# MonsieurETM/QPSK

Hardware: AMD Instinct MI355X
Metric: complex Msamples/s demodulated + % HBM roofline, 2400-baud RRC+Costas path (higher is better)
Workload: dtype f32

## Files before the change

qpsk_amd/csrc/api.cpp:

```cpp
#include "../../include/qpsk_hip.h"
#include "host_math.h"
#include "kernels.h"

#include <hip/hip_runtime.h>
#include <limits.h>
#include <math.h>
#include <stdarg.h>
#include <stdio.h>
#include <stdlib.h>
#include <string.h>
#include <time.h>
#include <algorithm>
#include <initializer_list>
#include <map>
#include <vector>

using namespace qpsk;

static thread_local char g_err[512] = "";

static int fail(int code, const char *fmt, ...)
{
    va_list ap;
    va_start(ap, fmt);
    vsnprintf(g_err, sizeof g_err, fmt, ap);
    va_end(ap);
    return code;
}

#define HIP_TRY(expr)                                                                         \
    do {                                                                                      \
        hipError_t e_ = (expr);                                                               \
        if (e_ != hipSuccess)                                                                 \
            return fail(QPSK_ERR_HIP, "%s: %s (%s:%d)", #expr, hipGetErrorString(e_), __FILE__, __LINE__); \
    } while (0)

#define KERNEL_TRY(expr)                                                                      \
    do {                                                                                      \
        (void)hipGetLastError();  \
        int e_ = (expr);                                                                      \
        if (e_ != 0)                                                                          \
            return fail(QPSK_ERR_HIP, "%s: %s (%s:%d)", #expr, hipGetErrorString((hipError_t)e_), __FILE__, __LINE__); \
    } while (0)

struct DevBuf {
    void *p = nullptr;
    size_t cap = 0;
};

struct Tuning {
    int fused_g = -1, fused_s = -1, fused_lds = -1;
    int generic = -1;
    int pipe_nf = -1;
    int pipe_v = -1, pipe_g = -1;
    int layout_lo = -1, layout_hi = -1;
    int pipe_variant = -1;
    int hist_generic = -1;
    int fir_generic = -1;
    int stream_scan = -1;
    int stream_poll = -1;
    int stream_block = -1;
    int stream_carrier = -1;
    int lean_dma = -1;
    int hist_onepass = -1;
    int est_waves = -1;
    int lean_pair = -1;
    int viterbi_lds = -1;
    int fft_fused = -1;
    int viterbi_chunk_rows = -1;
};

static const struct { const char *name; int Tuning::*field; } TUNING_KEYS[] = {
    {"QPSK_FUSED_G", &Tuning::fused_g},       {"QPSK_FUSED_S", &Tuning::fused_s},     {"QPSK_FUSED_LDS", &Tuning::fused_lds},
    {"QPSK_FUSED_GENERIC", &Tuning::generic}, {"QPSK_PIPE_NF", &Tuning::pipe_nf},
    {"QPSK_PIPE_DBG", &Tuning::pipe_variant}, {"QPSK_HIST_GENERIC", &Tuning::hist_generic},
    {"QPSK_PIPE_V", &Tuning::pipe_v},         {"QPSK_PIPE_G", &Tuning::pipe_g},
    {"QPSK_PIPE_LAYOUT_LO", &Tuning::layout_lo}, {"QPSK_PIPE_LAYOUT_HI", &Tuning::layout_hi},
    {"QPSK_FIR_GENERIC", &Tuning::fir_generic}, {"QPSK_FFT_FUSED", &Tuning::fft_fused},
    {"QPSK_STREAM_BLOCK", &Tuning::stream_block}, {"QPSK_STREAM_POLL", &Tuning::stream_poll},
    {"QPSK_STREAM_SCAN", &Tuning::stream_scan}, {"QPSK_STREAM_CARRIER", &Tuning::stream_carrier},
    {"QPSK_LEAN_DMA", &Tuning::lean_dma},     {"QPSK_LEAN_PAIR", &Tuning::lean_pair},
    {"QPSK_EST_WAVES", &Tuning::est_waves},   {"QPSK_HIST_ONEPASS", &Tuning::hist_onepass},
    {"QPSK_VITERBI_LDS", &Tuning::viterbi_lds},   {"QPSK_VITERBI_CHUNK_ROWS", &Tuning::viterbi_chunk_rows},
};

#ifdef QPSK_PIPE_PROFILE
static const int PIPE_VARIANT_MASK = ~0;
#else
static const int PIPE_VARIANT_MASK = 4 | 8 | 16 | 64 | 128 | 256 | 512 | 1024 | 8192;
#endif

struct qpsk_ctx {
    int device = 0;
    Tuning tune;
    int ncu = 256;
    const char *last_kernel = "";
    int viterbi_launches = 0;
    bool taps_symmetric = false;
    hipStream_t stream = nullptr;
    qpsk_params prm{};
    int cycles = 0, nsym = 0;
    float taps[QPSK_NTAPS];
    float damping = 0.f, alpha = 0.f, beta = 0.f;
    float min_freq = 0.f, max_freq = 0.f;
    float *d_taps = nullptr;
    float *d_gains = nullptr;
    unsigned *h_done = nullptr, *d_done = nullptr;
    unsigned done_expect = 0;
    int *h_status = nullptr;
    int *d_status = nullptr;
    std::vector<float> h_gains;
    DevBuf index, filtered, mixed, keystream, sympad, mislist;
    DevBuf datacostas;
    DevBuf vitdec;
    DevBuf softgain;
    int32_t *d_hint = nullptr;
    int32_t *h_hist_stats = nullptr, *d_hist_stats = nullptr;
    bool hint_valid = false;
    int keystream_len = 0;
    std::map<int, double *> twiddles;
    float *d_fast = nullptr;
    bool fast_valid = false;
    int nstreams = 0;
    float *s_memory = nullptr, *s_dec = nullptr, *s_loop = nullptr, *s_mixer = nullptr;
    float *s_ctab = nullptr, *s_cstate = nullptr;
    bool carrier_shared = false;
    unsigned carrier_blocks = 0;
    unsigned carrier_scans = 0;
    float *carrier_pending = nullptr;
    bool stream_work_unchecked = false;
    bool streams_poisoned = false;
    unsigned char *h_stage = nullptr, *d_stage = nullptr;
    size_t stage_cap = 0;
    int ntx = 0;
    uint8_t *t_hist = nullptr;
    float *t_mixer = nullptr;
    DevBuf tx_b;
    uint8_t *df_state = nullptr, *df_tables = nullptr;
    size_t df_stride = 0;
    int df_nstreams = 0, df_nsync = 0, df_min_score = 0, df_nbytes = 0, df_max_packets = 0;
    unsigned long long df_sync_lo[2] = {0, 0}, df_sync_hi[2] = {0, 0};
    bool df_ready = false;
    bool df_coded = false;
    int df_mode = 0, df_nsteps = 0;
    int df_nbody = 0;
    bool df_punct = false;
    Puncture df_pattern = {1, 1u, 1u, 2};
    float df_scale = 0.f;
    unsigned df_crc_init = 0;
    DevBuf dfstage;
};

static const int MAX_BW = 64;

static int ensure(qpsk_ctx *c, DevBuf &b, size_t bytes)
{
    if (b.cap >= bytes) return QPSK_OK;
    if (b.p) {
        HIP_TRY(hipStreamSynchronize(c->stream));
        HIP_TRY(hipFree(b.p));
        b.p = nullptr;
        b.cap = 0;
    }
    hipError_t e = hipMalloc(&b.p, bytes);
    if (e != hipSuccess) {
        b.p = nullptr;
        return fail(QPSK_ERR_ALLOC, "hipMalloc(%zu bytes): %s", bytes, hipGetErrorString(e));
    }
    b.cap = bytes;
    return QPSK_OK;
}

static int check_status(qpsk_ctx *c)
{
    const int st = __atomic_exchange_n(c->h_status, 0, __ATOMIC_ACQ_REL);
    if (st != STATUS_PIPE_TIMEOUT) c->stream_work_unchecked = false;
    if (st == STATUS_PIPE_TIMEOUT) {
        if (c->nstreams > 0 && c->stream_work_unchecked) {
            c->streams_poisoned = true;
            c->carrier_shared = false;
            c->carrier_pending = nullptr;
        }
        c->stream_work_unchecked = false;
        return fail(QPSK_ERR_HIP, "pipeline kernel: producer/consumer wait timed out; results of the calls since the last synchronisation are invalid");
    }
    if (st == STATUS_PHASE_RANGE)
        return fail(QPSK_ERR_RANGE, "Costas loop phase beyond the bounded 2 pi wrap (input amplitude far outside the modem's range; "
                                    "the reference's phase_wrap() would spin or hang, costas_loop.c:61-67); results of the calls since the last synchronisation are invalid");
    if (st == STATUS_BAD_INDEX)
        return fail(QPSK_ERR_ARG, "an external timing offset (qpsk_rx_batch_ext d_index_in) lies outside 0..%d: the kernel demodulated that frame "
                                  "at offset 0; results of the calls since the last synchronisation are invalid", MAX_INDEX);
    if (st == STATUS_EST_NONFINITE)
        return fail(QPSK_ERR_RANGE, "qpsk_carrier_est_batch: a NaN / Inf sample inside the window the estimate reads; results of the calls since "
                                    "the last synchronisation are invalid");
    if (st == STATUS_SOFT_NONFINITE)
        return fail(QPSK_ERR_RANGE, "qpsk_soft_batch / qpsk_deframer_push_coded: a NaN / Inf sample among those a row's sums or soft output use, or a NaN / Inf gain; "
                                    "results of the calls since the last synchronisation are invalid");
    if (st == STATUS_SOFT_BAD_LAG)
        return fail(QPSK_ERR_ARG, "qpsk_soft_batch: a lag in d_lag is negative or puts the payload beyond the row (that row's soft output is zeros); "
                                  "results of the calls since the last synchronisation are invalid");
    if (st == STATUS_NONFINITE)
        return fail(QPSK_ERR_RANGE, "a Costas loop ended on a NaN / Inf state: the input held a non-finite sample (the reference hangs in phase_wrap() "
                                    "on an infinite phase, costas_loop.c:61-67); results of the calls since the last synchronisation are invalid");
    if (st != 0) return fail(QPSK_ERR_HIP, "kernel status %d", st);
    return QPSK_OK;
}

int qpsk_test_inject_status(qpsk_ctx *c, int code)
{
    if (!c || !c->h_status) return fail(QPSK_ERR_ARG, "null context");
    __atomic_store_n(c->h_status, code, __ATOMIC_RELEASE);
    return QPSK_OK;
}

int qpsk_test_hist_state(qpsk_ctx *c, int32_t *out)
{
    if (!c || !out) return fail(QPSK_ERR_ARG, "null argument");
    out[0] = out[1] = out[2] = out[3] = out[4] = -1;
    if (!c->d_hint) return QPSK_OK;
    HIP_TRY(hipSetDevice(c->device));
    HIP_TRY(hipStreamSynchronize(c->stream));
    int32_t h[2];
    HIP_TRY(hipMemcpy(h, c->d_hint, sizeof h, hipMemcpyDeviceToHost));
    out[0] = c->hint_valid ? h[0] : -1;
    out[1] = h[1];
    out[2] = c->h_hist_stats[0]; out[3] = c->h_hist_stats[1]; out[4] = c->h_hist_stats[2];
    return QPSK_OK;
}

static int bind(const qpsk_ctx *c)
{
    HIP_TRY(hipSetDevice(c->device));
    return QPSK_OK;
}

static int use_context_gains(qpsk_ctx *c)
{
    const float g[2] = {c->alpha, c->beta};
    if (c->h_gains.size() != 2 || c->h_gains[0] != g[0] || c->h_gains[1] != g[1]) {
        HIP_TRY(hipStreamSynchronize(c->stream));
        c->h_gains.assign(g, g + 2);
        HIP_TRY(hipMemcpyAsync(c->d_gains, c->h_gains.data(), sizeof g, hipMemcpyHostToDevice, c->stream));
    }
    return QPSK_OK;
}

extern "C" {

const char *qpsk_last_error(void) { return g_err; }
const char *qpsk_version(void) { return "qpsk_hip 0.3 (gfx950)"; }

int qpsk_device_count(void)
{
    int n = 0;
    if (hipGetDeviceCount(&n) != hipSuccess) return 0;
    return n;
}

void qpsk_params_default(qpsk_params *p)
{
    if (!p) return;
    p->fs = 9600.0;
    p->rs = 2400.0;
    p->frame_size = 512;
    p->rrc_alpha = .35f;
    p->loop_bw = (float)(2.0 * 3.14159265358979323846 / 100.0f);
    p->min_freq = -1.0f;
    p->max_freq = 1.0f;
    p->timing_mode = QPSK_TIMING_HIST;
    p->fixed_index = 0;
}

static int upload_config(qpsk_ctx *c)
{
    float t128[128];
    memset(t128, 0, sizeof t128);
    memcpy(t128, c->taps, sizeof c->taps);
    c->taps_symmetric = true;
    for (int k = 0; k < QPSK_NTAPS / 2; k++)
        if (memcmp(&c->taps[k], &c->taps[QPSK_NTAPS - 1 - k], sizeof(float)) != 0) c->taps_symmetric = false;
    HIP_TRY(hipMemcpyAsync(c->d_taps, t128, sizeof t128, hipMemcpyHostToDevice, c->stream));
    const float g[2] = {c->alpha, c->beta};
    c->h_gains.assign(g, g + 2);
    HIP_TRY(hipMemcpyAsync(c->d_gains, c->h_gains.data(), sizeof g, hipMemcpyHostToDevice, c->stream));
    HIP_TRY(hipStreamSynchronize(c->stream));
    return QPSK_OK;
}

int qpsk_ctx_create(qpsk_ctx **out, int device, const qpsk_params *p, void *stream)
{
    if (!out || !p) return fail(QPSK_ERR_ARG, "qpsk_ctx_create: null argument");
    *out = nullptr;
    int ndev = 0;
    hipError_t e = hipGetDeviceCount(&ndev);
    if (e != hipSuccess || ndev <= 0)
        return fail(QPSK_ERR_NO_DEVICE, "no HIP device available (%s); this library has no CPU path",
                    e == hipSuccess ? "device count 0" : hipGetErrorString(e));
    if (device < 0) HIP_TRY(hipGetDevice(&device));
    if (device >= ndev) return fail(QPSK_ERR_NO_DEVICE, "device %d out of range (%d devices)", device, ndev);
    if (!(p->fs > 0.0) || !(p->rs > 0.0) || p->frame_size <= 0)
        return fail(QPSK_ERR_ARG, "fs, rs and frame_size must be positive");
    const int cycles = (int)(p->fs / p->rs);
    if (cycles < 1 || cycles > 64) return fail(QPSK_ERR_ARG, "CYCLES = (int)(fs/rs) = %d out of range 1..64", cycles);
    if (p->frame_size % cycles != 0)
        return fail(QPSK_ERR_ARG, "frame_size %d is not a multiple of CYCLES %d", p->frame_size, cycles);
    if (p->timing_mode < QPSK_TIMING_HIST || p->timing_mode > QPSK_TIMING_FFT)
        return fail(QPSK_ERR_ARG, "unknown timing_mode %d", p->timing_mode);
    if (p->fixed_index < 0 || p->fixed_index > MAX_INDEX)
        return fail(QPSK_ERR_ARG, "fixed_index %d outside 0..%d", p->fixed_index, MAX_INDEX);

    HIP_TRY(hipSetDevice(device));
    KERNEL_TRY(prepare_kernels());
    KERNEL_TRY(prepare_pipe_kernel());
    KERNEL_TRY(prepare_timing_scan());
    KERNEL_TRY(prepare_stream_block());
    KERNEL_TRY(prepare_stream_scan());
    KERNEL_TRY(prepare_carrier_est());
    qpsk_ctx *c = new qpsk_ctx();
    c->device = device;
    for (const auto &k : TUNING_KEYS) {
        const char *v = getenv(k.name);
        if (!v || !*v) continue;
        if (k.field == &Tuning::viterbi_chunk_rows) {
            char *end = nullptr;
            const long n = strtol(v, &end, 10);
            if (end == v || *end) continue;
            c->tune.*(k.field) = n < 0 ? -1 : n > INT_MAX ? INT_MAX : (int)n;
            continue;
        }
        c->tune.*(k.field) = atoi(v);
    }
    if (c->tune.viterbi_chunk_rows == 0) {
        delete c;
        return fail(QPSK_ERR_ARG, "qpsk_ctx_create: QPSK_VITERBI_CHUNK_ROWS = 0 in the environment (>= 1, or negative for the library's own choice)");
    }
    {
        int ncu = 0;
        if (hipDeviceGetAttribute(&ncu, hipDeviceAttributeMultiprocessorCount, device) == hipSuccess && ncu > 0)
            c->ncu = ncu;
    }
    c->prm = *p;
    c->cycles = cycles;
    c->nsym = p->frame_size / cycles;
    c->stream = (hipStream_t)stream;
    qpsk_host_rrc_taps((float)p->fs, (float)p->rs, p->rrc_alpha, c->taps);
    c->damping = sqrtf(2.0f) / 2.0f;
    qpsk_host_loop_gains(c->damping, p->loop_bw, &c->alpha, &c->beta);
    c->min_freq = p->min_freq;
    c->max_freq = p->max_freq;
    if (hipMalloc((void **)&c->d_taps, 128 * sizeof(float)) != hipSuccess ||
        hipMalloc((void **)&c->d_gains, MAX_BW * 2 * sizeof(float)) != hipSuccess ||
        hipHostMalloc((void **)&c->h_status, sizeof(int), hipHostMallocMapped) != hipSuccess ||
        hipHostGetDevicePointer((void **)&c->d_status, c->h_status, 0) != hipSuccess) {
        qpsk_ctx_destroy(c);
        return fail(QPSK_ERR_ALLOC, "hipMalloc of configuration buffers failed");
    }
    *c->h_status = 0;
    if (hipHostMalloc((void **)&c->h_done, sizeof(unsigned), hipHostMallocMapped) != hipSuccess ||
        hipHostGetDevicePointer((void **)&c->d_done, c->h_done, 0) != hipSuccess) {
        qpsk_ctx_destroy(c);
        return fail(QPSK_ERR_ALLOC, "pinned counter");
    }
    *c->h_done = 0;
    int rc = upload_config(c);
    if (rc != QPSK_OK) { qpsk_ctx_destroy(c); return rc; }
    *out = c;
    return QPSK_OK;
}

static void free_streams(qpsk_ctx *c)
{
    if (c->h_stage) hipHostFree(c->h_stage);
    hipFree(c->d_stage);
    c->h_stage = c->d_stage = nullptr;
    c->stage_cap = 0;
    hipFree(c->s_memory); hipFree(c->s_dec); hipFree(c->s_loop); hipFree(c->s_mixer); hipFree(c->s_ctab); hipFree(c->s_cstate);
    c->s_memory = c->s_dec = c->s_loop = c->s_mixer = c->s_ctab = c->s_cstate = nullptr;
    c->carrier_shared = false;
    c->carrier_pending = nullptr;
    c->nstreams = 0;
}

static void free_deframer(qpsk_ctx *c)
{
    hipFree(c->df_state); hipFree(c->df_tables);
    c->df_state = c->df_tables = nullptr;
    c->df_ready = false;
    c->df_coded = false;
    c->df_punct = false;
    c->df_nstreams = 0;
}

static void free_transmitters(qpsk_ctx *c)
{
    hipFree(c->t_hist); hipFree(c->t_mixer); hipFree(c->tx_b.p);
    c->t_hist = nullptr;
    c->t_mixer = nullptr;
    c->tx_b = DevBuf();
    c->ntx = 0;
}

void qpsk_ctx_destroy(qpsk_ctx *c)
{
    if (!c) return;
    hipSetDevice(c->device);
    hipStreamSynchronize(c->stream);
    hipFree(c->d_taps);
    hipFree(c->d_gains);
    if (c->h_status) hipHostFree(c->h_status);
    if (c->h_done) hipHostFree(c->h_done);
    hipFree(c->index.p);
    hipFree(c->filtered.p);
    hipFree(c->mixed.p);
    hipFree(c->keystream.p);
    hipFree(c->sympad.p);
    hipFree(c->mislist.p);
    hipFree(c->softgain.p);
    hipFree(c->vitdec.p);
    hipFree(c->dfstage.p);
    if (c->d_hint) hipFree(c->d_hint);
    if (c->h_hist_stats) hipHostFree(c->h_hist_stats);
    for (auto &kv : c->twiddles) hipFree(kv.second);
    hipFree(c->d_fast);
    free_streams(c);
    free_transmitters(c);
    free_deframer(c);
    delete c;
}

int qpsk_ctx_sync(qpsk_ctx *c)
{
    if (!c) return fail(QPSK_ERR_ARG, "null context");
    HIP_TRY(hipSetDevice(c->device));
    HIP_TRY(hipStreamSynchronize(c->stream));
    return check_status(c);
}

int qpsk_pack_symbols(qpsk_ctx *c, const uint8_t *d_sym, long long nrows, int nsym, uint8_t *d_packed)
{
    if (!c || !d_sym || !d_packed || nrows < 0 || nsym <= 0) return fail(QPSK_ERR_ARG, "qpsk_pack_symbols: bad argument");
    if (bind(c)) return QPSK_ERR_HIP;
    if ((nsym & 15) == 0 && (((uintptr_t)d_sym & 15) || ((uintptr_t)d_packed & 3)))
        return fail(QPSK_ERR_ARG, "qpsk_pack_symbols: d_sym must be 16-byte and d_packed 4-byte aligned");
    KERNEL_TRY(launch_pack_dibits(d_sym, d_packed, (size_t)nrows, nsym, c->stream));
    return QPSK_OK;
}

int qpsk_unpack_symbols_host(const uint8_t *h_packed, long long nrows, int nsym, uint8_t *h_sym)
{
    if (!h_packed || !h_sym || nrows < 0 || nsym <= 0) return fail(QPSK_ERR_ARG, "qpsk_unpack_symbols_host: bad argument");
    const size_t pb = (size_t)(nsym + 3) / 4;
    for (long long r = 0; r < nrows; r++) {
        const uint8_t *p = h_packed + (size_t)r * pb;
        uint8_t *o = h_sym + (size_t)r * (size_t)nsym;
        for (int i = 0; i < nsym; i++) o[i] = (uint8_t)((p[i >> 2] >> (2 * (i & 3))) & 3u);
    }
    return QPSK_OK;
}

int qpsk_ctx_check(qpsk_ctx *c)
{
    if (!c) return fail(QPSK_ERR_ARG, "null context");
    return check_status(c);
}

int qpsk_set_error(int code, const char *msg)
{
    return fail(code, "%s", msg ? msg : "");
}

int qpsk_ctx_set_stream(qpsk_ctx *c, void *stream)
{
    if (!c) return fail(QPSK_ERR_ARG, "null context");
    HIP_TRY(hipSetDevice(c->device));
    HIP_TRY(hipStreamSynchronize(c->stream));
    c->stream = (hipStream_t)stream;
    return QPSK_OK;
}

int qpsk_ctx_set_tuning(qpsk_ctx *c, const char *name, int value)
{
    if (!c || !name) return fail(QPSK_ERR_ARG, "null argument");
    for (const auto &k : TUNING_KEYS)
        if (!strcmp(k.name, name)) {
            if (value == 0 && k.field == &Tuning::viterbi_chunk_rows)
                return fail(QPSK_ERR_ARG, "qpsk_ctx_set_tuning: QPSK_VITERBI_CHUNK_ROWS = 0 (>= 1, or negative for the library's own choice)");
            c->tune.*(k.field) = value < 0 ? -1 : value;
            return QPSK_OK;
        }
    return fail(QPSK_ERR_ARG, "qpsk_ctx_set_tuning: unknown name '%s'", name);
}

int qpsk_ctx_cycles(const qpsk_ctx *c) { return c ? c->cycles : 0; }
int qpsk_ctx_nsym(const qpsk_ctx *c) { return c ? c->nsym : 0; }
const char *qpsk_ctx_last_kernel(const qpsk_ctx *c) { return c ? c->last_kernel : ""; }

int qpsk_ctx_get_taps(const qpsk_ctx *c, float *h)
{
    if (!c || !h) return fail(QPSK_ERR_ARG, "null argument");
    memcpy(h, c->taps, sizeof c->taps);
    return QPSK_OK;
}

int qpsk_ctx_get_gains(const qpsk_ctx *c, float *a, float *b)
{
    if (!c || !a || !b) return fail(QPSK_ERR_ARG, "null argument");
    *a = c->alpha;
    *b = c->beta;
    return QPSK_OK;
}

int qpsk_ctx_set_taps(qpsk_ctx *c, const float *h)
{
    if (!c || !h) return fail(QPSK_ERR_ARG, "null argument");
    if (bind(c)) return QPSK_ERR_HIP;
    memcpy(c->taps, h, sizeof c->taps);
    c->fast_valid = false;
    return upload_config(c);
}

int qpsk_ctx_set_loop(qpsk_ctx *c, float alpha, float beta, float min_freq, float max_freq)
{
    if (!c) return fail(QPSK_ERR_ARG, "null argument");
    if (bind(c)) return QPSK_ERR_HIP;
    c->min_freq = min_freq; c->max_freq = max_freq;
    if (alpha == c->alpha && beta == c->beta && !(alpha == 0.0f && beta == 0.0f)) return QPSK_OK;
    c->alpha = alpha; c->beta = beta;
    return upload_config(c);
}

static int tuned(int v, int dflt) { return v >= 0 ? v : dflt; }

static int fir_full_rate(qpsk_ctx *c, const float *x, const float *memory, float *y, int nframes, int length, size_t in_pitch = 0)
{
    if (c->taps_symmetric && tuned(c->tune.fir_generic, 0) == 0)
        return launch_rrc_fir_stream(x, memory, y, c->d_taps, nframes, length, c->stream, in_pitch, c->ncu);
    return launch_rrc_fir(x, memory, y, c->d_taps, nframes, length, c->stream, in_pitch);
}

static void pick_tiling(const qpsk_ctx *c, int nframes, int nbw, int *G, int *S)
{
    int g = nframes / 256;
    if (g < 1) g = 1;
    if (g > 64 / nbw) g = 64 / nbw;
    if (g < 1) g = 1;
    g = tuned(c->tune.fused_g, g);
    if (g < 1) g = 1;
    if (g * nbw > 64) g = 64 / nbw;
    int s = tuned(c->tune.fused_s, 64);
    s &= ~7;
    if (s < 8) s = 8;
    const size_t budget = (size_t)tuned(c->tune.fused_lds, 64 * 1024);
    while (s > 8 && fused_lds_bytes(g, s, c->cycles, nbw) > budget) s -= 8;
    while (g > 1 && fused_lds_bytes(g, s, c->cycles, nbw) > (size_t)MAX_LDS_BYTES) g--;
    *G = g;
    *S = s;
}

static int get_twiddles(qpsk_ctx *c, int n, double **out)
{
    auto it = c->twiddles.find(n);
    if (it != c->twiddles.end()) { *out = it->second; return QPSK_OK; }
    const size_t cnt = n >= 2 ? (size_t)n / 2 : 1;
    std::vector<double> h(2 * cnt, 0.0);
    qpsk_host_twiddles(n, h.data());
    double *tw = nullptr;
    HIP_TRY(hipMalloc((void **)&tw, sizeof(double) * 2 * cnt));
    HIP_TRY(hipMemcpy(tw, h.data(), sizeof(double) * 2 * cnt, hipMemcpyHostToDevice));
    c->twiddles[n] = tw;
    *out = tw;
    return QPSK_OK;
}

static int fft_timing_tables(qpsk_ctx *c, double **tw_out, double **cs_out)
{
    const int C = c->cycles, nfft = timing_fft_nfft();
    if (C < 2 || C > 8 || (C & (C - 1)))
        return fail(QPSK_ERR_ARG, "QPSK_TIMING_FFT needs CYCLES in {2,4,8} (the symbol-rate bin NFFT/CYCLES must be exact and the offset < 8); CYCLES = %d", C);
    if (c->prm.frame_size < timing_fft_first() + nfft)
        return fail(QPSK_ERR_ARG, "QPSK_TIMING_FFT needs frame_size >= %d", timing_fft_first() + nfft);
    double *tw = nullptr;
    int rc = get_twiddles(c, nfft, &tw);
    if (rc) return rc;
    double *cs = nullptr;
    auto it = c->twiddles.find(-C);
    if (it == c->twiddles.end()) {
        std::vector<double> full(2 * (size_t)C);
        qpsk_host_phases(C, full.data());
        HIP_TRY(hipMalloc((void **)&cs, sizeof(double) * 2 * C));
        HIP_TRY(hipMemcpy(cs, full.data(), sizeof(double) * 2 * C, hipMemcpyHostToDevice));
        c->twiddles[-C] = cs;
    } else {
        cs = it->second;
    }
    *tw_out = tw;
    *cs_out = cs;
    return QPSK_OK;
}

static int fft_timing_indices(qpsk_ctx *c, const float *d_in, int nframes, int32_t *d_index, float *d_y = nullptr,
                              double *d_X = nullptr, size_t pitch = 0, double *d_bin = nullptr)
{
    double *tw = nullptr, *cs = nullptr;
    int rc = fft_timing_tables(c, &tw, &cs);
    if (rc) return rc;
    KERNEL_TRY(launch_timing_fft(d_in, nframes, c->prm.frame_size, c->cycles, c->d_taps, tw, cs, d_index, d_y, d_X, d_bin, c->stream, pitch,
                                 c->ncu, c->taps_symmetric && tuned(c->tune.fir_generic, 0) == 0));
    return QPSK_OK;
}

static bool scan_fused_ok(const qpsk_ctx *c, const float *d_in)
{
    return c->cycles == 8 && c->prm.frame_size % timing_scan_tile() == 0 && ((uintptr_t)d_in % 16) == 0 &&
           tuned(c->tune.hist_generic, 0) == 0;
}

static int timing_indices(qpsk_ctx *c, const float *d_in, size_t pitch, int nframes, const int32_t **d_index_out, bool fused_fft = false)
{
    *d_index_out = nullptr;
    if (c->prm.timing_mode == QPSK_TIMING_FIXED) return QPSK_OK;
    int rc = ensure(c, c->index, sizeof(int32_t) * (size_t)nframes);
    if (rc) return rc;
    if (fused_fft && c->prm.timing_mode == QPSK_TIMING_FFT) return QPSK_OK;
    if (c->prm.timing_mode == QPSK_TIMING_HIST) {
        if (scan_fused_ok(c, d_in) && (pitch & 1) == 0) {
            KERNEL_TRY(launch_timing_scan(d_in, nframes, c->prm.frame_size, c->d_taps, (int32_t *)c->index.p, nullptr,
                                          c->d_status, c->stream, pitch, c->taps_symmetric && tuned(c->tune.fir_generic, 0) == 0));
            *d_index_out = (const int32_t *)c->index.p;
            return QPSK_OK;
        }
        const size_t bytes = sizeof(float) * 2 * (size_t)nframes * c->prm.frame_size;
        rc = ensure(c, c->filtered, bytes);
        if (rc) return rc;
        KERNEL_TRY(fir_full_rate(c, d_in, nullptr, (float *)c->filtered.p, nframes, c->prm.frame_size, pitch));
        KERNEL_TRY(launch_timing_hist((const float *)c->filtered.p, nframes, c->prm.frame_size, c->cycles,
                                      (int32_t *)c->index.p, nullptr, tuned(c->tune.hist_generic, 0) == 2, c->stream));
        *d_index_out = (const int32_t *)c->index.p;
        return QPSK_OK;
    }
    rc = fft_timing_indices(c, d_in, nframes, (int32_t *)c->index.p, nullptr, nullptr, pitch);
    if (rc) return rc;
    *d_index_out = (const int32_t *)c->index.p;
    return QPSK_OK;
}

struct ExtAcq {
    const int32_t *index;
    const float *seed;
};

enum RxKind { K_GENERIC, K_FUSED_PIPE, K_PIPE2, K_LEAN };

struct RxRoute {
    RxKind kind = K_GENERIC;
    int G = 0;
    int nf = 0;
    unsigned long long layout = 0;
    bool pipe_ok = false;
    bool fused_fft = false;
    bool need_pad = false;
    bool data_rule = false;
    bool need_dump = false;
};

static bool tuned_layout(const qpsk_ctx *c, unsigned long long *layout)
{
    if (c->tune.layout_lo < 0 && c->tune.layout_hi < 0) return false;
    *layout = ((unsigned long long)(unsigned)tuned(c->tune.layout_lo, 0) << 4) | ((unsigned long long)(unsigned)tuned(c->tune.layout_hi, 0) << 24);
    return true;
}

static int rx_route(const qpsk_ctx *c, const FusedArgs &a, bool want_data, RxRoute *rt)
{
    const int nframes = a.nframes, nbw = a.nbw;
    *rt = RxRoute{};
    const bool pipe_ok = rt->pipe_ok = c->cycles == pipe_cycles() && (a.frame_size % 2) == 0 && (a.frame_pitch % 2) == 0 &&
                                       ((uintptr_t)a.x % 16) == 0 && nbw * pipe_frames(1) <= 64 && tuned(c->tune.generic, 0) == 0;
    const int by_size = nframes > 16 * c->ncu ? 2 : 1;
    int pipe_v = tuned(c->tune.pipe_v, by_size);
    unsigned long long own_layout = 0;
    const bool has_layout = tuned_layout(c, &own_layout);

    if (pipe_ok && c->taps_symmetric && (pipe_v == 3 || c->tune.pipe_v < 0) && !(want_data && !a.data_rule)) {
        int G = tuned(c->tune.pipe_g, (nframes + c->ncu - 1) / c->ncu);
        if (G > pipe2_max_frames()) G = pipe2_max_frames();
        G += G & 1;
        const bool wanted = pipe_v == 3 || G >= 4;
        const unsigned long long layout = has_layout ? own_layout : G >= 2 ? lean_default_layout(G / 2) : 0;
        if (wanted && layout && lean_shape_ok(a, G)) {
            const LayoutCount n = layout_count(layout);
            if (n.units == G / 2 && lean_lds_bytes(G, n.nwin) <= (size_t)MAX_LDS_BYTES) {
                rt->kind = K_LEAN;
                rt->G = G;
                rt->layout = layout;
                rt->need_pad = nframes % G != 0;
                rt->data_rule = a.data_rule != 0;
            }
        }
    }
    const bool older = rt->kind != K_LEAN && pipe_ok;
    if (pipe_v == 3) pipe_v = by_size;
    if (older && pipe_v == 2) {
        int G = tuned(c->tune.pipe_g, (nframes + c->ncu - 1) / c->ncu);
        if (G > pipe2_max_frames()) G = pipe2_max_frames();
        if (G * nbw > 64) G = 64 / nbw;
        if (G < 1) G = 1;
        unsigned long long layout = own_layout;
        if (has_layout) {
            const LayoutCount n = layout_count(layout);
            if (n.units < 1 || (G + 1) / 2 != n.units || pipe2_lds_bytes(G, n.nwin, nbw) > (size_t)MAX_LDS_BYTES)
                return fail(QPSK_ERR_ARG, "QPSK_PIPE_LAYOUT_*: %d units on %d waves do not match %d frames per workgroup", n.units, n.nwin, G);
        } else {
            for (;;) {
                layout = pipe2_default_layout((G + 1) / 2);
                if (layout && pipe2_lds_bytes(G, layout_count(layout).nwin, nbw) <= (size_t)MAX_LDS_BYTES) break;
                if (G == 1) return fail(QPSK_ERR_ARG, "pipeline geometry does not fit: %d loops per frame", nbw);
                G--;
            }
        }
        rt->kind = K_PIPE2;
        rt->G = G;
        rt->layout = layout;
    } else if (older) {
        const int full = pipe_max_nf();
        int nf = 1;
        while (nf < full && (long long)c->ncu * pipe_frames(nf) < nframes) nf++;
        nf = tuned(c->tune.pipe_nf, nf);
        if (nf < 1) nf = 1;
        if (nf > full) nf = full;
        while (pipe_frames(nf) * nbw > 64 || pipe_lds_bytes(nf, nbw) > (size_t)MAX_LDS_BYTES) {
            if (nf == 1) return fail(QPSK_ERR_ARG, "pipeline geometry does not fit: nf %d, %d loops per frame", nf, nbw);
            nf--;
        }
        rt->kind = K_FUSED_PIPE;
        rt->nf = nf;
    }
    rt->need_dump = want_data && !rt->data_rule && !a.costas;
    rt->fused_fft = c->prm.timing_mode == QPSK_TIMING_FFT && !a.index && nbw == 1 && tuned(c->tune.fft_fused, 1) != 0 &&
                    a.frame_size >= timing_fft_first() + timing_fft_nfft() &&
                    ((rt->kind == K_FUSED_PIPE && rt->nf == pipe_max_nf() && !(a.dbg & (128 | 4))) ||
                     (rt->kind == K_LEAN && lean_est_ok(a, rt->G, rt->layout)));
    return QPSK_OK;
}

static int rx_hist_onepass(qpsk_ctx *c, const FusedArgs &a, const RxRoute &rt, int32_t *d_index, bool *taken)
{
    *taken = false;
    if (!rt.pipe_ok || !c->taps_symmetric || !scan_fused_ok(c, (const float *)a.x) || c->tune.pipe_v >= 0) return QPSK_OK;
    if (!c->d_hint) {
        HIP_TRY(hipMalloc((void **)&c->d_hint, 2 * sizeof(int32_t)));
        HIP_TRY(hipMemset(c->d_hint, 0, 2 * sizeof(int32_t)));
        HIP_TRY(hipHostMalloc((void **)&c->h_hist_stats, 4 * sizeof(int32_t), hipHostMallocMapped));
        HIP_TRY(hipHostGetDevicePointer((void **)&c->d_hist_stats, c->h_hist_stats, 0));
        c->h_hist_stats[0] = c->h_hist_stats[1] = c->h_hist_stats[2] = -1;
        c->hint_valid = false;
    }
    const int op = tuned(c->tune.hist_onepass, -1);
    const int seen = __atomic_load_n(&c->h_hist_stats[1], __ATOMIC_ACQUIRE), off_majority = __atomic_load_n(&c->h_hist_stats[2], __ATOMIC_ACQUIRE);
    const bool guess_is_good = seen > 0 && off_majority == 0;
    if (op == 0 || !c->hint_valid || !(op == 1 || guess_is_good) || !rx_hist_shape_ok(a)) return QPSK_OK;
    if (int rc = ensure(c, c->index, sizeof(int32_t) * (size_t)a.nframes)) return rc;
    if (int rc = ensure(c, c->mislist, sizeof(int32_t) * (size_t)a.nframes)) return rc;
    int32_t *mis_count = c->d_hint + 1;
    KERNEL_TRY(launch_rx_hist(a, (int32_t *)c->index.p, c->d_hint, (int32_t *)c->mislist.p, mis_count, c->d_status, c->stream));
    FusedArgs af = a;
    af.index = (const int32_t *)c->index.p;
    af.frame_list = (const int32_t *)c->mislist.p;
    af.frame_list_count = mis_count;
    af.G = 4;
    af.S = 64;
    KERNEL_TRY(launch_rx_fused(af, c->stream));
    KERNEL_TRY(launch_index_majority((const int32_t *)c->index.p, a.nframes, c->d_hint, mis_count, c->d_hist_stats, c->stream));
    c->last_kernel = "rx_hist_kernel (one pass on the guessed index) + rx_fused_kernel (fall-back list)";
    if (d_index)
        HIP_TRY(hipMemcpyAsync(d_index, c->index.p, sizeof(int32_t) * (size_t)a.nframes, hipMemcpyDeviceToDevice, c->stream));
    *taken = true;
    return QPSK_OK;
}

static int rx_launch(qpsk_ctx *c, const FusedArgs &a, const RxRoute &rt)
{
    if (a.est_tw && !(rt.kind == K_FUSED_PIPE && rt.nf == pipe_max_nf()) && rt.kind != K_LEAN)
        return fail(QPSK_ERR_STATE, "internal: in-launch FFT timing estimate planned for a kernel that has none");
    if (a.data_rule && rt.kind != K_LEAN)
        return fail(QPSK_ERR_STATE, "internal: data rule planned for a kernel that has none");
    switch (rt.kind) {
    case K_LEAN:
        KERNEL_TRY(launch_rx_lean(a, rt.G, rt.layout, c->d_status, c->stream));
        c->last_kernel = a.est_tw ? "rx_lean_kernel (FFT timing estimate inside the launch)" : "rx_lean_kernel";
        break;
    case K_PIPE2:
        KERNEL_TRY(launch_rx_pipe2(a, rt.G, rt.layout, c->d_status, c->stream));
        c->last_kernel = "rx_pipe2_kernel";
        break;
    case K_FUSED_PIPE:
        KERNEL_TRY(launch_rx_fused_pipe(a, rt.nf, c->d_status, c->stream));
        c->last_kernel = a.est_tw ? "rx_fused_pipe_kernel (FFT timing estimate inside the launch)" : "rx_fused_pipe_kernel";
        break;
    default:
        KERNEL_TRY(launch_rx_fused(a, c->stream));
        c->last_kernel = "rx_fused_kernel";
    }
    return QPSK_OK;
}

static int rx_batch_common(qpsk_ctx *c, const float *d_in, long long frame_pitch, int nframes, int nbw, uint8_t *d_sym,
                           float *d_freq, float *d_phase, float *d_costas, int32_t *d_index, float *d_hz,
                           const ExtAcq *ext = nullptr, uint8_t *d_data = nullptr)
{
    if (!c || !d_in || !(d_sym || d_data)) return fail(QPSK_ERR_ARG, "qpsk_rx_batch: null context, input or symbol buffer");
    if (nframes <= 0) return fail(QPSK_ERR_ARG, "qpsk_rx_batch: nframes = %d", nframes);
    if (frame_pitch == 0) frame_pitch = c->prm.frame_size;
    if (frame_pitch < c->prm.frame_size)
        return fail(QPSK_ERR_ARG, "qpsk_rx_batch_pitched: frame_pitch %lld below frame_size %d", frame_pitch, c->prm.frame_size);
    if (bind(c)) return QPSK_ERR_HIP;
    FusedArgs a{};
    a.x = reinterpret_cast<const float2 *>(d_in);
    a.frame_pitch = (size_t)frame_pitch;
    a.nframes = nframes;
    a.frame_size = c->prm.frame_size;
    a.cycles = c->cycles;
    a.nsym = c->nsym;
    pick_tiling(c, nframes, nbw, &a.G, &a.S);
    a.fixed_index = c->prm.fixed_index;
    a.dbg = tuned(c->tune.pipe_variant, 0) & PIPE_VARIANT_MASK;
    a.lean_dma = tuned(c->tune.lean_dma, 1) != 0;
    a.lean_twowin = tuned(c->tune.lean_dma, 1) != 2 ? 1 : 0;
    a.est_waves = tuned(c->tune.est_waves, 0);
    a.lean_pair = tuned(c->tune.lean_pair, 3);
    a.taps = c->d_taps;
    a.gains = c->d_gains;
    a.nbw = nbw;
    a.min_freq = c->min_freq;
    a.max_freq = c->max_freq;
    a.rs = c->prm.rs;
    a.sym = d_sym ? d_sym : d_data;
    a.data_rule = d_data && !d_sym;
    a.freq = d_freq;
    a.phase = d_phase;
    a.costas = reinterpret_cast<float2 *>(d_costas);
    a.hz = d_hz;
    a.status = c->d_status;
    if (ext) a.index = ext->index;
    if (ext && ext->seed) {
        a.state_in = ext->seed;
        a.seed_setters = 1;
    }

    RxRoute rt;
    if (int rc = rx_route(c, a, d_data != nullptr, &rt)) return rc;

    a.data_rule = rt.data_rule;
    if (rt.need_pad) {
        if (int rc = ensure(c, c->sympad, (size_t)rt.G * (size_t)c->nsym)) return rc;
        a.sym_pad = (uint8_t *)c->sympad.p;
    }
    if (rt.need_dump) {
        if (int rc = ensure(c, c->datacostas, sizeof(float2) * (size_t)nframes * (size_t)c->nsym)) return rc;
        a.costas = (float2 *)c->datacostas.p;
    }

    const bool hist_guess = c->prm.timing_mode == QPSK_TIMING_HIST && !ext;
    if (hist_guess) {
        bool taken = false;
        const int rc = rx_hist_onepass(c, a, rt, d_index, &taken);
        if (rc || taken) return rc;
    }

    const int32_t *idx = a.index;
    if (!idx) {
        if (int rc = timing_indices(c, d_in, (size_t)frame_pitch, nframes, &idx, rt.fused_fft)) return rc;
        a.index = idx;
    }
    if (rt.fused_fft) {
        double *est_tw = nullptr, *est_cs = nullptr;
        if (int rc = fft_timing_tables(c, &est_tw, &est_cs)) return rc;
        a.est_tw = reinterpret_cast<const double2 *>(est_tw);
        a.est_cs = reinterpret_cast<const double2 *>(est_cs);
        a.index_out = d_index ? (int32_t *)c->index.p : nullptr;
        if (d_index) idx = (const int32_t *)c->index.p;
    }

    if (int rc = rx_launch(c, a, rt)) return rc;

    if (hist_guess && c->d_hint && idx && tuned(c->tune.hist_onepass, -1) != 0) {
        KERNEL_TRY(launch_index_majority(idx, nframes, c->d_hint, c->d_hint + 1, c->d_hist_stats, c->stream));
        c->hint_valid = true;
    }
    if (rt.kind == K_LEAN && (nframes & 1)) {
        const size_t last0 = (size_t)((nframes - 1) / rt.G) * (size_t)rt.G;
        HIP_TRY(hipMemcpyAsync(a.sym + (size_t)(nframes - 1) * (size_t)c->nsym, a.sym_pad + ((size_t)(nframes - 1) - last0) * (size_t)c->nsym,
                               (size_t)c->nsym, hipMemcpyDeviceToDevice, c->stream));
    }
    if (d_data && !a.data_rule)
        KERNEL_TRY(launch_data_from_costas(a.costas, d_data, (size_t)nframes * (size_t)c->nsym, c->stream));
    if (d_index) {
        if (idx == d_index) {
        } else if (idx)
            HIP_TRY(hipMemcpyAsync(d_index, idx, sizeof(int32_t) * (size_t)nframes, hipMemcpyDeviceToDevice, c->stream));
        else
            KERNEL_TRY(launch_fill_i32(d_index, nframes, c->prm.fixed_index, c->stream));
    }
    return QPSK_OK;
}

static int rx_prologue(qpsk_ctx *c)
{
    if (!c) return QPSK_OK;
    if (bind(c)) return QPSK_ERR_HIP;
    return use_context_gains(c);
}

int qpsk_rx_batch(qpsk_ctx *c, const float *d_in, int nframes, uint8_t *d_sym, float *d_freq, float *d_phase,
                  float *d_costas, int32_t *d_index, float *d_hz)
{
    if (int rp = rx_prologue(c)) return rp;
    return rx_batch_common(c, d_in, 0, nframes, 1, d_sym, d_freq, d_phase, d_costas, d_index, d_hz);
}

int qpsk_rx_batch_pitched(qpsk_ctx *c, const float *d_in, long long frame_pitch, int nframes, uint8_t *d_sym, float *d_freq,
                          float *d_phase, float *d_costas, int32_t *d_index, float *d_hz)
{
    if (int rp = rx_prologue(c)) return rp;
    if (frame_pitch <= 0) return fail(QPSK_ERR_ARG, "qpsk_rx_batch_pitched: frame_pitch = %lld", frame_pitch);
    return rx_batch_common(c, d_in, frame_pitch, nframes, 1, d_sym, d_freq, d_phase, d_costas, d_index, d_hz);
}

static int rx_batch_bw_impl(qpsk_ctx *c, const float *d_in, int nframes, const float *h_loop_bw, int nbw, uint8_t *d_sym,
                            float *d_freq, float *d_phase, int32_t *d_index, const ExtAcq *ext)
{
    if (!c || !h_loop_bw) return fail(QPSK_ERR_ARG, "qpsk_rx_batch_bw: null argument");
    if (nbw < 1 || nbw > MAX_BW) return fail(QPSK_ERR_ARG, "nbw = %d outside 1..%d", nbw, MAX_BW);
    if (bind(c)) return QPSK_ERR_HIP;
    std::vector<float> g(2 * (size_t)nbw);
    for (int b = 0; b < nbw; b++)
        qpsk_host_loop_gains(c->damping, h_loop_bw[b], &g[2 * b], &g[2 * b + 1]);
    if (g != c->h_gains) {
        HIP_TRY(hipStreamSynchronize(c->stream));
        c->h_gains = g;
        HIP_TRY(hipMemcpyAsync(c->d_gains, c->h_gains.data(), sizeof(float) * g.size(), hipMemcpyHostToDevice, c->stream));
    }
    return rx_batch_common(c, d_in, 0, nframes, nbw, d_sym, d_freq, d_phase, nullptr, d_index, nullptr, ext);
}

int qpsk_rx_batch_bw(qpsk_ctx *c, const float *d_in, int nframes, const float *h_loop_bw, int nbw, uint8_t *d_sym,
                     float *d_freq, float *d_phase, int32_t *d_index)
{
    return rx_batch_bw_impl(c, d_in, nframes, h_loop_bw, nbw, d_sym, d_freq, d_phase, d_index, nullptr);
}

int qpsk_rx_batch_ext(qpsk_ctx *c, const float *d_in, long long frame_pitch, int nframes, const int32_t *d_index_in, const float *d_seed,
                      uint8_t *d_sym, float *d_freq, float *d_phase, float *d_costas, int32_t *d_index, float *d_hz)
{
    if (int rp = rx_prologue(c)) return rp;
    if (frame_pitch < 0) return fail(QPSK_ERR_ARG, "qpsk_rx_batch_ext: frame_pitch = %lld", frame_pitch);
    const ExtAcq ext = {d_index_in, d_seed};
    return rx_batch_common(c, d_in, frame_pitch, nframes, 1, d_sym, d_freq, d_phase, d_costas, d_index, d_hz, &ext);
}

int qpsk_rx_batch_data(qpsk_ctx *c, const float *d_in, long long frame_pitch, int nframes, const int32_t *d_index_in, const float *d_seed,
                       uint8_t *d_data, uint8_t *d_sym, float *d_freq, float *d_phase, int32_t *d_index, float *d_hz)
{
    if (int rp = rx_prologue(c)) return rp;
    if (frame_pitch < 0) return fail(QPSK_ERR_ARG, "qpsk_rx_batch_data: frame_pitch = %lld", frame_pitch);
    if (!d_data) return fail(QPSK_ERR_ARG, "qpsk_rx_batch_data: d_data is NULL");
    const ExtAcq ext = {d_index_in, d_seed};
    return rx_batch_common(c, d_in, frame_pitch, nframes, 1, d_sym, d_freq, d_phase, nullptr, d_index, d_hz, &ext, d_data);
}

int qpsk_sync_batch(qpsk_ctx *c, const uint8_t *d_data, int nframes, int nsym, const uint8_t *h_sync, int nsync, int lag_min, int lag_max,
                    int nout, uint8_t *d_out, int32_t *d_lag, int32_t *d_rot, int32_t *d_score)
{
    if (!c || !d_data || !h_sync) return fail(QPSK_ERR_ARG, "qpsk_sync_batch: null context, data or sync word");
    if (nframes <= 0 || nsym <= 0) return fail(QPSK_ERR_ARG, "qpsk_sync_batch: nframes = %d, nsym = %d", nframes, nsym);
    if (nsync < 1 || nsync > SYNC_MAX_WORD) return fail(QPSK_ERR_ARG, "qpsk_sync_batch: nsync = %d outside 1..%d", nsync, SYNC_MAX_WORD);
    if (nout < 0 || lag_min < 0 || lag_max < lag_min || (long long)lag_max + nsync + nout > nsym)
        return fail(QPSK_ERR_ARG, "qpsk_sync_batch: lags %d..%d, nsync %d, nout %d do not fit a row of %d", lag_min, lag_max, nsync, nout, nsym);
    if (!d_out && !d_lag && !d_rot && !d_score) return fail(QPSK_ERR_ARG, "qpsk_sync_batch: every output is NULL");
    for (int i = 0; i < nsync; i++)
        if (h_sync[i] > 3) return fail(QPSK_ERR_ARG, "qpsk_sync_batch: sync[%d] = %d is not a dibit", i, (int)h_sync[i]);
    if (d_out && nout > 0) {
        const uintptr_t o0 = (uintptr_t)d_out, o1 = o0 + (size_t)nframes * (size_t)nout;
        const uintptr_t d0 = (uintptr_t)d_data, d1 = d0 + (size_t)nframes * (size_t)nsym;
        if (o0 < d1 && d0 < o1) return fail(QPSK_ERR_ARG, "qpsk_sync_batch: d_out overlaps d_data");
    }
    if (bind(c)) return QPSK_ERR_HIP;
    KERNEL_TRY(launch_sync_search(d_data, nframes, nsym, h_sync, nsync, lag_min, lag_max, nout, nout > 0 ? d_out : nullptr, d_lag, d_rot,
                                  d_score, c->stream));
    c->last_kernel = "sync_search_kernel";
    return QPSK_OK;
}

int qpsk_rx_batch_bw_ext(qpsk_ctx *c, const float *d_in, int nframes, const float *h_loop_bw, int nbw, const int32_t *d_index_in,
                         const float *d_seed, uint8_t *d_sym, float *d_freq, float *d_phase, int32_t *d_index)
{
    const ExtAcq ext = {d_index_in, d_seed};
    return rx_batch_bw_impl(c, d_in, nframes, h_loop_bw, nbw, d_sym, d_freq, d_phase, d_index, &ext);
}

static int costas_over_symbols(qpsk_ctx *c, float *d_symbols, int nframes, int nsym, int dstride, float *d_state,
                               uint8_t *d_sym, float *d_costas, const float *refill = nullptr,
                               const int32_t *refill_index = nullptr, bool refill_planar = false)
{
    float *carrier_tab = c->carrier_pending;
    c->carrier_pending = nullptr;
    if (tuned(c->tune.generic, 0)) {
        if (carrier_tab) KERNEL_TRY(launch_carrier_table(c->s_cstate, carrier_tab, c->prm.frame_size, true, c->stream));
        KERNEL_TRY(launch_costas(d_symbols, nframes, nsym, dstride, 1, c->d_gains, c->min_freq, c->max_freq, d_state, d_state,
                                 d_sym, d_costas, c->d_status, c->stream));
        if (refill) {
            if (dstride != nsym) return fail(QPSK_ERR_ARG, "internal: refill needs packed rows");
            KERNEL_TRY(launch_decimate(refill, refill_index, d_symbols, nframes, nsym * c->cycles, c->cycles, nsym, c->stream));
        }
        return QPSK_OK;
    }
    FusedArgs a{};
    a.nframes = nframes;
    a.nsym = nsym;
    a.frame_size = nsym * c->cycles;
    a.cycles = c->cycles;
    a.refill = reinterpret_cast<const float2 *>(refill);
    a.refill_dst = reinterpret_cast<float2 *>(d_symbols);
    a.refill_planar = refill_planar ? 1 : 0;
    a.index = refill_index;
    a.gains = c->d_gains;
    a.nbw = 1;
    a.min_freq = c->min_freq;
    a.max_freq = c->max_freq;
    a.rs = c->prm.rs;
    a.state_in = d_state;
    a.state_out = d_state;
    a.sym = d_sym;
    a.costas = reinterpret_cast<float2 *>(d_costas);
    a.dsrc = reinterpret_cast<const float2 *>(d_symbols);
    a.dstride = dstride;
    a.status = c->d_status;
    if (carrier_tab) {
        a.carrier_state = c->s_cstate;
        a.carrier_tab = reinterpret_cast<float2 *>(carrier_tab);
        a.carrier_frame = c->prm.frame_size;
    }
    a.dbg = tuned(c->tune.pipe_variant, 0) & PIPE_VARIANT_MASK;
    int nf = (nframes + c->ncu * pipe_frames(1) - 1) / (c->ncu * pipe_frames(1));
    if (nf < 1) nf = 1;
    if (nf > pipe_max_nf()) nf = pipe_max_nf();
    KERNEL_TRY(launch_costas_pipe(a, nf, c->d_status, c->stream));
    return QPSK_OK;
}

int qpsk_rrc_fir_batch(qpsk_ctx *c, float *d_memory, const float *d_in, float *d_out, int nframes, int length)
{
    if (!c || !d_in || !d_out) return fail(QPSK_ERR_ARG, "qpsk_rrc_fir_batch: null argument");
    if (nframes <= 0 || length <= 0) return fail(QPSK_ERR_ARG, "qpsk_rrc_fir_batch: nframes %d length %d", nframes, length);
    if (bind(c)) return QPSK_ERR_HIP;
    const float *src = d_in;
    if (d_in == d_out) {
        const size_t bytes = sizeof(float) * 2 * (size_t)nframes * length;
        int rc = ensure(c, c->mixed, bytes);
        if (rc) return rc;
        HIP_TRY(hipMemcpyAsync(c->mixed.p, d_in, bytes, hipMemcpyDeviceToDevice, c->stream));
        src = (const float *)c->mixed.p;
    }
    KERNEL_TRY(fir_full_rate(c, src, d_memory, d_out, nframes, length));
    if (d_memory) KERNEL_TRY(launch_delay_line(src, d_memory, nframes, length, c->stream));
    return QPSK_OK;
}

int qpsk_rrc_fir_batch_fast(qpsk_ctx *c, float *d_memory, const float *d_in, float *d_out, int nframes, int length)
{
    if (!c || !d_in || !d_out) return fail(QPSK_ERR_ARG, "qpsk_rrc_fir_batch_fast: null argument");
    if (nframes <= 0 || length <= 0) return fail(QPSK_ERR_ARG, "qpsk_rrc_fir_batch_fast: nframes %d length %d", nframes, length);
    if (d_in == d_out) return fail(QPSK_ERR_ARG, "qpsk_rrc_fir_batch_fast: every block reads 126 samples in front of it: separate buffers");
    if (bind(c)) return QPSK_ERR_HIP;
    if (!c->fast_valid) {
        const int n = rrc_fir_fast_nfft();
        std::vector<float> t(4 * (size_t)n);
        qpsk_host_fir_fast_tables(c->taps, t.data(), t.data() + 2 * n);
        if (!c->d_fast) HIP_TRY(hipMalloc((void **)&c->d_fast, sizeof(float) * t.size()));
        HIP_TRY(hipStreamSynchronize(c->stream));
        HIP_TRY(hipMemcpy(c->d_fast, t.data(), sizeof(float) * t.size(), hipMemcpyHostToDevice));
        c->fast_valid = true;
    }
    KERNEL_TRY(launch_rrc_fir_fast(d_in, d_memory, d_out, c->d_fast, c->d_fast + 2 * rrc_fir_fast_nfft(), nframes, length, c->stream));
    if (d_memory) KERNEL_TRY(launch_delay_line(d_in, d_memory, nframes, length, c->stream));
    return QPSK_OK;
}

int qpsk_timing_hist_batch(qpsk_ctx *c, const float *d_filtered, int nframes, int32_t *d_index, int32_t *d_hist)
{
    if (!c || !d_filtered || !d_index) return fail(QPSK_ERR_ARG, "qpsk_timing_hist_batch: null argument");
    if (nframes <= 0) return fail(QPSK_ERR_ARG, "nframes = %d", nframes);
    if (bind(c)) return QPSK_ERR_HIP;
    KERNEL_TRY(launch_timing_hist(d_filtered, nframes, c->prm.frame_size, c->cycles, d_index, d_hist,
                                  tuned(c->tune.hist_generic, 0) == 2, c->stream));
    return QPSK_OK;
}

int qpsk_timing_scan_batch(qpsk_ctx *c, const float *d_in, int nframes, int32_t *d_index, int32_t *d_hist)
{
    if (!c || !d_in || !d_index) return fail(QPSK_ERR_ARG, "qpsk_timing_scan_batch: null argument");
    if (nframes <= 0) return fail(QPSK_ERR_ARG, "nframes = %d", nframes);
    if (bind(c)) return QPSK_ERR_HIP;
    if (!(c->cycles == 8 && c->prm.frame_size % timing_scan_tile() == 0 && ((uintptr_t)d_in % 16) == 0))
        return fail(QPSK_ERR_ARG, "qpsk_timing_scan_batch needs CYCLES = 8, frame_size %% %d == 0 and 16-byte aligned input "
                                  "(use qpsk_rrc_fir_batch + qpsk_timing_hist_batch otherwise)", timing_scan_tile());
    KERNEL_TRY(launch_timing_scan(d_in, nframes, c->prm.frame_size, c->d_taps, d_index, d_hist, c->d_status, c->stream, 0,
                                  c->taps_symmetric && tuned(c->tune.fir_generic, 0) == 0));
    return QPSK_OK;
}

int qpsk_timing_fft_batch(qpsk_ctx *c, const float *d_in, int nframes, int32_t *d_index, float *d_filtered, double *d_spectrum)
{
    if (!c || !d_in || !d_index) return fail(QPSK_ERR_ARG, "qpsk_timing_fft_batch: null argument");
    if (nframes <= 0) return fail(QPSK_ERR_ARG, "nframes = %d", nframes);
    if (bind(c)) return QPSK_ERR_HIP;
    return fft_timing_indices(c, d_in, nframes, d_index, d_filtered, d_spectrum);
}

int qpsk_timing_fft_bin_batch(qpsk_ctx *c, const float *d_in, int nframes, int32_t *d_index, float *d_filtered, double *d_bin)
{
    if (!c || !d_in || !d_index) return fail(QPSK_ERR_ARG, "qpsk_timing_fft_bin_batch: null argument");
    if (nframes <= 0) return fail(QPSK_ERR_ARG, "nframes = %d", nframes);
    if (bind(c)) return QPSK_ERR_HIP;
    return fft_timing_indices(c, d_in, nframes, d_index, d_filtered, nullptr, 0, d_bin);
}

static float carrier_est_omega(int k, int C, int n)
{
    const double tau = 2.0 * 3.14159265358979323846;
    return (float)(tau * (double)(k * C) / (double)(4 * n));
}

int qpsk_carrier_est_batch(qpsk_ctx *c, const float *d_in, long long frame_pitch, int nframes, int start, int n, float *d_seed,
                           float *d_freq, int32_t *d_bin, double *d_line)
{
    if (!c || !d_in) return fail(QPSK_ERR_ARG, "qpsk_carrier_est_batch: null context or input");
    if (!d_seed && !d_freq && !d_bin && !d_line) return fail(QPSK_ERR_ARG, "qpsk_carrier_est_batch: every output is NULL");
    if (nframes <= 0) return fail(QPSK_ERR_ARG, "qpsk_carrier_est_batch: nframes = %d", nframes);
    if (n < 64 || n > 8192 || (n & (n - 1)))
        return fail(QPSK_ERR_ARG, "qpsk_carrier_est_batch: n = %d must be a power of two in 64..8192", n);
    const int fs = c->prm.frame_size;
    if (start < 0 || (long long)start + n > fs)
        return fail(QPSK_ERR_ARG, "qpsk_carrier_est_batch: start %d + n %d outside the frame (%d samples)", start, n, fs);
    if (frame_pitch == 0) frame_pitch = fs;
    if (frame_pitch < fs || (frame_pitch % 2) != 0)
        return fail(QPSK_ERR_ARG, "qpsk_carrier_est_batch: frame_pitch = %lld (0, or even and >= frame_size %d)", frame_pitch, fs);
    const int C = c->cycles;
    int klo = 1, khi = 0;
    for (int k = -(n / (2 * C)); k <= n / (2 * C); k++) {
        if ((long long)(k < 0 ? -k : k) * 2 * C >= n) continue;
        const float w = carrier_est_omega(k, C, n);
        if (!(w >= c->min_freq && w <= c->max_freq)) continue;
        if (klo > khi) klo = k;
        khi = k;
    }
    if (klo > khi)
        return fail(QPSK_ERR_ARG, "qpsk_carrier_est_batch: no bin |k| < n / (2 CYCLES) = %d / %d lies in the loop clamp [%g, %g]", n, 2 * C,
                    (double)c->min_freq, (double)c->max_freq);
    const int kdef = klo <= 0 && khi >= 0 ? 0 : (khi < 0 ? khi : klo);
    if (bind(c)) return QPSK_ERR_HIP;
    double *tw = nullptr;
    if (int rt = get_twiddles(c, n, &tw)) return rt;
    KERNEL_TRY(launch_carrier_est(d_in, (size_t)frame_pitch, nframes, start, n, C, klo, khi, kdef, c->d_taps, tw, d_seed, d_freq, d_bin,
                                  d_line, c->d_status, c->taps_symmetric && tuned(c->tune.fir_generic, 0) == 0, c->stream));
    c->last_kernel = "carrier_est_kernel";
    return QPSK_OK;
}

int qpsk_soft_batch(qpsk_ctx *c, const float *d_costas, long long row_pitch, int nrows, int nsym, int skip, int mode, float scale,
                    const float *d_gain_in, const int32_t *d_lag, const int32_t *d_rot, int first, int nout, int8_t *d_soft,
                    float *d_quality, double *d_sums)
{
    if (!c || !d_costas) return fail(QPSK_ERR_ARG, "qpsk_soft_batch: null context or input");
    if (!d_soft && !d_quality && !d_sums) return fail(QPSK_ERR_ARG, "qpsk_soft_batch: every output is NULL");
    if (nrows <= 0 || nsym <= 0 || nsym > SOFT_MAX_NSYM)
        return fail(QPSK_ERR_ARG, "qpsk_soft_batch: nrows = %d, nsym = %d (1..%d)", nrows, nsym, SOFT_MAX_NSYM);
    if (skip < 0 || skip >= nsym) return fail(QPSK_ERR_ARG, "qpsk_soft_batch: skip = %d outside 0..%d", skip, nsym - 1);
    if (mode != QPSK_SOFT_UNIT && mode != QPSK_SOFT_LLR) return fail(QPSK_ERR_ARG, "qpsk_soft_batch: unknown mode %d", mode);
    if (!(scale > 0.0f && scale <= 3.402823466e+38f)) return fail(QPSK_ERR_ARG, "qpsk_soft_batch: scale = %g is not finite and > 0", (double)scale);
    if (row_pitch == 0) row_pitch = nsym;
    if (row_pitch < nsym) return fail(QPSK_ERR_ARG, "qpsk_soft_batch: row_pitch = %lld (0, or >= nsym %d)", row_pitch, nsym);
    if ((uintptr_t)d_costas % 8) return fail(QPSK_ERR_ARG, "qpsk_soft_batch: d_costas is not 8-byte aligned");
    if (d_soft) {
        if (nout < 0 || first < 0 || (long long)first + nout > nsym)
            return fail(QPSK_ERR_ARG, "qpsk_soft_batch: first %d, nout %d do not fit a row of %d", first, nout, nsym);
        if ((uintptr_t)d_soft % 2) return fail(QPSK_ERR_ARG, "qpsk_soft_batch: d_soft is not 2-byte aligned");
        const uintptr_t o0 = (uintptr_t)d_soft, o1 = o0 + 2 * (size_t)nrows * (size_t)nout;
        const uintptr_t i0 = (uintptr_t)d_costas, i1 = i0 + 8 * ((size_t)(nrows - 1) * (size_t)row_pitch + (size_t)nsym);
        if (o0 < i1 && i0 < o1) return fail(QPSK_ERR_ARG, "qpsk_soft_batch: d_soft overlaps d_costas");
    }
    static_assert(QPSK_SOFT_UNIT == SOFT_MODE_UNIT && QPSK_SOFT_LLR == SOFT_MODE_LLR, "the kernels take the header's mode values");
    if (bind(c)) return QPSK_ERR_HIP;
    const size_t pitch = (size_t)row_pitch;
    const bool need_sums = d_quality || d_sums || !d_gain_in;
    if (!d_soft) {
// ... 971 lines not shown
```

qpsk_amd/csrc/kernels.h:

```cpp
#ifndef QPSK_KERNELS_H
#define QPSK_KERNELS_H

#include <hip/hip_runtime.h>
#include <stddef.h>
#include <stdint.h>

namespace qpsk {

constexpr int LOOKBACK = 128;
constexpr int LOOKAHEAD = 8;
constexpr int MAX_LDS_BYTES = 160 * 1024;
constexpr int MAX_INDEX = 7;
constexpr int STATUS_PIPE_TIMEOUT = 1;
constexpr int STATUS_PHASE_RANGE = 2;
constexpr int STATUS_NONFINITE = 3;
constexpr int STATUS_BAD_INDEX = 4;
constexpr int STATUS_EST_NONFINITE = 5;
constexpr int STATUS_SOFT_NONFINITE = 6;
constexpr int STATUS_SOFT_BAD_LAG = 7;

struct FusedArgs {
    const float2 *x;
    size_t frame_pitch;
    int nframes, frame_size, cycles, nsym;
    int G, S;
    int mixed;
    int share_simd0;
    const int32_t *index;
    int fixed_index;
    const double2 *est_tw, *est_cs;
    int32_t *index_out;
    int lean_twowin;
    int lean_dma;
    int est_waves;
    int lean_pair;
    int dbg;
    const float2 *dsrc;
    int dstride;
    const float2 *refill;
    float2 *refill_dst;
    int refill_planar;
    const int32_t *frame_list, *frame_list_count;
    const float *taps;
    const float *gains;
    int nbw;
    float min_freq, max_freq;
    double rs;
    const float *state_in;
    int seed_setters;
    float *state_out;
    uint8_t *sym;
    uint8_t *sym_pad;
    float *freq, *phase;
    float2 *costas;
    float *hz;
    int *status;
    float *carrier_state;
    float2 *carrier_tab;
    int carrier_frame;
    int data_rule;
};

size_t fused_lds_bytes(int G, int S, int cycles, int nbw);
int prepare_kernels(void);
int launch_rx_fused(const FusedArgs &a, hipStream_t s);
size_t pipe_lds_bytes(int NF, int nbw);
int pipe_frames(int NF);
int pipe_cycles(void);
int pipe_max_nf(void);
int prepare_pipe_kernel(void);
int launch_rx_fused_pipe(const FusedArgs &a, int NF, int *status, hipStream_t s);
int launch_costas_pipe(const FusedArgs &a, int NF, int *status, hipStream_t s);
size_t pipe2_lds_bytes(int G, int nwin, int nbw);
int pipe2_max_fir(void);
int pipe2_max_frames(void);
int pipe2_max_units_per_wave(void);
int pipe2_max_hw_waves(void);
unsigned long long pipe2_default_layout(int NU);
struct LayoutCount { int units, nwin; };
inline LayoutCount layout_count(unsigned long long layout)
{
    LayoutCount n = {0, 0};
    for (int w = 1; w < 16; w++) {
        const int cw = (int)((layout >> (4 * w)) & 15);
        n.units += cw;
        n.nwin += cw != 0;
    }
    return n;
}
int launch_rx_pipe2(const FusedArgs &a, int G, unsigned long long layout, int *status, hipStream_t s);
size_t lean_lds_bytes(int G, int nwin);
unsigned long long lean_default_layout(int NU);
bool lean_shape_ok(const FusedArgs &a, int G);
int launch_rx_lean(const FusedArgs &a, int G, unsigned long long layout, int *status, hipStream_t s);
bool lean_est_ok(const FusedArgs &a, int G, unsigned long long layout);
bool rx_hist_shape_ok(const FusedArgs &a);
int launch_rx_hist(const FusedArgs &a, int32_t *index_true, const int32_t *hint, int32_t *mis_list, int32_t *mis_count, int *status, hipStream_t s);
int launch_index_majority(const int32_t *index, int nframes, int32_t *hint, int32_t *mis_count, int32_t *h_stats, hipStream_t s);
int launch_rrc_fir(const float *x, const float *memory, float *y, const float *taps, int nframes, int length,
                   hipStream_t s, size_t in_pitch = 0);
int launch_rrc_fir_stream(const float *x, const float *memory, float *y, const float *taps, int nframes, int length,
                          hipStream_t s, size_t in_pitch = 0, int ncu = 0);
int launch_delay_line(const float *x, float *memory, int nframes, int length, hipStream_t s);
int launch_rrc_fir_fast(const float *x, const float *memory, float *y, const float *H, const float *tw, int nframes, int length,
                        hipStream_t s);
int rrc_fir_fast_hop(void);
int rrc_fir_fast_nfft(void);
int launch_timing_hist(const float *y, int nframes, int frame_size, int cycles, int32_t *index, int32_t *hist,
                       bool generic, hipStream_t s);
int launch_costas(const float *d, int nframes, int nsym, int dstride, int nbw, const float *gains, float min_freq,
                  float max_freq, const float *state_in, float *state_out, uint8_t *sym, float *costas, int *status,
                  hipStream_t s);
int launch_decimate(const float *filtered, const int32_t *index, float *dec, int nstreams, int frame_size,
                    int cycles, int nsym, hipStream_t s);
int launch_mixer(const int16_t *pcm, float *out, float *state, int nstreams, int frame_size, hipStream_t s);
int launch_fft(const double *in, double *out, const double *tw, int nbatch, int n, int log2n, int inverse,
               hipStream_t s);
int fft_lds_max_n(void);
int fft_big_block(void);
int launch_fft_big(const double *in, double *out, const double *twb, const double *twn, int nbatch, int n, int log2n,
                   int inverse, hipStream_t s);
size_t timing_scan_lds_bytes(void);
int timing_scan_tile(void);
int prepare_timing_scan(void);
int launch_timing_scan(const float *x, int nframes, int frame_size, const float *taps, int32_t *index, int32_t *hist,
                       int *status, hipStream_t s, size_t pitch = 0, bool symmetric = false);
int launch_timing_fft(const float *x, int nframes, int frame_size, int cycles, const float *taps, const double *tw,
                      const double *cs, int32_t *index, float *yout, double *Xout, double *Xk, hipStream_t s, size_t pitch = 0,
                      int ncu = 0, bool symmetric = false);
int timing_fft_nfft(void);
int timing_fft_first(void);
int prepare_carrier_est(void);
int launch_carrier_est(const float *x, size_t pitch, int nframes, int start, int n, int cycles, int klo, int khi, int kdef,
                       const float *taps, const double *tw, float *seed, float *freq, int32_t *bin, double *line, int *status,
                       bool symmetric, hipStream_t s);
struct StreamBlockArgs {
    const int16_t *pcm;
    const float2 *cplx;
    float *mixer;
    float2 *memory;
    float2 *dec;
    float *loop;
    const float *loop_in;
    float *loop_out;
    const float *taps, *gains;
    float min_freq, max_freq;
    int frame_size, cycles, nsym, hist_timing, fixed_index;
    uint8_t *sym;
    float2 *costas;
    int32_t *index;
    float2 *filtered;
    int *status;
    unsigned *done;
    const float2 *ctab;
    float2 *ctab_next;
    float *cstate;
};
struct StreamBlockInline {
    static constexpr int MAX_STREAMS = 8, MAX_SAMPLES = 1024;
    float loop[2 * MAX_STREAMS];
    uint4 pcm[MAX_SAMPLES / 8];
};
size_t stream_block_lds_bytes(int frame_size, int nsym);
int stream_block_max_frame(void);
int prepare_stream_block(void);
int launch_stream_block(const StreamBlockArgs &a, int nstreams, hipStream_t s, const StreamBlockInline *inl = nullptr);
int stream_scan_tile(void);
int prepare_stream_scan(void);
int launch_stream_scan(const int16_t *pcm, const float *x, float *mixer, float *memory, float *yout, const float *taps, int32_t *index,
                       int nstreams, int frame_size, int *status, hipStream_t s, const float *ctab = nullptr, float *ctab_next = nullptr,
                       float *cstate = nullptr, unsigned cseq = 0, int cycles = 8);
int launch_carrier_table(float *cstate, float *tab, int frame_size, bool rest_only, hipStream_t s);
int launch_carrier_broadcast(const float *cstate, float *mixer, int nstreams, hipStream_t s);
int launch_crc16(const uint8_t *data, int npackets, int nbytes, uint16_t *crc, hipStream_t s);
int launch_interleave(uint8_t *data, int npackets, int nbytes, unsigned b, int dir, hipStream_t s);
int launch_scramble(uint8_t *sym, const uint8_t *keystream, int npackets, int nsym, hipStream_t s);
int launch_pack_dibits(const uint8_t *sym, uint8_t *packed, size_t nrows, int nsym, hipStream_t s);
constexpr int SYNC_MAX_WORD = 128;
int launch_sync_search(const uint8_t *data, int nframes, int nsym, const uint8_t *h_sync, int nsync, int lag_min, int lag_max, int nout,
                       uint8_t *out, int32_t *lag, int32_t *rot, int32_t *score, hipStream_t s);
int launch_data_from_costas(const float2 *costas, uint8_t *data, size_t n, hipStream_t s);
constexpr int SOFT_ONE_PASS_MAX = 4096;
constexpr int SOFT_MAX_NSYM = 1 << 21;
constexpr int SOFT_MODE_UNIT = 0, SOFT_MODE_LLR = 1;
int launch_soft_onepass(const float *x, size_t pitch, int nrows, int nsym, int skip, int mode, float scale, const float *gain_in,
                        const int32_t *lag, const int32_t *rot, int first, int nout, int8_t *soft, float *quality, double *sums, int *status,
                        hipStream_t s);
int launch_soft_sums(const float *x, size_t pitch, int nrows, int nsym, int skip, int mode, float scale, float *gain_out, float *quality,
                     double *sums, int *status, hipStream_t s);
int launch_soft_apply(const float *x, size_t pitch, int nrows, int nsym, const float *gain, bool check_gain, const int32_t *lag,
                      const int32_t *rot, int first, int nout, int8_t *soft, int *status, hipStream_t s);
constexpr int VITERBI_MAX_STEPS = 131072;
constexpr int VITERBI_LDS_MAX_BYTES = 65536;
constexpr int VITERBI_OPEN_START = 1, VITERBI_OPEN_END = 2, VITERBI_PROFILE_FORWARD_ONLY = 0x100, VITERBI_PROFILE_CYCLES = 0x200;
size_t viterbi_scratch_bytes_per_row(int nsteps);
struct Puncture {
    int period;
    unsigned keep0, keep1;
    int K;
};
inline long long punct_nsent(const Puncture &p, int nsteps)
{
    const unsigned r = (unsigned)(nsteps % p.period), low = (1u << r) - 1u;
    return (long long)(nsteps / p.period) * p.K + __builtin_popcount(p.keep0 & low) + __builtin_popcount(p.keep1 & low);
}
int launch_viterbi(const int8_t *soft, size_t pitch, int nrows, int nsteps, const Puncture *punct, const uint8_t *flip, int flags,
                   unsigned long long *scratch, bool lds, uint8_t *bits, int32_t *info, hipStream_t s);
int launch_conv_encode(const uint8_t *bits, int nrows, int nbits, int nsteps, uint8_t *dibits, hipStream_t s);
int launch_conv_encode_punct(const uint8_t *bits, int nrows, int nbits, int nsteps, const Puncture &punct, uint8_t *dibits, hipStream_t s);
struct DeframeHeader {
    long long len;
    long long h;
    long long ppos;
    int pending, have, prot, pscore;
};
constexpr int DEFRAME_TAIL_OFFSET = 64, DEFRAME_PEND_OFFSET = 192;
constexpr int DEFRAME_MAX_BYTES = 1024, DEFRAME_MAX_PACKETS = 64, DEFRAME_MAX_NSYM = 1 << 21;
struct DeframeHuntArgs {
    int nstreams, nsym;
    int nsync, min_score;
    uint8_t *state;
    size_t state_stride;
    unsigned long long sync_lo[2], sync_hi[2];
    long long *pos;
    int32_t *rot, *score;
    int32_t *count;
};
__device__ __forceinline__ void report(const DeframeHuntArgs &a, size_t r, long long pos, int rot, int score, int lane)
{
    if (a.pos) {
        if (lane == 0) a.pos[r] = pos;
    }
    if (a.rot) {
        if (lane == 0) a.rot[r] = rot;
    }
    if (a.score) {
        if (lane == 0) a.score[r] = score;
    }
}
struct DeframeArgs : DeframeHuntArgs {
    uint8_t *bytes;
    const uint8_t *data;
    const float2 *costas;
    int nbytes, max_packets;
    int bytes_per_lane;
    const uint8_t *keystream;
    const uint16_t *crc_adv;
    uint8_t *crc_ok;
};
int launch_deframe(const DeframeArgs &a, hipStream_t s);
constexpr int DEFRAME_CODED_MAX_STEPS = 8 * (DEFRAME_MAX_BYTES + 2) + 6;
struct DeframeCodedArgs : DeframeHuntArgs {
    uint8_t *bytes;
    const float2 *costas;
    const float *gain;
    int check_gain;
    int nbytes, max_packets;
    int nsteps;
    int per_stream;
    int8_t *stage;
    const uint8_t *flip;
    const uint16_t *crc_adv;
    unsigned crc_init;
    uint8_t *crc_ok;
    int32_t *info;
    int *status;
};
struct DeframeCodedBody {
    int nbody;
    int stage_pitch;
    int punctured;
    Puncture punct;
};
int launch_deframe_coded_hunt(const DeframeCodedArgs &a, const DeframeCodedBody &b, hipStream_t s);
int launch_deframe_coded_decode(const DeframeCodedArgs &a, const DeframeCodedBody &b, int row0, int nrows, unsigned long long *scratch, bool lds,
                                hipStream_t s);
int tx_history_symbols(void);
int launch_tx_shape(const uint8_t *sym, uint8_t *hist, const float *taps, float *sig, int nstreams, int nsym,
                    int cycles, hipStream_t s);
int launch_tx_upmix(const float *sig, int16_t *pcm, float *state, int nstreams, int length, hipStream_t s);
int launch_fill_i32(int32_t *p, int n, int32_t v, hipStream_t s);
int launch_sincos_hash(uint32_t first, uint32_t count, unsigned long long *acc, hipStream_t s);

}
#endif
```

qpsk_amd/csrc/kernels.hip:

```cpp
#include <hip/hip_runtime.h>
#include <stdint.h>
#include "qpsk_device.h"
#include "fft_lds.h"
#include "kernels.h"

namespace qpsk {

constexpr int FUSED_THREADS = 256;

__global__ void __launch_bounds__(FUSED_THREADS)
rx_fused_kernel(FusedArgs a)
{
    extern __shared__ __attribute__((aligned(16))) unsigned char smem[];
    const int G = a.G, S = a.S, C = a.cycles, L = a.frame_size, N = a.nsym, nbw = a.nbw;
    const int W = S * C + LOOKBACK + LOOKAHEAD;
    float *taps = reinterpret_cast<float *>(smem);
    float2 *xs = reinterpret_cast<float2 *>(smem + 512);
    float2 *ds = xs + (size_t)G * W;
    float2 *zs = ds + (size_t)G * S;
    uint8_t *ss = reinterpret_cast<uint8_t *>(zs + (size_t)G * nbw * S);
    int *idx = reinterpret_cast<int *>(ss + (size_t)G * nbw * S);
    int *fid = idx + G;

    const int tid = threadIdx.x;
    const int f0 = blockIdx.x * G;
    const int total = a.frame_list_count ? min(*a.frame_list_count, a.nframes) : a.nframes;
    if (f0 >= total) return;
    const int gcount = min(G, total - f0);

    if (tid < 128)
        taps[tid] = tid < NTAPS ? a.taps[tid] : 0.0f;
    if (tid < G) {
        const int fr = tid < gcount ? (a.frame_list ? a.frame_list[f0 + tid] : f0 + tid) : 0;
        fid[tid] = fr;
        idx[tid] = (tid < gcount) ? checked_index(a.index ? a.index[fr] : a.fixed_index, a.status) : 0;
    }

    const int lane_g = tid / nbw, lane_b = tid % nbw;
    const bool costas_lane = tid < gcount * nbw && tid < 64;
    Loop st = {0.0f, 0.0f};
    bool over = false;
    LoopGains lg = {0.0f, 0.0f, a.min_freq, a.max_freq};
    __syncthreads();
    if (costas_lane) {
        lg.alpha = a.gains[2 * lane_b];
        lg.beta = a.gains[2 * lane_b + 1];
        if (a.state_in) {
            st.phase = a.state_in[2 * ((size_t)fid[lane_g] * nbw + lane_b)];
            st.freq = a.state_in[2 * ((size_t)fid[lane_g] * nbw + lane_b) + 1];
            if (a.seed_setters) seed_setters(st.phase, st.freq, a.min_freq, a.max_freq, over);
        }
    }

    const int nchunks = (N + S - 1) / S;
    for (int c = 0; c < nchunks; c++) {
        const int sym0 = c * S;
        const int base = sym0 * C - LOOKBACK;

        for (int i = tid; i < gcount * W; i += FUSED_THREADS) {
            const int g = i / W, w = i - g * W;
            const int n = base + w;
            float2 v = make_float2(0.0f, 0.0f);
            if (n >= 0 && n < L)
                v = a.x[(size_t)fid[g] * a.frame_pitch + n];
            xs[(size_t)g * W + w] = v;
        }
        __syncthreads();

        for (int o = tid; o < gcount * S; o += FUSED_THREADS) {
            const int g = o / S, j = o - g * S;
            const int n = (sym0 + j) * C + idx[g];
            float2 d = make_float2(0.0f, 0.0f);
            if (n < L && sym0 + j < N) {
                const float2 *w = xs + (size_t)g * W + (n - HIST - base);
                float2 y = make_float2(0.0f, 0.0f);
#pragma unroll 8
                for (int k = 0; k < NTAPS; k++)
                    fir_mac(y, w[k], taps[k]);
                d = fir_gain(y);
            }
            ds[o] = d;
        }
        __syncthreads();

        if (costas_lane) {
            const int cnt = min(S, N - sym0);
            const float2 *dl = ds + (size_t)lane_g * S;
            for (int j = 0; j < cnt; j++) {
                const float2 z = (c == 0 && j == 0) ? costas_step<true>(st, lg, dl[j], over) : costas_step<false>(st, lg, dl[j], over);
                ss[(size_t)tid * S + j] = (uint8_t)slicer(z);
                if (a.costas)
                    zs[(size_t)tid * S + j] = z;
            }
        }
        __syncthreads();

        {
            const int cnt = min(S, N - sym0);
            const int rows = gcount * nbw;
            for (int i = tid; i < rows * cnt; i += FUSED_THREADS) {
                const int r = i / cnt, j = i - r * cnt;
                const size_t o = ((size_t)fid[r / nbw] * nbw + r % nbw) * N + sym0 + j;
                a.sym[o] = ss[(size_t)r * S + j];
                if (a.costas)
                    a.costas[o] = zs[(size_t)r * S + j];
            }
        }
    }

    if (costas_lane) {
        const size_t o = (size_t)fid[lane_g] * nbw + lane_b;
        if (a.freq) a.freq[o] = st.freq;
        if (a.phase) a.phase[o] = st.phase;
        if (a.hz) a.hz[o] = (float)((double)st.freq * a.rs / TAU);
        if (a.state_out) {
            a.state_out[2 * o] = st.phase;
            a.state_out[2 * o + 1] = st.freq;
        }
        if (over && a.status) __hip_atomic_store(a.status, STATUS_PHASE_RANGE, __ATOMIC_RELAXED, __HIP_MEMORY_SCOPE_SYSTEM);
        else if (a.status && !loop_state_finite(st.phase, st.freq))
            __hip_atomic_store(a.status, STATUS_NONFINITE, __ATOMIC_RELAXED, __HIP_MEMORY_SCOPE_SYSTEM);
    }
}

size_t fused_lds_bytes(int G, int S, int cycles, int nbw)
{
    const size_t W = (size_t)S * cycles + LOOKBACK + LOOKAHEAD;
    size_t b = 512 + sizeof(float2) * ((size_t)G * W + (size_t)G * S + (size_t)G * nbw * S);
    b += (size_t)G * nbw * S;
    b = (b + 15) & ~(size_t)15;
    b += sizeof(int) * 2 * (size_t)G;
    return b;
}

constexpr int FIR_THREADS = 256;
constexpr int FR = 8;
constexpr int FIR_TILE = FIR_THREADS * FR;
constexpr int FIR_WIN = FIR_TILE + HIST;
constexpr int FIR_SLOTS = FIR_WIN + FIR_WIN / 8 + 1;

__global__ void __launch_bounds__(FIR_THREADS, 2)
rrc_fir_kernel(const float2 *__restrict__ x, const float2 *__restrict__ memory, float2 *__restrict__ y,
               const float *__restrict__ taps_g, int length, size_t in_pitch)
{
    __shared__ __attribute__((aligned(16))) float taps[128];
    __shared__ float2 xs[FIR_SLOTS];
    const int tid = threadIdx.x, f = blockIdx.y;
    const int n0 = blockIdx.x * FIR_TILE;
    if (tid < 128)
        taps[tid] = tid < NTAPS ? taps_g[tid] : 0.0f;
    for (int i = tid; i < FIR_WIN; i += FIR_THREADS) {
        const int n = n0 - HIST + i;
        float2 v = make_float2(0.0f, 0.0f);
        if (n >= 0) {
            if (n < length) v = x[(size_t)f * in_pitch + n];
        } else if (memory) {
            v = memory[(size_t)f * NTAPS + (NTAPS + n)];
        }
        xs[i + (i >> 3)] = v;
    }
    __syncthreads();

    const float2 *rd = xs + 9 * tid;
    const float4 *taps4 = reinterpret_cast<const float4 *>(taps);
    constexpr int TS = NTAPS + FR - 1, NB = (TS + 7) / 8;
    static_assert(FR == 8, "the pinned step names 8 products");
    float tg[3][8];
    float2 wv[2][8];
    auto fetch_block = [&](int tb) {
        if (tb * 8 < NTAPS) {
            const float4 ta = taps4[2 * tb], tc = taps4[2 * tb + 1];
            float *g_ = tg[tb % 3];
            g_[0] = ta.x; g_[1] = ta.y; g_[2] = ta.z; g_[3] = ta.w;
            g_[4] = tc.x; g_[5] = tc.y; g_[6] = tc.z; g_[7] = tc.w;
        }
#pragma unroll
        for (int u = 0; u < 8; u++) {
            const int t = tb * 8 + u;
            if (t < TS) wv[tb & 1][u] = rd[t + (t >> 3)];
        }
    };
    v2f ac[FR];
#pragma unroll
    for (int r = 0; r < FR; r++) ac[r] = v2f{0.0f, 0.0f};
    fetch_block(0);
    static_for<0, NB>([&](auto tbc) {
        constexpr int tb = decltype(tbc)::value;
        if (tb + 1 < NB) fetch_block(tb + 1);
        static_for<0, 8>([&](auto uc) {
            constexpr int u = decltype(uc)::value, t = tb * 8 + u;
            if constexpr (t < TS) {
                const v2f v = v2f{wv[tb & 1][u].x, wv[tb & 1][u].y};
                v2f p[FR];
                static_for<0, FR>([&](auto rc) {
                    constexpr int r = decltype(rc)::value, k = t - r;
                    if constexpr (k >= 0 && k < NTAPS) p[r] = v * tg[(k >> 3) % 3][k & 7];
                });
                if constexpr (t >= FR - 1 && t < NTAPS) {
                    asm volatile("" : "+v"(p[0]), "+v"(p[1]), "+v"(p[2]), "+v"(p[3]), "+v"(p[4]), "+v"(p[5]), "+v"(p[6]), "+v"(p[7]));
                } else {
#define QPSK_PIN_P(r) if constexpr (t - (r) >= 0 && t - (r) < NTAPS) asm volatile("" : "+v"(p[r]))
                    QPSK_PIN_P(0); QPSK_PIN_P(1); QPSK_PIN_P(2); QPSK_PIN_P(3);
                    QPSK_PIN_P(4); QPSK_PIN_P(5); QPSK_PIN_P(6); QPSK_PIN_P(7);
#undef QPSK_PIN_P
                }
                static_for<0, FR>([&](auto rc) {
                    constexpr int r = decltype(rc)::value, k = t - r;
                    if constexpr (k >= 0 && k < NTAPS) ac[r] = ac[r] + p[r];
                });
                asm volatile("" : "+v"(ac[0]), "+v"(ac[1]), "+v"(ac[2]), "+v"(ac[3]), "+v"(ac[4]), "+v"(ac[5]), "+v"(ac[6]), "+v"(ac[7]));
            }
        });
    });
    __syncthreads();
#pragma unroll
    for (int r = 0; r < FR; r++)
        xs[9 * tid + r] = fir_gain(make_float2(ac[r].x, ac[r].y));
    __syncthreads();
#pragma unroll
    for (int j = 0; j < FR; j++) {
        const int i = j * FIR_THREADS + tid, n = n0 + i;
        if (n < length)
            y[(size_t)f * length + n] = xs[i + (i >> 3)];
    }
}

__global__ void __launch_bounds__(128)
delay_line_kernel(const float2 *__restrict__ x, float2 *memory, int length)
{
    const int f = blockIdx.x, i = threadIdx.x;
    float2 v = make_float2(0.0f, 0.0f);
    if (i < NTAPS) {
        const int src = i + length - NTAPS;
        v = src >= 0 ? x[(size_t)f * length + src] : memory[(size_t)f * NTAPS + (i + length)];
    }
    __syncthreads();
    if (i < NTAPS)
        memory[(size_t)f * NTAPS + i] = v;
}

constexpr int TH_FRAMES = 16;
constexpr int TH_TILE = 64;

__global__ void __launch_bounds__(64)
timing_hist_kernel(const float *__restrict__ y, int nframes, int frame_size, int cycles, int32_t *index,
                   int32_t *hist_out)
{
    __shared__ float2 tile[TH_FRAMES][TH_TILE + 1];
    const int lane = threadIdx.x;
    const int f0 = blockIdx.x * TH_FRAMES;
    const int fl = (lane >> 1) & (TH_FRAMES - 1), comp = lane & 1;
    const bool scanning = lane < 2 * TH_FRAMES && f0 + fl < nframes;
    const float2 *y2 = reinterpret_cast<const float2 *>(y);
    const int ntiles = (frame_size + TH_TILE - 1) / TH_TILE;

    float2 pre[TH_FRAMES];
    auto fetch = [&](int t) {
        const int s = min(t * TH_TILE + lane, frame_size - 1);
#pragma unroll
        for (int r = 0; r < TH_FRAMES; r++)
            pre[r] = y2[(size_t)min(f0 + r, nframes - 1) * frame_size + s];
    };

    int hist[8] = {0, 0, 0, 0, 0, 0, 0, 0};
    float av = 0.0f, mx = 0.0f;
    const float fc = (float)cycles;
    int j = 0;
    const float *row = reinterpret_cast<const float *>(&tile[fl][0]) + comp;
    fetch(0);
    for (int t = 0; t < ntiles; t++) {
#pragma unroll
        for (int r = 0; r < TH_FRAMES; r++)
            tile[r][lane] = pre[r];
        if (t + 1 < ntiles) fetch(t + 1);
        __syncthreads();
        if (scanning) {
            const int cnt = min(TH_TILE, frame_size - t * TH_TILE);
            auto symbol_end = [&]() {
                av = av / fc;
                if (av > mx) mx = av;
                const float hv = mx / 8.0f;
                int k = 8;
#pragma unroll
                for (int q = 7; q >= 1; q--)
                    if (av <= hv * (float)q) k = q;
#pragma unroll
                for (int q = 1; q < 8; q++)
                    hist[q] += (q == k) ? 1 : 0;
            };
            if (cycles == 8 && cnt == TH_TILE && j == 0) {
#pragma unroll 2
                for (int sy = 0; sy < TH_TILE / 8; sy++) {
                    float v[8];
#pragma unroll
                    for (int u = 0; u < 8; u++) v[u] = row[2 * (sy * 8 + u)];
#pragma unroll
                    for (int u = 0; u < 8; u++) av += fabsf(v[u]);
                    symbol_end();
                }
            } else if (cycles == 4 && cnt == TH_TILE && j == 0) {
#pragma unroll 2
                for (int sy = 0; sy < TH_TILE / 4; sy++) {
                    float v[4];
#pragma unroll
                    for (int u = 0; u < 4; u++) v[u] = row[2 * (sy * 4 + u)];
#pragma unroll
                    for (int u = 0; u < 4; u++) av += fabsf(v[u]);
                    symbol_end();
                }
            } else {
                for (int i = 0; i < cnt; i++) {
                    av += fabsf(row[2 * i]);
                    if (++j == cycles) {
                        j = 0;
                        symbol_end();
                    }
                }
            }
        }
        __syncthreads();
    }
    int hmax = 0, best = 0;
#pragma unroll
    for (int q = 0; q < 8; q++) {
        const int h = hist[q] + __shfl_xor(hist[q], 1);
        if (h > hmax) { hmax = h; best = q; }
        if (hist_out && scanning && comp == 0) hist_out[(size_t)(f0 + fl) * 8 + q] = h;
    }
    if (scanning && comp == 0)
        index[f0 + fl] = best;
}

constexpr int TH8_FRAMES = 4;
constexpr int TH8_TILE = 128;
constexpr int TH8_PITCH = TH8_TILE + 4;

__global__ void __launch_bounds__(64)
timing_hist8_kernel(const float *__restrict__ y, int nframes, int frame_size, int32_t *index, int32_t *hist_out)
{
    __shared__ __attribute__((aligned(16))) float tile[2][TH8_FRAMES][TH8_PITCH];
    const int lane = threadIdx.x;
    const int f0 = blockIdx.x * TH8_FRAMES;
    const int ntiles = frame_size / TH8_TILE;

    const float4 *y4 = reinterpret_cast<const float4 *>(y);
    float4 pre[TH8_FRAMES];
    auto fetch = [&](int t) {
#pragma unroll
        for (int r = 0; r < TH8_FRAMES; r++)
            pre[r] = y4[((size_t)min(f0 + r, nframes - 1) * frame_size + (size_t)t * TH8_TILE) / 2 + lane];
    };

    const int fl = lane >> 4, comp = (lane >> 3) & 1, q = lane & 7;
    const float qf = (float)q;
    const float4 *row = reinterpret_cast<const float4 *>(&tile[comp][fl][0]);
    float av = 0.0f, mx = 0.0f;
    int cum = 0;

    fetch(0);
    for (int t = 0; t < ntiles; t++) {
        __syncthreads();
#pragma unroll
        for (int r = 0; r < TH8_FRAMES; r++) {
            *reinterpret_cast<float2 *>(&tile[0][r][2 * lane]) = make_float2(pre[r].x, pre[r].z);
            *reinterpret_cast<float2 *>(&tile[1][r][2 * lane]) = make_float2(pre[r].y, pre[r].w);
        }
        if (t + 1 < ntiles) fetch(t + 1);
        __syncthreads();
#pragma unroll 4
        for (int s = 0; s < TH8_TILE / 8; s++) {
            const float4 a = row[2 * s], b = row[2 * s + 1];
            av += fabsf(a.x); av += fabsf(a.y); av += fabsf(a.z); av += fabsf(a.w);
            av += fabsf(b.x); av += fabsf(b.y); av += fabsf(b.z); av += fabsf(b.w);
            av *= 0.125f;
            if (av > mx) mx = av;
            const float th = (mx * 0.125f) * qf;
            cum += (av <= th) ? 0 : 1;
        }
    }
    if (q == 0) cum = frame_size / 8;
    int h = __shfl_up(cum, 1) - cum;
    if (q == 0) h = 0;
    h += __shfl_xor(h, 8);
    int hmax = 0, best = 0;
#pragma unroll
    for (int k = 0; k < 8; k++) {
        const int hk = __shfl(h, (lane & ~7) + k);
        if (hk > hmax) { hmax = hk; best = k; }
    }
    if (f0 + fl < nframes && comp == 0) {
        if (hist_out) hist_out[(size_t)(f0 + fl) * 8 + q] = h;
        if (q == 0) index[f0 + fl] = best;
    }
}

__global__ void __launch_bounds__(64)
costas_kernel(const float2 *__restrict__ d, int nframes, int nsym, int dstride, int nbw, const float *__restrict__ gains,
              float min_freq, float max_freq, const float *state_in, float *state_out, uint8_t *sym,
              float2 *costas, int *status)
{
    const int t = blockIdx.x * 64 + threadIdx.x;
    if (t >= nframes * nbw) return;
    const int f = t / nbw, b = t - f * nbw;
    Loop st = {0.0f, 0.0f};
    if (state_in) { st.phase = state_in[2 * t]; st.freq = state_in[2 * t + 1]; }
    const LoopGains lg = {gains[2 * b], gains[2 * b + 1], min_freq, max_freq};
    bool over = false;
    const float2 *p = d + (size_t)f * dstride;
    for (int i = 0; i < nsym; i++) {
        const float2 z = i == 0 ? costas_step<true>(st, lg, p[i], over) : costas_step<false>(st, lg, p[i], over);
        if (sym) sym[(size_t)t * nsym + i] = (uint8_t)slicer(z);
        if (costas) costas[(size_t)t * nsym + i] = z;
    }
    if (state_out) { state_out[2 * t] = st.phase; state_out[2 * t + 1] = st.freq; }
    if (over && status) __hip_atomic_store(status, STATUS_PHASE_RANGE, __ATOMIC_RELAXED, __HIP_MEMORY_SCOPE_SYSTEM);
    else if (status && !loop_state_finite(st.phase, st.freq))
        __hip_atomic_store(status, STATUS_NONFINITE, __ATOMIC_RELAXED, __HIP_MEMORY_SCOPE_SYSTEM);
}

__global__ void __launch_bounds__(256)
decimate_kernel(const float2 *__restrict__ filtered, const int32_t *__restrict__ index, float2 *dec,
                int nstreams, int frame_size, int cycles, int nsym)
{
    const int i = blockIdx.x * 256 + threadIdx.x, f = blockIdx.y;
    if (i >= nsym) return;
    float2 *row = dec + (size_t)f * nsym;
    const int src = i * cycles + index[f];
    row[i] = src < frame_size ? filtered[(size_t)f * frame_size + src] : make_float2(0.0f, 0.0f);
}

constexpr int MX_STREAMS = 16;
constexpr int MX_TILE = 128;

__global__ void __launch_bounds__(64)
mixer_kernel(const int16_t *__restrict__ pcm, float2 *__restrict__ out, float *state, int nstreams, int frame_size)
{
    __shared__ __attribute__((aligned(16))) float2 ph[MX_STREAMS][MX_TILE + 2];
    const int lane = threadIdx.x, f0 = blockIdx.x * MX_STREAMS;
    const bool scanning = lane < MX_STREAMS && f0 + lane < nstreams;
    const int f = min(f0 + (lane & (MX_STREAMS - 1)), nstreams - 1);
    float2 p = make_float2(state[4 * f], state[4 * f + 1]);
    const float rr = state[4 * f + 2], ri = state[4 * f + 3];
    const int ntiles = (frame_size + MX_TILE - 1) / MX_TILE;

    const bool fast = f0 + MX_STREAMS <= nstreams && (frame_size & 1) == 0 &&
                      (reinterpret_cast<uintptr_t>(pcm) & 3) == 0 && (reinterpret_cast<uintptr_t>(out) & 15) == 0;
    uint32_t pre[MX_STREAMS];
    auto fetch = [&](int t) {
#pragma unroll
        for (int r = 0; r < MX_STREAMS; r++) {
            const int16_t *rowp = pcm + (size_t)(f0 + r) * frame_size + (size_t)t * MX_TILE;
            pre[r] = reinterpret_cast<const uint32_t *>(rowp)[lane];
        }
    };
    float nri = -ri;
    asm volatile("" : "+v"(nri));
    auto step = [&]() {
        const float2 a = make_float2(p.x * rr, p.y * rr);
        const float2 b = make_float2(p.y * nri, p.x * ri);
        p = make_float2(a.x + b.x, a.y + b.y);
    };
    if (fast && frame_size >= MX_TILE) fetch(0);
    for (int t = 0; t < ntiles; t++) {
        const int cnt = min(MX_TILE, frame_size - t * MX_TILE);
        __syncthreads();
        if (scanning) {
            float4 *prow = reinterpret_cast<float4 *>(&ph[lane][0]);
            if (cnt == MX_TILE) {
#pragma unroll 8
                for (int i = 0; i < MX_TILE / 2; i++) {
                    step();
                    const float2 p0 = p;
                    step();
                    prow[i] = make_float4(p0.x, p0.y, p.x, p.y);
                }
            } else {
                for (int i = 0; i < cnt; i++) {
                    step();
                    ph[lane][i] = p;
                }
            }
        }
        __syncthreads();
        if (fast && cnt == MX_TILE) {
            float4 c[MX_STREAMS];
#pragma unroll
            for (int r = 0; r < MX_STREAMS; r++)
                c[r] = *reinterpret_cast<const float4 *>(&ph[r][2 * lane]);
#pragma unroll
            for (int r = 0; r < MX_STREAMS; r++) {
                float2 *orow = out + (size_t)(f0 + r) * frame_size + (size_t)t * MX_TILE;
                const float v0 = (float)(int16_t)(pre[r] & 0xffffu) / 16384.0f;
                const float v1 = (float)(int16_t)(pre[r] >> 16) / 16384.0f;
                reinterpret_cast<float4 *>(orow)[lane] =
                    make_float4(c[r].x * v0, c[r].y * v0, c[r].z * v1, c[r].w * v1);
            }
            if ((t + 2) * MX_TILE <= frame_size) fetch(t + 1);
        } else {
            for (int i = lane; i < cnt; i += 64) {
#pragma unroll 1
                for (int r = 0; r < MX_STREAMS && f0 + r < nstreams; r++) {
                    const size_t at = (size_t)(f0 + r) * frame_size + (size_t)t * MX_TILE + i;
                    const float v = (float)pcm[at] / 16384.0f;
                    const float2 c = ph[r][i];
                    out[at] = make_float2(c.x * v, c.y * v);
                }
            }
        }
    }
    const float pr = p.x, pi = p.y;
    if (scanning) {
        const float mag = (float)sqrt((double)pr * (double)pr + (double)pi * (double)pi);
        state[4 * f] = pr / mag;
        state[4 * f + 1] = pi / mag;
    }
}

__global__ void __launch_bounds__(256)
fft_kernel(const double2 *__restrict__ in, double2 *__restrict__ out, const double2 *__restrict__ tw, int n,
           int log2n, int inverse)
{
    extern __shared__ __attribute__((aligned(16))) unsigned char smem[];
    double2 *v = reinterpret_cast<double2 *>(smem);
    const int tid = threadIdx.x;
    const double2 *src = in + (size_t)blockIdx.x * n;
    double2 *dst = out + (size_t)blockIdx.x * n;
    for (int i = tid; i < n; i += blockDim.x) {
        const int r = (int)(__brev((unsigned)i) >> (32 - log2n));
        v[r] = src[i];
    }
    __syncthreads();
    fft_lds_stages(v, tw, n, log2n, tid, (int)blockDim.x, inverse ? 1.0 : -1.0);
    const double dn = (double)n;
    for (int i = tid; i < n; i += blockDim.x) {
        double2 r = v[i];
        if (!inverse) { r.x = r.x / dn; r.y = r.y / dn; }
        dst[i] = r;
    }
}

__global__ void fill_i32_kernel(int32_t *p, int n, int32_t v)
{
    const int i = blockIdx.x * blockDim.x + threadIdx.x;
    if (i < n) p[i] = v;
}

__global__ void sincos_hash_kernel(uint32_t first, uint32_t count, unsigned long long *acc)
{
    unsigned long long h = 0;
    for (uint32_t i = blockIdx.x * blockDim.x + threadIdx.x; i < count; i += gridDim.x * blockDim.x) {
        const uint32_t u = first + i;
        for (int sg = 0; sg < 2; sg++) {
            const float y = __uint_as_float(u | ((uint32_t)sg << 31));
            const SinCos r = sincos_f32(y);
            unsigned long long v = ((unsigned long long)__float_as_uint(r.s) << 32) | __float_as_uint(r.c);
            v ^= (unsigned long long)(u | ((uint32_t)sg << 31)) * 0x9E3779B97F4A7C15ull;
            v *= 0xD6E8FEB86659FD93ull;
            v ^= v >> 32;
            h += v;
        }
    }
    atomicAdd(acc, h);
}

#define LAUNCH_CHECK()                          \
    do {                                        \
        hipError_t e_ = hipGetLastError();      \
        if (e_ != hipSuccess) return (int)e_;   \
    } while (0)

int launch_rx_fused(const FusedArgs &a, hipStream_t s)
{
    if (a.est_tw) return (int)hipErrorInvalidValue;
    const int blocks = (a.nframes + a.G - 1) / a.G;
    const size_t lds = fused_lds_bytes(a.G, a.S, a.cycles, a.nbw);
    hipLaunchKernelGGL(rx_fused_kernel, dim3(blocks), dim3(FUSED_THREADS), lds, s, a);
    LAUNCH_CHECK();
    return 0;
}

__global__ void fft_big_first_kernel(const double2 *__restrict__ in, double2 *__restrict__ out, const double2 *__restrict__ twb,
                                     int n, int log2n, int inverse);
__global__ void fft_big_late_kernel(double2 *__restrict__ data, const double2 *__restrict__ twn, int n, int log2n, int inverse);

int prepare_kernels(void)
{
    hipError_t e = hipFuncSetAttribute(reinterpret_cast<const void *>(rx_fused_kernel),
                                       hipFuncAttributeMaxDynamicSharedMemorySize, MAX_LDS_BYTES);
    if (e != hipSuccess) return (int)e;
    e = hipFuncSetAttribute(reinterpret_cast<const void *>(fft_big_first_kernel), hipFuncAttributeMaxDynamicSharedMemorySize,
                            MAX_LDS_BYTES);
    if (e != hipSuccess) return (int)e;
    e = hipFuncSetAttribute(reinterpret_cast<const void *>(fft_big_late_kernel), hipFuncAttributeMaxDynamicSharedMemorySize,
                            MAX_LDS_BYTES);
    if (e != hipSuccess) return (int)e;
    e = hipFuncSetAttribute(reinterpret_cast<const void *>(fft_kernel),
                            hipFuncAttributeMaxDynamicSharedMemorySize, MAX_LDS_BYTES);
    return (int)e;
}

int launch_rrc_fir(const float *x, const float *memory, float *y, const float *taps, int nframes, int length,
                   hipStream_t s, size_t in_pitch)
{
    dim3 grid((length + FIR_TILE - 1) / FIR_TILE, nframes);
    hipLaunchKernelGGL(rrc_fir_kernel, grid, dim3(FIR_THREADS), 0, s, reinterpret_cast<const float2 *>(x),
                       reinterpret_cast<const float2 *>(memory), reinterpret_cast<float2 *>(y), taps, length,
                       in_pitch ? in_pitch : (size_t)length);
    LAUNCH_CHECK();
    return 0;
}

int launch_delay_line(const float *x, float *memory, int nframes, int length, hipStream_t s)
{
    hipLaunchKernelGGL(delay_line_kernel, dim3(nframes), dim3(128), 0, s, reinterpret_cast<const float2 *>(x),
                       reinterpret_cast<float2 *>(memory), length);
    LAUNCH_CHECK();
    return 0;
}

int launch_timing_hist(const float *y, int nframes, int frame_size, int cycles, int32_t *index, int32_t *hist,
                       bool generic, hipStream_t s)
{
    if (cycles == 8 && frame_size % TH8_TILE == 0 && (reinterpret_cast<uintptr_t>(y) & 15) == 0 && !generic) {
        hipLaunchKernelGGL(timing_hist8_kernel, dim3((nframes + TH8_FRAMES - 1) / TH8_FRAMES), dim3(64), 0, s, y,
                           nframes, frame_size, index, hist);
        LAUNCH_CHECK();
        return 0;
    }
    hipLaunchKernelGGL(timing_hist_kernel, dim3((nframes + TH_FRAMES - 1) / TH_FRAMES), dim3(64), 0, s, y, nframes,
                       frame_size, cycles, index, hist);
    LAUNCH_CHECK();
    return 0;
}

int launch_costas(const float *d, int nframes, int nsym, int dstride, int nbw, const float *gains, float min_freq,
                  float max_freq, const float *state_in, float *state_out, uint8_t *sym, float *costas, int *status,
                  hipStream_t s)
{
    const int threads = nframes * nbw;
    hipLaunchKernelGGL(costas_kernel, dim3((threads + 63) / 64), dim3(64), 0, s,
                       reinterpret_cast<const float2 *>(d), nframes, nsym, dstride, nbw, gains, min_freq, max_freq,
                       state_in, state_out, sym, reinterpret_cast<float2 *>(costas), status);
    LAUNCH_CHECK();
    return 0;
}

int launch_decimate(const float *filtered, const int32_t *index, float *dec, int nstreams, int frame_size,
                    int cycles, int nsym, hipStream_t s)
{
    dim3 grid((nsym + 255) / 256, nstreams);
    hipLaunchKernelGGL(decimate_kernel, grid, dim3(256), 0, s, reinterpret_cast<const float2 *>(filtered), index,
                       reinterpret_cast<float2 *>(dec), nstreams, frame_size, cycles, nsym);
    LAUNCH_CHECK();
    return 0;
}

int launch_mixer(const int16_t *pcm, float *out, float *state, int nstreams, int frame_size, hipStream_t s)
{
    hipLaunchKernelGGL(mixer_kernel, dim3((nstreams + MX_STREAMS - 1) / MX_STREAMS), dim3(64), 0, s, pcm,
                       reinterpret_cast<float2 *>(out), state, nstreams, frame_size);
    LAUNCH_CHECK();
    return 0;
}

constexpr int FFTB_LOG2 = 12, FFTB = 1 << FFTB_LOG2, FFTB_COLS = 16, FFTB_THREADS = 256;

__global__ void __launch_bounds__(FFTB_THREADS)
fft_big_first_kernel(const double2 *__restrict__ in, double2 *__restrict__ out, const double2 *__restrict__ twb, int n,
                     int log2n, int inverse)
{
    extern __shared__ __attribute__((aligned(16))) unsigned char smem[];
    double2 *v = reinterpret_cast<double2 *>(smem);
    const int tid = threadIdx.x;
    const double2 *src = in + (size_t)blockIdx.y * n;
    double2 *dst = out + (size_t)blockIdx.y * n;
    const int base = blockIdx.x * FFTB;
    for (int i = tid; i < FFTB; i += FFTB_THREADS)
        v[i] = src[__brev((unsigned)(base + i)) >> (32 - log2n)];
    __syncthreads();
    fft_lds_stages(v, twb, FFTB, FFTB_LOG2, tid, FFTB_THREADS, inverse ? 1.0 : -1.0);
    for (int i = tid; i < FFTB; i += FFTB_THREADS)
        dst[base + i] = v[i];
}

__global__ void __launch_bounds__(FFTB_THREADS)
fft_big_late_kernel(double2 *__restrict__ data, const double2 *__restrict__ twn, int n, int log2n, int inverse)
{
    extern __shared__ __attribute__((aligned(16))) unsigned char smem[];
    double2 *t = reinterpret_cast<double2 *>(smem);
    const int tid = threadIdx.x;
    const int rows = n >> FFTB_LOG2, lrows = log2n - FFTB_LOG2;
    const int c0 = blockIdx.x * FFTB_COLS;
    double2 *d = data + (size_t)blockIdx.y * n;
    for (int e = tid; e < rows * FFTB_COLS; e += FFTB_THREADS)
        t[e] = d[(size_t)(e / FFTB_COLS) * FFTB + c0 + (e % FFTB_COLS)];
    __syncthreads();
    const double sgn = inverse ? 1.0 : -1.0;
    for (int st = 1; st <= lrows; st++) {
        const int h = 1 << (st - 1);
        const int stride = n >> (FFTB_LOG2 + st);
        for (int b = tid; b < (rows / 2) * FFTB_COLS; b += FFTB_THREADS) {
            const int rr = b / FFTB_COLS, c = b % FFTB_COLS;
            const int kr = rr & (h - 1);
            const int lo = (((rr >> (st - 1)) << st) + kr) * FFTB_COLS + c, hi = lo + h * FFTB_COLS;
            const double2 w = twn[(size_t)(kr * FFTB + c0 + c) * stride];
            const double wr = w.x, wi = sgn * w.y;
            const double2 e = t[lo], o = t[hi];
            const double zr = wr * o.x - wi * o.y;
            const double zi = wr * o.y + wi * o.x;
            t[lo] = make_double2(e.x + zr, e.y + zi);
            t[hi] = make_double2(e.x - zr, e.y - zi);
        }
        __syncthreads();
    }
    const double dn = (double)n;
    for (int e = tid; e < rows * FFTB_COLS; e += FFTB_THREADS) {
        double2 r = t[e];
        if (!inverse) { r.x = r.x / dn; r.y = r.y / dn; }
        d[(size_t)(e / FFTB_COLS) * FFTB + c0 + (e % FFTB_COLS)] = r;
    }
}

int fft_lds_max_n(void) { return 8192; }
int fft_big_block(void) { return FFTB; }

int launch_fft_big(const double *in, double *out, const double *twb, const double *twn, int nbatch, int n, int log2n,
                   int inverse, hipStream_t s)
{
    const int rows = n >> FFTB_LOG2;
    if (n <= FFTB || rows * FFTB_COLS * (int)sizeof(double2) > MAX_LDS_BYTES || in == out) return (int)hipErrorInvalidValue;
    hipLaunchKernelGGL(fft_big_first_kernel, dim3(n / FFTB, nbatch), dim3(FFTB_THREADS), sizeof(double2) * (size_t)FFTB, s,
                       reinterpret_cast<const double2 *>(in), reinterpret_cast<double2 *>(out),
                       reinterpret_cast<const double2 *>(twb), n, log2n, inverse);
    LAUNCH_CHECK();
    hipLaunchKernelGGL(fft_big_late_kernel, dim3(FFTB / FFTB_COLS, nbatch), dim3(FFTB_THREADS),
                       sizeof(double2) * (size_t)rows * FFTB_COLS, s, reinterpret_cast<double2 *>(out),
                       reinterpret_cast<const double2 *>(twn), n, log2n, inverse);
    LAUNCH_CHECK();
    return 0;
}

int launch_fft(const double *in, double *out, const double *tw, int nbatch, int n, int log2n, int inverse,
               hipStream_t s)
{
    const int threads = n / 2 < 256 ? (n / 2 < 64 ? 64 : n / 2) : 256;
    hipLaunchKernelGGL(fft_kernel, dim3(nbatch), dim3(threads), sizeof(double2) * (size_t)n, s,
                       reinterpret_cast<const double2 *>(in), reinterpret_cast<double2 *>(out),
                       reinterpret_cast<const double2 *>(tw), n, log2n, inverse);
    LAUNCH_CHECK();
    return 0;
}

int launch_fill_i32(int32_t *p, int n, int32_t v, hipStream_t s)
{
    hipLaunchKernelGGL(fill_i32_kernel, dim3((n + 255) / 256), dim3(256), 0, s, p, n, v);
    LAUNCH_CHECK();
    return 0;
}

int launch_sincos_hash(uint32_t first, uint32_t count, unsigned long long *acc, hipStream_t s)
{
    hipLaunchKernelGGL(sincos_hash_kernel, dim3(2048), dim3(256), 0, s, first, count, acc);
    LAUNCH_CHECK();
    return 0;
}

}
```

qpsk_amd/csrc/rx_fused.hip:

```cpp
#include <hip/hip_runtime.h>
#include <stdint.h>
#include "qpsk_device.h"
#include "costas_asm.h"
#include "costas_asm_lo.h"
#include "fir_full8s_asm.h"
#include "fir_r2_asm.h"
#include "fir_r4_asm.h"
#include "fir_lean_asm.h"
#include "fir_lean_data_asm.h"
#include "fir_full8_asm.h"
#include "timing_fft_wave.h"
#include "carrier.h"
#ifdef QPSK_PIPE_PROFILE
#include "fir_lean_prof_asm.h"
#endif
#include "kernels.h"

#ifndef QPSK_PIPE1_ASM
#define QPSK_PIPE1_ASM 1
#endif

namespace qpsk {

static_assert(FIR_R2_ASM_END_VGPR <= 168, "rx_pipe2_kernel: three FIR waves per SIMD");
static_assert(FIR_R4_ASM_END_VGPR <= 256, "rx_fused_pipe_kernel: two waves per SIMD");

namespace pipe {

constexpr int C = 8;
constexpr int DR = 2;
constexpr int MAX_WAVES = 16;
constexpr int SPIN_LIMIT = 1 << 24;

#ifdef QPSK_PIPE_PROFILE
#define QPSK_ABLATE(a, bit) (((a).dbg & (bit)) != 0)
#else
#define QPSK_ABLATE(a, bit) false
#endif

template <int QL_, int R_, int MAX_NF_, int SPARE_, bool PINNED_>
struct Geom {
    static constexpr bool PINNED = PINNED_;
    static constexpr int QL = QL_;
    static constexpr int R = R_;
    static constexpr int MAX_NF = MAX_NF_;
    static constexpr int SPARE = SPARE_;
    static constexpr int FWV = 64 / QL;
    static constexpr int S = R * QL;
    static constexpr int CH = S * C;
    static constexpr int TSTEPS = NTAPS + C * (R - 1);
    static constexpr int PAD = R * C;
    static constexpr int WL = CH + 128;
    static constexpr int WSLOTS = ((WL + 2 * (WL / (2 * C)) + 31) / 32) * 32;
    static constexpr int DSTRIDE = DR * S + 2;
    static constexpr int ZSTRIDE = DR * S + 4;
    static constexpr int MAX_THREADS = SPARE ? 512 : 64 * (MAX_NF + 1);
    static_assert(QL == 16 && 64 % QL == 0 && 128 % PAD == 0, "slot arithmetic assumes 16 lanes per frame");
};
template <int QL_, int R_>
struct WaveMap {
    static constexpr int QL = QL_, R = R_;
};
using GeomNarrow = Geom<16, 4, 4, 1, true>;

#define QPSK_GEOM_CONSTANTS(GM)                                                                          \
    constexpr int QL = GM::QL, R = GM::R, FWV = GM::FWV, S = GM::S, CH = GM::CH, WSLOTS = GM::WSLOTS,    \
                  DSTRIDE = GM::DSTRIDE, ZSTRIDE = GM::ZSTRIDE, TSTEPS = GM::TSTEPS, PAD = GM::PAD,      \
                  MAX_NF = GM::MAX_NF;                                                                   \
    (void)QL; (void)R; (void)FWV; (void)S; (void)CH; (void)WSLOTS; (void)DSTRIDE; (void)ZSTRIDE;         \
    (void)TSTEPS; (void)PAD; (void)MAX_NF

#ifdef QPSK_PIPE_PROFILE
__device__ unsigned long long g_timeline[1024 * 48];
#define QPSK_TL_STAMP(SLOT) do { if ((a.dbg & 8388608) && lane == 0 && blockIdx.x < 1024) { unsigned long long t_; asm volatile("s_memrealtime %0\n\ts_waitcnt lgkmcnt(0)" : "=s"(t_)::"memory"); g_timeline[48 * blockIdx.x + (SLOT)] = t_; } } while (0)
#endif
struct Smem {
    float taps[128];
    int ready[MAX_WAVES];
    int consumed;
    int abort_flag;
    int pad_[2];
    int est_index[16];
};

__device__ __forceinline__ int ld_acquire(const int *p)
{
    int v = __hip_atomic_load(p, __ATOMIC_RELAXED, __HIP_MEMORY_SCOPE_WORKGROUP);
    __builtin_amdgcn_fence(__ATOMIC_ACQUIRE, "workgroup");
    return v;
}

__device__ __forceinline__ void st_release(int *p, int v)
{
    __builtin_amdgcn_fence(__ATOMIC_RELEASE, "workgroup");
    __hip_atomic_store(p, v, __ATOMIC_RELAXED, __HIP_MEMORY_SCOPE_WORKGROUP);
}

__device__ __forceinline__ void report_status(int *status, int what)
{
    __hip_atomic_store(status, what, __ATOMIC_RELAXED, __HIP_MEMORY_SCOPE_SYSTEM);
}

__device__ __forceinline__ bool wait_ge(int *p, int target, int *abort_flag)
{
    int spins = 0;
    while (ld_acquire(p) < target) {
        __builtin_amdgcn_s_sleep(2);
        if (++spins > SPIN_LIMIT || __hip_atomic_load(abort_flag, __ATOMIC_RELAXED, __HIP_MEMORY_SCOPE_WORKGROUP)) {
            __hip_atomic_store(abort_flag, 1, __ATOMIC_RELAXED, __HIP_MEMORY_SCOPE_WORKGROUP);
            return false;
        }
    }
    return true;
}

}

using namespace pipe;

struct StreamHi {
    template <class... A> static __device__ __forceinline__ void ring(A &&...a) { costas_asm_run_ring(a...); }
    template <class... A> static __device__ __forceinline__ void ring_pair(A &&...a) { costas_asm_run_ring_pair(a...); }
    template <class... A> static __device__ __forceinline__ unsigned run(A &&...a) { return costas_asm_run(a...); }
};
struct StreamLo {
    template <class... A> static __device__ __forceinline__ void ring(A &&...a) { costas_asm_run_ring_lo(a...); }
    template <class... A> static __device__ __forceinline__ void ring_pair(A &&...a) { costas_asm_run_ring_pair_lo(a...); }
    template <class... A> static __device__ __forceinline__ unsigned run(A &&...a) { return costas_asm_run_lo(a...); }
};

template <class GM, class ST = StreamHi, class SM>
__device__ __forceinline__ void costas_wave(const FusedArgs &a, SM *sm, const float2 *dring, float *zring, int G,
                                            int f0, int lane, int nchunks, int *status)
{
    QPSK_GEOM_CONSTANTS(GM);
    const int nbw = a.nbw, N = a.nsym;
    if (a.share_simd0 != ((a.dbg & 512) != 0)) __builtin_amdgcn_s_setprio(1);
    else __builtin_amdgcn_s_setprio(3);
    const bool pair = a.lean_pair != 0;
    const bool odd = pair && (lane & 1);
    const int g = pair ? lane >> 1 : lane / nbw, b = pair ? 0 : lane - g * nbw;
    const bool inwg = pair ? lane < 2 * G : lane < G * nbw;
    const bool active = inwg && f0 + g < a.nframes;
    Loop st = {0.0f, 0.0f};
    LoopGains lg = {0.0f, 0.0f, a.min_freq, a.max_freq};
    bool over = false;
    if (active) {
        lg.alpha = a.gains[2 * b];
        lg.beta = a.gains[2 * b + 1];
        if (a.state_in) {
            st.phase = a.state_in[2 * ((size_t)(f0 + g) * nbw + b)];
            st.freq = a.state_in[2 * ((size_t)(f0 + g) * nbw + b) + 1];
            if (a.seed_setters) seed_setters(st.phase, st.freq, a.min_freq, a.max_freq, over);
        }
    }
    const int gl = inwg ? g : 0;
    const int gw = a.mixed == 2 ? gl / 2 : a.mixed == 1 && gl >= 12 ? 3 + (gl - 12) / 2 : gl / FWV;
    const float2 *dl = dring + (size_t)gl * DSTRIDE;
    float *zl = zring + (size_t)(pair ? gl : lane) * ZSTRIDE;
    const bool fast_clamp = a.min_freq < 0.0f && a.max_freq > 0.0f;
    float ph = st.phase, fr = st.freq;
    auto zero_run = [&](int from, int to) {
        const uint4 *p = reinterpret_cast<const uint4 *>(dl + from);
        unsigned acc = 0;
        for (int i = 0; i < (to - from) / 2; i++) {
            const uint4 v = p[i];
            acc |= v.x | v.y | v.z | v.w;
        }
        return acc == 0u;
    };
    auto excusable = [&](unsigned long long lanes, int from, int to) {
        const bool z = ((lanes >> lane) & 1ull) != 0ull && __float_as_uint(ph) != 0x80000000u && __float_as_uint(fr) != 0x80000000u &&
                       zero_run(from, to);
        return (unsigned long long)__ballot(z);
    };
    const float al = lg.alpha, be = lg.beta, fmin_ = a.min_freq, fmax_ = a.max_freq;
    bool ok = true;
#ifdef QPSK_PIPE_PROFILE
    const bool cprof = (a.dbg & 32) && blockIdx.x == 0;
    unsigned long long cw = 0, cs = 0, ct = 0;
    auto ctick = [&](unsigned long long &acc) {
        if (cprof) {
            unsigned long long t;
            asm volatile("s_memtime %0\n\ts_waitcnt lgkmcnt(0)" : "=s"(t)::"memory");
            acc += t - ct;
            ct = t;
        }
    };
    unsigned long long dummy = 0;
    ctick(dummy);
#endif
#ifdef QPSK_PIPE_PROFILE
    const bool timeline = (a.dbg & 8388608) != 0;
    const bool ring_prof = (a.dbg & 4096) != 0 && (blockIdx.x == 0 || blockIdx.x == 77 || timeline);
    unsigned long long rp_in = 0, rp_out = 0, rp_t = 0, rp_calls = 0, rp_rt0 = 0, rp_rt1 = 0, rp_rt2 = 0;
    auto rp_real = [&]() {
        unsigned long long t = 0;
        if (ring_prof) asm volatile("s_memrealtime %0\n\ts_waitcnt lgkmcnt(0)" : "=s"(t)::"memory");
        return t;
    };
    rp_rt0 = rp_real();
    auto rp_tick = [&](unsigned long long &acc) {
        if (ring_prof) {
            unsigned long long t;
            asm volatile("s_memtime %0\n\ts_waitcnt lgkmcnt(0)" : "=s"(t)::"memory");
            if (rp_t) acc += t - rp_t;
            rp_t = t;
        }
    };
    const bool ring_stream = fast_clamp && !(a.dbg & (2 | 8 | 16 | ((a.dbg & 4096) ? 0 : 32))) && S == 4 * COSTAS_ASM_GROUP && DR == 2;
#else
    const bool ring_stream = fast_clamp && !(a.dbg & (8 | 16)) && S == 4 * COSTAS_ASM_GROUP && DR == 2;
#endif
    const int first_ring_chunk = __any(active && __float_as_uint(ph) == 0x80000000u) ? 1 : 0;
    for (int c = 0; c < nchunks && ok; c++) {
        if (ring_stream && c >= first_ring_chunk && (c + 1) * S <= N) {
            const int cfull = N / S;
            if (active) {
                constexpr int AG = COSTAS_ASM_GROUP;
                unsigned k = 4u * (unsigned)c;
                const unsigned kend = 4u * (unsigned)cfull;
                const unsigned d_base = lds_addr(dl), z_base = lds_addr(zl);
                const unsigned ready_addr = lds_addr(&sm->ready[gw]), consumed_addr = lds_addr(&sm->consumed);
                unsigned long long ign = 0ull;
                while (k < kend) {
                    if ((k & 3u) == 0u) {
                        ok = wait_ge(&sm->ready[gw], (int)(k >> 2) + 1, &sm->abort_flag);
                        if (!__all(ok)) { ok = false; break; }
                        if (ign) {
                            const int at = (int)(k & 7u) * AG;
                            ign = excusable(ign, at, at + S);
                        }
                    }
                    unsigned long long fl = 0ull;
                    bool ran = false;
                    if (!__any(__float_as_uint(fr) == 0x80000000u)) {
                        unsigned ks = __builtin_amdgcn_readfirstlane(k);
                        const unsigned kstop = ign ? min(kend, (ks | 3u) + 1u) : kend;
#ifdef QPSK_PIPE_PROFILE
                        rp_tick(rp_out);
                        if (rp_calls++ == 0) rp_rt1 = rp_real();
#endif
                        if (pair)
                            ST::ring_pair(ph, fr, d_base, z_base, ready_addr, consumed_addr, ks, kstop, al, be, fmin_, fmax_, odd, fl, ign);
                        else
                            ST::ring(ph, fr, d_base, z_base, ready_addr, consumed_addr, ks, kstop, al, be, fmin_, fmax_, fl, ign);
                        ran = true;
#ifdef QPSK_PIPE_PROFILE
                        rp_tick(rp_in);
                        rp_rt2 = rp_real();
#endif
                        k = ks;
                    }
                    if ((!ran || fl != 0ull) && k < kend) {
                        const int at = (int)(k & 7u) * AG;
                        const unsigned long long fresh = fl & ~ign;
                        if (ran && fresh) {
                            const unsigned long long zm = excusable(fresh, at, ((int)(k & 7u) | 3) * AG + AG);
                            if ((fresh & ~zm) == 0ull) { ign |= zm; continue; }
                        }
                        for (int i = 0; i < AG; i++) {
                            float tx, ty; unsigned qq;
                            zl[at + i] = ph;
                            costas_step_t<true>(ph, fr, al, be, fmin_, fmax_, dl[at + i], tx, ty, qq, over);
                        }
                        k++;
                        if ((k & 3u) == 0u && lane == 0) st_release(&sm->consumed, (int)(k >> 2));
                    }
                }
            }
            ok = __all(ok);
            c = cfull - 1;
            continue;
        }
        ok = wait_ge(&sm->ready[gw], c + 1, &sm->abort_flag);
        if (!__all(ok)) { ok = false; break; }
#ifdef QPSK_PIPE_PROFILE
        {
            const unsigned long long before = cw;
            ctick(cw);
            if (cprof && lane == 0 && (a.dbg & 2048) && (c < 4 || c % 8 == 0)) printf("  serial wave: chunk %d waited %llu cycles\n", c, cw - before);
        }
#endif
        const int slot = (c % DR) * S;
        const int cnt = min(S, N - c * S);
        if (active && !QPSK_ABLATE(a, 2)) {
            int j = 0;
            if (c == 0) {
                Loop s0 = {ph, fr};
                zl[slot] = ph;
                costas_step<true>(s0, lg, dl[slot], over);
                ph = s0.phase; fr = s0.freq;
                j = 1;
                for (; j < min(4, cnt); j++) {
                    float tx, ty; unsigned qq;
                    zl[slot + j] = ph;
                    if (fast_clamp) costas_step_t<true>(ph, fr, al, be, fmin_, fmax_, dl[slot + j], tx, ty, qq, over);
                    else costas_step_t<false>(ph, fr, al, be, fmin_, fmax_, dl[slot + j], tx, ty, qq, over);
                }
            }
            if (fast_clamp && !(a.dbg & 8)) {
                constexpr int AG = COSTAS_ASM_GROUP;
                unsigned long long ign = 0ull;
                while (cnt - j >= AG) {
                    unsigned da = lds_addr(dl + slot + j), za = lds_addr(zl + slot + j);
                    unsigned long long fl = 0ull;
                    bool ran = false;
                    const unsigned want = __builtin_amdgcn_readfirstlane((unsigned)(cnt - j) / AG);
                    unsigned left = want;
                    if (!__any(__float_as_uint(fr) == 0x80000000u)) {
                        left = ST::run(ph, fr, da, za, want, al, be, fmin_, fmax_, fl, ign);
                        ran = true;
                    }
                    j += AG * (int)(want - left);
                    if (left != 0) {
                        const unsigned long long fresh = fl & ~ign;
                        if (ran && fresh) {
                            const unsigned long long zm = excusable(fresh, slot + j, slot + j + AG * (int)left);
                            if ((fresh & ~zm) == 0ull) { ign |= zm; continue; }
                        }
                        for (int i = 0; i < AG; i++, j++) {
                            float tx, ty; unsigned qq;
                            zl[slot + j] = ph;
                            costas_step_t<true>(ph, fr, al, be, fmin_, fmax_, dl[slot + j], tx, ty, qq, over);
                        }
                    }
                }
            }
            float2 dcur = dl[slot + j];
            if (fast_clamp) {
#pragma unroll 1
                for (; j < cnt; j++) {
                    const float2 dnext = dl[slot + j + 1];
                    float tx, ty; unsigned qq;
                    zl[slot + j] = ph;
                    costas_step_t<true>(ph, fr, al, be, fmin_, fmax_, dcur, tx, ty, qq, over);
                    dcur = dnext;
                }
            } else {
#pragma unroll 4
                for (; j < cnt; j++) {
                    const float2 dnext = dl[slot + j + 1];
                    float tx, ty; unsigned qq;
                    zl[slot + j] = ph;
                    costas_step_t<false>(ph, fr, al, be, fmin_, fmax_, dcur, tx, ty, qq, over);
                    dcur = dnext;
                }
            }
        }
        if (lane == 0) st_release(&sm->consumed, c + 1);
#ifdef QPSK_PIPE_PROFILE
        ctick(cs);
#endif
    }
#ifdef QPSK_PIPE_PROFILE
    if (cprof && lane == 0 && !ring_prof)
        printf("serial wave: %d chunks; cycles per chunk: wait for the FIR waves %llu, steps %llu\n", nchunks, cw / nchunks, cs / nchunks);
    if (timeline) {
        if (lane == 0 && blockIdx.x < 1024) {
            unsigned long long *tl = g_timeline + 48 * blockIdx.x;
            tl[1] = rp_rt0; tl[2] = rp_rt1; tl[3] = rp_rt2; tl[4] = rp_real();
        }
    } else if (ring_prof && lane == 0)
        printf("wg %3d serial wave: %d chunks, %llu entries into the stream; cycles per chunk inside the stream %llu (= %llu per step), "
               "outside it (waiting for the FIR waves, redone groups) %llu; wall time (100 MHz clock): wave start -> first step %.2f us, "
               "first -> last step %.2f us\n", (int)blockIdx.x, nchunks, rp_calls, rp_in / nchunks,
               rp_in / nchunks / S, rp_out / nchunks, (double)(rp_rt1 - rp_rt0) * 0.01, (double)(rp_rt2 - rp_rt1) * 0.01);
#endif
    st.phase = ph; st.freq = fr;
    if (active && ok && !odd) {
        const size_t o = (size_t)(f0 + g) * nbw + b;
        if (a.freq) a.freq[o] = st.freq;
        if (a.phase) a.phase[o] = st.phase;
        if (a.hz) a.hz[o] = (float)((double)st.freq * a.rs / TAU);
        if (a.state_out) { a.state_out[2 * o] = st.phase; a.state_out[2 * o + 1] = st.freq; }
    }
    if (!ok && lane == 0) report_status(status, STATUS_PIPE_TIMEOUT);
    if (over) report_status(status, STATUS_PHASE_RANGE);
    else if (active && ok && !loop_state_finite(ph, fr)) report_status(status, STATUS_NONFINITE);
}

template <class GM, int RW = GM::R, bool DATA = false>
__device__ __forceinline__ void flush_records(const FusedArgs &a, const float *zring, const float2 *dring, int g, int frame,
                                              int q, int chunk, uint8_t *sym_row = nullptr)
{
    constexpr int DSTRIDE = GM::DSTRIDE;
    constexpr int R = RW, S = GM::S, ZSTRIDE = GM::ZSTRIDE;
    static_assert(R == 2 || R == 4, "packs 2 or 4 symbols per store");
    const int nbw = a.nbw, N = a.nsym;
    const int slot = (chunk % DR) * S, sym0 = chunk * S;
    const int cnt = min(S, N - sym0);
    for (int b = 0; b < nbw; b++) {
        const int row = g * nbw + b;
        const size_t o = ((size_t)frame * nbw + b) * N + sym0 + R * q;
        float2 z[R];
        uint32_t packed = 0;
        float phv[R];
        float2 dv[R];
        {
            const float *zp = zring + (size_t)row * ZSTRIDE + slot + R * q;
            const float2 *dp = dring + (size_t)g * DSTRIDE + slot + R * q;
            if constexpr (R == 4) {
                const float4 p4 = *reinterpret_cast<const float4 *>(zp);
                const float4 da = reinterpret_cast<const float4 *>(dp)[0], db = reinterpret_cast<const float4 *>(dp)[1];
                phv[0] = p4.x; phv[1] = p4.y; phv[2] = p4.z; phv[3] = p4.w;
                dv[0] = make_float2(da.x, da.y); dv[1] = make_float2(da.z, da.w);
                dv[2] = make_float2(db.x, db.y); dv[3] = make_float2(db.z, db.w);
            } else {
                const float2 p2 = *reinterpret_cast<const float2 *>(zp);
                const float4 da = *reinterpret_cast<const float4 *>(dp);
                phv[0] = p2.x; phv[1] = p2.y;
                dv[0] = make_float2(da.x, da.y); dv[1] = make_float2(da.z, da.w);
            }
        }
#pragma unroll
        for (int r = 0; r < R; r++)
            z[r] = derotate<false>(phv[r], dv[r]);
        if (chunk == 0 && q == 0)
            z[0] = derotate<true>(phv[0], dv[0]);
#pragma unroll
        for (int r = 0; r < R; r++)
            packed |= (uint32_t)(DATA ? data_rule(z[r]) : slicer(z[r])) << (8 * r);
        if (a.sym) {
            uint8_t *so = sym_row ? sym_row + sym0 + R * q : a.sym + o;
            if (R * q + R <= cnt && ((N | sym0) & (R - 1)) == 0) {
                if constexpr (R == 4) *reinterpret_cast<uint32_t *>(so) = packed;
                else *reinterpret_cast<uint16_t *>(so) = (uint16_t)packed;
            } else {
                for (int r = 0; r < R; r++)
                    if (R * q + r < cnt) so[r] = (uint8_t)(packed >> (8 * r));
            }
        }
        if (a.costas) {
            for (int r = 0; r < R; r++)
                if (R * q + r < cnt) a.costas[o + r] = z[r];
        }
    }
}

__global__ void __launch_bounds__(64 * (GeomNarrow::MAX_NF + 2))
costas_pipe_kernel(FusedArgs a, int *status)
{
    using GM = GeomNarrow;
    QPSK_GEOM_CONSTANTS(GM);
    static_assert(R == 2 || R == 4, "flush_records packs 2 or 4 symbols per store");
    extern __shared__ __attribute__((aligned(16))) unsigned char smem_raw[];
    Smem *sm = reinterpret_cast<Smem *>(smem_raw);
    const int NF = (int)blockDim.x / 64 - 1 - (a.carrier_state ? 1 : 0);
    const int G = NF * FWV;
    float2 *dring = reinterpret_cast<float2 *>(smem_raw + sizeof(Smem));
    float *zring = reinterpret_cast<float *>(dring + (size_t)G * DSTRIDE);
    const int tid = threadIdx.x, wave = tid >> 6, lane = tid & 63;
    const int N = a.nsym;
    const int f0 = blockIdx.x * G;
    const int nchunks = (N + S - 1) / S;
    if (tid < MAX_WAVES) sm->ready[tid] = 0;
    if (tid == 0) { sm->consumed = 0; sm->abort_flag = 0; }
    __syncthreads();

    if (wave == 0) {
        costas_wave<GM>(a, sm, dring, zring, G, f0, lane, nchunks, status);
        return;
    }
    if (wave == NF + 1) {
        if (blockIdx.x == 0 && lane == 0)
            carrier_block(a.carrier_state, a.carrier_tab, a.carrier_frame, carrier_split(a.carrier_frame), a.carrier_frame / 2);
        return;
    }
    const int w = wave - 1;
    const int fl = lane / QL, q = lane % QL;
    const int g = w * FWV + fl;
    const int frame = f0 + g;
    const bool fvalid = frame < a.nframes;
    const float2 *src = a.dsrc + (size_t)(fvalid ? frame : 0) * a.dstride;
    int flushed = 0;
    bool ok = true;
    float2 pre[R];
    auto fetch = [&](int c) {
#pragma unroll
        for (int r = 0; r < R; r++)
            pre[r] = src[min(c * S + R * q + r, N - 1)];
    };
    fetch(0);
    for (int c = 0; c < nchunks; c++) {
        if (c >= DR) {
            ok = wait_ge(&sm->consumed, c - DR + 1, &sm->abort_flag);
            if (!ok) break;
            for (; flushed < c - DR + 1; flushed++)
                if (fvalid) flush_records<GM>(a, zring, dring, g, frame, q, flushed);
        }
        float2 *dw = dring + (size_t)g * DSTRIDE + (c % DR) * S + R * q;
#pragma unroll
        for (int r = 0; r < R; r++)
            dw[r] = pre[r];
        if (c + 1 < nchunks) fetch(c + 1);
        if (lane == 0) st_release(&sm->ready[w], c + 1);
        if (a.refill && fvalid) {
            const float2 *blk = a.refill + (size_t)frame * a.frame_size;
            float2 *row = a.refill_dst + (size_t)frame * a.dstride;
            const int ix = checked_index(a.index ? a.index[frame] : a.fixed_index, a.status);
#pragma unroll
            for (int r = 0; r < R; r++) {
                const int i = c * S + R * q + r, s = i * a.cycles + ix;
                if (i < N) {
                    if (a.refill_planar) {
                        const int pl = ix % a.cycles, sy = i + ix / a.cycles;
                        row[i] = sy < N ? blk[(size_t)pl * N + sy] : make_float2(0.0f, 0.0f);
                    } else {
                        row[i] = s < a.frame_size ? blk[s] : make_float2(0.0f, 0.0f);
                    }
                }
            }
        }
    }
    if (ok) {
        ok = wait_ge(&sm->consumed, nchunks, &sm->abort_flag);
        if (ok)
            for (; flushed < nchunks; flushed++)
                if (fvalid) flush_records<GM>(a, zring, dring, g, frame, q, flushed);
    }
    if (!ok && lane == 0) report_status(status, STATUS_PIPE_TIMEOUT);
}

template <class GM>
__global__ void __launch_bounds__(GM::MAX_THREADS)
rx_fused_pipe_kernel(FusedArgs a, int *status)
{
    QPSK_GEOM_CONSTANTS(GM);
    extern __shared__ __attribute__((aligned(16))) unsigned char smem_raw[];
    Smem *sm = reinterpret_cast<Smem *>(smem_raw);
    const bool spares = GM::SPARE && !(a.dbg & 4);
    const int nwaves = (int)blockDim.x / 64;
    const bool mixed = a.mixed != 0;
    const int nfir = spares ? (nwaves - 1) - (nwaves - 1) / 4 : nwaves - 1;
    const int G = a.mixed == 1 ? 4 * FWV : a.mixed == 2 ? 2 * nfir : nfir * FWV;
    float2 *win = reinterpret_cast<float2 *>(smem_raw + sizeof(Smem));
    float2 *dring = win + (size_t)G * WSLOTS;
    float *zring = reinterpret_cast<float *>(dring + (size_t)G * DSTRIDE);

    const int tid = threadIdx.x, lane = tid & 63;
    const int wave = __builtin_amdgcn_readfirstlane(tid >> 6);
    const int L = a.frame_size, N = a.nsym;
    const int f0 = blockIdx.x * G;
    const int nchunks = (N + S - 1) / S;

    for (int i = tid; i < 128; i += blockDim.x)
        sm->taps[i] = i < NTAPS ? a.taps[i] : 0.0f;
    if (tid < MAX_WAVES) sm->ready[tid] = 0;
    if (tid == 0) { sm->consumed = 0; sm->abort_flag = 0; }
    __syncthreads();

    if (a.est_tw) {
        float2 *ewin = win + (size_t)wave * tfft::WSLOTS;
        const unsigned erd = lds_addr(ewin + (tfft::R + tfft::PADS) * lane), etap = lds_addr(sm->taps);
        const int fe0 = f0 + 2 * wave;
        const float2 *srcA = a.x + (size_t)min(fe0, a.nframes - 1) * a.frame_pitch;
        const float2 *srcB = a.x + (size_t)min(fe0 + 1, a.nframes - 1) * a.frame_pitch;
        tfft::Pre5 pre = tfft::load_frame5(srcA, lane);
#pragma unroll
        for (int i = 0; i < 2; i++) {
            tfft::stage_frame5(ewin, lane, pre);
            if (i == 0) pre = tfft::load_frame5(srcB, lane);
            tfft::wave_sync();
            v2f e0, e1, e2, e3, e4, e5, e6, e7;
            fir_full8_asm(erd, etap, e0, e1, e2, e3, e4, e5, e6, e7);
            const v2f eacc[tfft::R] = {e0, e1, e2, e3, e4, e5, e6, e7};
            double epv[tfft::R];
            const tfft::cd u = tfft::power_bin(eacc, ewin, lane, a.est_tw, tfft::NFFT / C, nullptr, epv);
            if (lane == 0 && fe0 + i < a.nframes) {
                const int best = tfft::pick_index(u, a.est_cs, C, nullptr);
                sm->est_index[2 * wave + i] = best;
                if (a.index_out) a.index_out[fe0 + i] = best;
            }
        }
        __syncthreads();
    }

    if (wave == 0) {
        costas_wave<GM>(a, sm, dring, zring, G, f0, lane, nchunks, status);
        return;
    }

    int w, gbase, rslot;
    bool half = false;
    if (a.mixed == 2) {
        if (spares && (wave & 3) == 0) return;
        w = spares ? wave - 1 - wave / 4 : wave - 1;
        half = true;
        gbase = 2 * w;
        rslot = w;
    } else if (mixed) {
        if (wave >= 4 && wave <= 5) return;
        half = wave >= 6;
        w = half ? wave - 3 : wave - 1;
        gbase = half ? 12 + 2 * (wave - 6) : 4 * (wave - 1);
        rslot = w;
    } else {
        if (spares && (wave & 3) == 0) return;
        w = spares ? wave - 1 - wave / 4 : wave - 1;
        gbase = w * GM::FWV;
        rslot = w;
    }

  auto fir_wave = [&](auto wmap) {
    constexpr int PADS = 2;
    constexpr int QL = decltype(wmap)::QL, R = decltype(wmap)::R, FWV = 64 / QL, PAD = R * C,
                  TSTEPS = NTAPS + C * (R - 1);
    static_assert(QL * R == S && 128 % PAD == 0 && PAD >= 2 * C, "chunk size and window padding are the workgroup's");
    const int fl = lane / QL, q = lane % QL;

    const float4 *taps4 = reinterpret_cast<const float4 *>(sm->taps);
    constexpr int NLD = CH / 128;

    struct Ctx {
        int group, g, frame;
        bool fvalid, all_valid;
        float2 *wf;
        const float2 *rd;
        int wr0[FWV], wr1[FWV];
        bool even[FWV];
        bool h0[FWV], h1[FWV];
        float4 hist[FWV];
        const float4 *src[FWV];
        bool fv[FWV];
    };
    auto make_ctx = [&]() {
        Ctx cx;
        cx.group = rslot;
        cx.g = gbase + fl;
        cx.frame = f0 + cx.g;
        cx.fvalid = cx.frame < a.nframes;
        cx.all_valid = f0 + gbase + FWV <= a.nframes;
        cx.wf = win + (size_t)cx.g * WSLOTS;
        cx.rd = cx.wf + (PAD + PADS) * q;
#pragma unroll
        for (int ff = 0; ff < FWV; ff++) {
            const int fr = f0 + gbase + ff;
            cx.fv[ff] = fr < a.nframes;
            const int ix = a.est_tw ? (cx.fv[ff] ? sm->est_index[gbase + ff] : 0)
                                    : checked_index(a.index ? (cx.fv[ff] ? a.index[fr] : 0) : a.fixed_index, a.status);
            const int p0 = 2 * lane + 126 - ix;
            cx.wr0[ff] = (gbase + ff) * WSLOTS + p0 + PADS * (p0 / PAD);
            cx.wr1[ff] = (gbase + ff) * WSLOTS + (p0 + 1) + PADS * ((p0 + 1) / PAD);
            cx.even[ff] = (ix & 1) == 0;
            cx.h0[ff] = p0 >= 128;
            cx.h1[ff] = p0 + 1 >= 128;
            cx.hist[ff] = make_float4(0.0f, 0.0f, 0.0f, 0.0f);
            cx.src[ff] = reinterpret_cast<const float4 *>(a.x + (size_t)(cx.fv[ff] ? fr : 0) * a.frame_pitch);
        }
        return cx;
    };

    auto prefetch = [&](const Ctx &cx, float4 (&pre)[FWV][NLD], int c) {
        if (cx.all_valid && (c + 1) * CH <= L) {
#pragma unroll
            for (int ff = 0; ff < FWV; ff++)
#pragma unroll
                for (int j = 0; j < NLD; j++)
                    pre[ff][j] = load_once(&cx.src[ff][(c * CH + 128 * j + 2 * lane) >> 1]);
        } else {
#pragma unroll
            for (int ff = 0; ff < FWV; ff++) {
#pragma unroll
                for (int j = 0; j < NLD; j++) {
                    const int s = c * CH + 128 * j + 2 * lane;
                    const bool in = cx.fv[ff] && s + 1 < L;
                    float4 v = load_once(&cx.src[ff][in ? (s >> 1) : 0]);
                    if (!in) v = make_float4(0.0f, 0.0f, 0.0f, 0.0f);
                    pre[ff][j] = v;
                }
            }
        }
    };

#ifdef QPSK_PIPE_PROFILE
    const bool prof = (a.dbg & 32) && blockIdx.x == 0;
    unsigned long long tacc[5] = {0, 0, 0, 0, 0}, tlast = 0;
    auto tick = [&](int k) {
        if (prof) {
            unsigned long long t;
            asm volatile("s_memtime %0\n\ts_waitcnt lgkmcnt(0)" : "=s"(t)::"memory");
            if (k >= 0) tacc[k] += t - tlast;
// ... 466 lines not shown
    if (mine == 0) return;
    int u0 = 0, widx = 0;
    for (int v = 1; v < wave; v++) {
        const int cv = (int)((layout >> (4 * v)) & 15);
        u0 += cv;
        widx += cv != 0;
    }
    float2 *mywin = win + (size_t)widx * UF * WS;
    if (mine == 2)
        fir_wave2<2>(a, sm, mywin, dring, zring, G, widx, u0, f0, lane, nchunks, status);
    else
        fir_wave2<1>(a, sm, mywin, dring, zring, G, widx, u0, f0, lane, nchunks, status);
}

size_t pipe2_lds_bytes(int G, int nwin, int nbw)
{
    using GM = GeomNarrow;
    size_t b = sizeof(Smem) + sizeof(float2) * ((size_t)nwin * pipe2::UF * pipe2::WS + (size_t)G * GM::DSTRIDE) +
               sizeof(float) * (size_t)G * nbw * GM::ZSTRIDE;
    return (b + 15) & ~(size_t)15;
}

int pipe2_max_fir(void) { return pipe2::MAX_FIR; }
int pipe2_max_frames(void) { return pipe2::UF * pipe2::MAX_UNITS; }
int pipe2_max_units_per_wave(void) { return pipe2::MAX_UW; }
int pipe2_max_hw_waves(void) { return pipe2::MAX_THREADS / 64; }

unsigned long long pipe2_default_layout(int NU)
{
    using namespace pipe2;
    int cnt[16] = {0};
    const int hwmax = MAX_THREADS / 64;
    const bool share = NU > 8 && MAX_UW == 2;
    int left = NU;
    for (int round = 0; round < MAX_UW && left > 0; round++)
        for (int w = 1; w < hwmax && left > 0; w++) {
            if ((w & 3) == 0 && !(share && w == 4)) continue;
            if (share && (w == 11 || (round == 1 && w > 7))) continue;
            cnt[w]++;
            left--;
        }
    unsigned long long layout = 0;
    for (int w = 1; w < hwmax; w++) layout |= (unsigned long long)cnt[w] << (4 * w);
    return left == 0 ? layout : 0;
}

int launch_rx_pipe2(const FusedArgs &a0, int G, unsigned long long layout, int *status, hipStream_t s)
{
    using namespace pipe2;
    if (a0.est_tw) return (int)hipErrorInvalidValue;
    FusedArgs a = a0;
    const int NU = (G + UF - 1) / UF;
    int units = 0, nwin = 0, hw = 1;
    for (int w = 1; w < 16; w++) {
        const int cw = (int)((layout >> (4 * w)) & 15);
        if (cw > MAX_UW || (cw && w >= MAX_THREADS / 64)) return (int)hipErrorInvalidValue;
        units += cw;
        nwin += cw != 0;
        if (cw) hw = w + 1;
    }
    if (G < 1 || G > UF * MAX_UNITS || G * a.nbw > 64 || units != NU || (layout & 15) ||
        pipe2_lds_bytes(G, nwin, a.nbw) > (size_t)MAX_LDS_BYTES)
        return (int)hipErrorInvalidValue;
    a.G = G;
    a.lean_pair = 0;
    a.mixed = 2;
    a.share_simd0 = ((layout >> 16) & 15) != 0 || ((layout >> 32) & 15) != 0;
    const int blocks = (a.nframes + G - 1) / G;
    hipLaunchKernelGGL(rx_pipe2_kernel, dim3(blocks), dim3(64 * hw), pipe2_lds_bytes(G, nwin, a.nbw), s, a, layout, nwin, status);
    return (int)hipGetLastError();
}

namespace lean {
constexpr int PRM_DWORDS = 20;
constexpr int HW_WAVES = pipe2::MAX_THREADS / 64;
constexpr int WS = WS_LEAN_SLOTS;
struct Ctl {
    int ready[MAX_WAVES];
    int consumed;
    int abort_flag;
    int pad_[2];
};
struct GeomLean : GeomNarrow {
    static constexpr int DSTRIDE = 194;
    static constexpr int ZSTRIDE = 388;
};
constexpr int ROW_BYTES = 1552, Z_OFFSET_BYTES = 1024;
static_assert(GeomLean::DSTRIDE * 8 == ROW_BYTES && GeomLean::ZSTRIDE * 4 == ROW_BYTES &&
              Z_OFFSET_BYTES == DR * GeomNarrow::S * 8 && Z_OFFSET_BYTES + DR * GeomNarrow::S * 4 <= ROW_BYTES &&
              ROW_BYTES % 16 == 0 && (ROW_BYTES / 4) % 64 == 4, "ring rows: symbols, records, bank spread");
static_assert(sizeof(Ctl) % 16 == 0 && offsetof(Ctl, ready) == 0 && offsetof(Ctl, consumed) == 64 &&
              offsetof(Ctl, abort_flag) == 68, "fir_lean_asm.h addresses the counters by these offsets");
static_assert(PRM_DWORDS * 4 <= ROW_BYTES - Z_OFFSET_BYTES, "a parameter block fits the record half of a row");
static_assert(FIR_LEAN_END_VGPR <= 168, "three waves per SIMD");
static_assert(FIR_LEAN_WOFF == sizeof(float2) * pipe2::UF * WS, "fir_lean_loop2_dma2w: unit 1's window follows unit 0's");
static_assert(WS % 2 == 0 && pipe2::slot_of(pipe2::PAD * (pipe2::QL - 1) + pipe2::TSTEPS - 1) < WS &&
              pipe2::slot_of(pipe2::CH + HIST - 1) < WS + 16, "window: every position a lane reads, and a frame's spill stays in the next frame's history slots");
__device__ __host__ constexpr int rows_of(int G) { return G > HW_WAVES ? G : HW_WAVES; }
}
constexpr size_t LEAN_EST_LDS_BYTES = 128 * sizeof(float) + 32 * sizeof(int);

__device__ __forceinline__ uint8_t *lean_unit_rows(const FusedArgs &a, int f0, int u)
{
    const int fa = f0 + pipe2::UF * u;
    return fa + pipe2::UF <= a.nframes ? a.sym + (size_t)fa * a.nsym : a.sym_pad + (size_t)(pipe2::UF * u) * a.nsym;
}

template <int NUW>
__device__ __forceinline__ void lean_dma_table(unsigned *tab, float2 *mywin, unsigned ixpack, bool two_windows, int lane)
{
    using namespace pipe2;
    constexpr int WS = lean::WS;
#pragma unroll
    for (int ui = 0; ui < NUW; ui++)
#pragma unroll
        for (int ff = 0; ff < UF; ff++) {
            const int k = 2 * ui + ff;
            const int ix = (int)((ixpack >> (4 * k)) & 15u);
            const int S0 = slot_of(HIST - ix);
            for (int j = 0; j < 4; j++) {
                const int sl = S0 + 2 * (64 * j + lane);
                const int grp = sl / (PAD + PADS);
                int r = sl % (PAD + PADS);
                if (r >= PAD) r = PAD - 2;
                int n = PAD * grp + r - HIST + ix;
                if (n > CH - 2) n = CH - 2;
                tab[(4 * k + j) * 64 + lane] = 8u * (unsigned)n;
            }
            tab[(16 + k) * 64 + lane] = lds_addr(mywin + ((two_windows && ui == 1) ? UF * WS : 0) + ff * WS + S0);
        }
}

template <int NUW, bool DATA>
__device__ __forceinline__ void fir_wave_lean(const FusedArgs &a, lean::Ctl *sm, unsigned char *rows, float2 *mywin,
                                              int hwave, int u0, int f0, int lane, int nchunks, int *status, const int *est)
{
    using namespace pipe2;
    using GM = lean::GeomLean;
    constexpr int WS = lean::WS;
    float2 *dring = reinterpret_cast<float2 *>(rows);
    float *zring = reinterpret_cast<float *>(rows + lean::Z_OFFSET_BYTES);
    const int N = a.nsym;
    const int fl = lane / QL, q = lane % QL;
    const bool simd0 = (hwave & 3) == 0;
    unsigned *prm = reinterpret_cast<unsigned *>(rows + (size_t)hwave * lean::ROW_BYTES + lean::Z_OFFSET_BYTES);
    unsigned ixpack = ((unsigned)(4 * u0) << 16) | (simd0 && !(a.dbg & 1024) ? 0x80000000u : 0u);
#pragma unroll
    for (int ui = 0; ui < NUW; ui++)
#pragma unroll
        for (int ff = 0; ff < UF; ff++) {
            const int fr = f0 + UF * (u0 + ui) + ff;
            const int ix = checked_index(__builtin_amdgcn_readfirstlane(est ? est[UF * (u0 + ui) + ff] : a.index ? a.index[min(fr, a.nframes - 1)] : a.fixed_index), status);
            ixpack |= (unsigned)ix << (4 * (2 * ui + ff));
        }
    const bool use_dma = a.lean_dma && (ixpack & 0x1111u) == 0;
    const bool two_windows = NUW == 2 && a.lean_twowin && use_dma;
    LeanLaneAddr w;
#pragma unroll
    for (int ui = 0; ui < 2; ui++) {
        const int u = u0 + (ui < NUW ? ui : 0);
#pragma unroll
        for (int ff = 0; ff < UF; ff++) {
            const int fr = f0 + UF * u + ff;
            const int ix = (int)((ixpack >> (4 * (2 * (ui < NUW ? ui : 0) + ff))) & 7u);
            const int p0 = 2 * lane + HIST - ix;
            const int wu = (two_windows && ui == 1) ? UF * WS : 0;
            w.wr0[ui][ff] = lds_addr(mywin + wu + ff * WS + slot_of(p0)) - 8u * BLK;
            w.wr1[ui][ff] = lds_addr(mywin + wu + ff * WS + slot_of(p0 + 1)) - 8u * BLK;
            if (lane == 0) {
                size_t fsrc = (size_t)min(fr, a.nframes - 1);
#ifdef QPSK_PIPE_PROFILE
                if (a.dbg & 2097152) fsrc = (size_t)(UF * u + ff) * gridDim.x + blockIdx.x;
#endif
                unsigned long long src = (unsigned long long)(a.x + fsrc * a.frame_pitch);
#ifdef QPSK_PIPE_PROFILE
                if (a.dbg & 4194304) src = (unsigned long long)(a.x + (size_t)f0 * a.frame_pitch) + (unsigned long long)(UF * u + ff) * 4096ull;
#endif
                prm[4 * ui + 2 * ff] = (unsigned)src;
                prm[4 * ui + 2 * ff + 1] = (unsigned)(src >> 32);
            }
        }
        const int g = UF * u + fl;
        w.ring[ui] = lds_addr(dring + (size_t)g * GM::DSTRIDE + R * q);
        w.z[ui] = lds_addr(zring + (size_t)g * GM::ZSTRIDE + R * q);
        if (lane == 0) {
            const unsigned long long sb = (unsigned long long)lean_unit_rows(a, f0, u);
            prm[8 + 2 * ui] = (unsigned)sb;
            prm[8 + 2 * ui + 1] = (unsigned)(sb >> 32);
        }
    }
    w.wlim = lds_addr(mywin + WS + (WS - 2));
    w.wpad = lds_addr(mywin + WS + PAD);
    if (lane == 0) {
        prm[12] = (unsigned)nchunks;
        prm[13] = ixpack;
        prm[16] = (unsigned)(unsigned long long)a.taps;
        prm[17] = (unsigned)((unsigned long long)a.taps >> 32);
    }
    if (simd0 && !(a.dbg & 1024)) __builtin_amdgcn_s_setprio(3);
    const unsigned rd = lds_addr(mywin + fl * WS + (PAD + PADS) * q);
    int st;
#ifdef QPSK_PIPE_PROFILE
    if (a.dbg & 32) {
        unsigned pf[FIR_LEAN_NPROF];
        unsigned long long t0, t1;
        asm volatile("s_memtime %0\n\ts_waitcnt lgkmcnt(0)" : "=s"(t0)::"memory");
        if constexpr (NUW == 2)
            st = fir_lean_loop2_prof(lds_addr(prm), rd, 16u * lane, (unsigned)(fl * N + R * q), lds_addr(sm), w, pf);
        else
            st = fir_lean_loop1_prof(lds_addr(prm), rd, 16u * lane, (unsigned)(fl * N + R * q), lds_addr(sm), w, pf);
        asm volatile("s_memtime %0\n\ts_waitcnt lgkmcnt(0)" : "=s"(t1)::"memory");
        if ((blockIdx.x == 0 || blockIdx.x == 77) && lane == 0)
            printf("wg %3d FIR wave hw %2d (%d units): %d chunks, %llu cycles in the stream; per chunk: samples %u, stage+loads %u, "
                   "filter+gain %u, wait for the loop %u, flush %u, hand-over %u\n", (int)blockIdx.x, hwave, NUW, nchunks, t1 - t0,
                   pf[0] / nchunks, pf[1] / nchunks, pf[2] / nchunks, pf[3] / nchunks, pf[4] / nchunks, pf[5] / nchunks);
    } else if (a.dbg & (1 | 16384 | 32768 | 65536 | 262144 | 524288 | 1048576 | 4194304)) {
#define QPSK_LEAN_ABLATED(SFX)                                                                                          \
        (NUW == 2 ? fir_lean_loop2_##SFX(lds_addr(prm), rd, 16u * lane, (unsigned)(fl * N + R * q), lds_addr(sm), w)    \
                  : fir_lean_loop1_##SFX(lds_addr(prm), rd, 16u * lane, (unsigned)(fl * N + R * q), lds_addr(sm), w))
        if (a.dbg & 1) st = QPSK_LEAN_ABLATED(avalu);
        else if (a.dbg & 16384) st = QPSK_LEAN_ABLATED(alds);
        else if (a.dbg & 32768) st = QPSK_LEAN_ABLATED(aflush);
        else if (a.dbg & 65536) st = QPSK_LEAN_ABLATED(astage);
        else if (a.dbg & 262144) st = QPSK_LEAN_ABLATED(astore);
        else if (a.dbg & 524288) st = QPSK_LEAN_ABLATED(aring);
        else if (a.dbg & 4194304) st = QPSK_LEAN_ABLATED(atiled);
        else st = QPSK_LEAN_ABLATED(aorder);
#undef QPSK_LEAN_ABLATED
    } else
#endif
#ifdef QPSK_PIPE_PROFILE
    QPSK_TL_STAMP(32 + hwave);
#endif
    if constexpr (DATA) {
        unsigned *tab = reinterpret_cast<unsigned *>(mywin);
        if (use_dma) lean_dma_table<NUW>(tab, mywin, ixpack, two_windows, lane);
        if constexpr (NUW == 2) {
            if (use_dma && two_windows)
                st = fir_lean_loop2_dma2w_data(lds_addr(prm), rd, 16u * lane, (unsigned)(fl * N + R * q), lds_addr(sm), lds_addr(tab + lane), w);
            else if (use_dma)
                st = fir_lean_loop2_dma_data(lds_addr(prm), rd, 16u * lane, (unsigned)(fl * N + R * q), lds_addr(sm), lds_addr(tab + lane), w);
            else
                st = fir_lean_loop2_data(lds_addr(prm), rd, 16u * lane, (unsigned)(fl * N + R * q), lds_addr(sm), w);
        } else if (use_dma)
            st = fir_lean_loop1_dma_data(lds_addr(prm), rd, 16u * lane, (unsigned)(fl * N + R * q), lds_addr(sm), lds_addr(tab + lane), w);
        else
            st = fir_lean_loop1_data(lds_addr(prm), rd, 16u * lane, (unsigned)(fl * N + R * q), lds_addr(sm), w);
    } else if (use_dma) {
        unsigned *tab = reinterpret_cast<unsigned *>(mywin);
#pragma unroll
        for (int ui = 0; ui < NUW; ui++)
#pragma unroll
            for (int ff = 0; ff < UF; ff++) {
                const int k = 2 * ui + ff;
                const int ix = (int)((ixpack >> (4 * k)) & 15u);
                const int S0 = slot_of(HIST - ix);
                for (int j = 0; j < 4; j++) {
                    const int sl = S0 + 2 * (64 * j + lane);
                    const int grp = sl / (PAD + PADS);
                    int r = sl % (PAD + PADS);
                    if (r >= PAD) r = PAD - 2;
                    int n = PAD * grp + r - HIST + ix;
                    if (n > CH - 2) n = CH - 2;
                    tab[(4 * k + j) * 64 + lane] = 8u * (unsigned)n;
                }
                tab[(16 + k) * 64 + lane] = lds_addr(mywin + ((two_windows && ui == 1) ? UF * WS : 0) + ff * WS + S0);
            }
        if constexpr (NUW == 2) {
            if (two_windows)
                st = fir_lean_loop2_dma2w(lds_addr(prm), rd, 16u * lane, (unsigned)(fl * N + R * q), lds_addr(sm), lds_addr(tab + lane), w);
            else
                st = fir_lean_loop2_dma(lds_addr(prm), rd, 16u * lane, (unsigned)(fl * N + R * q), lds_addr(sm), lds_addr(tab + lane), w);
        } else
            st = fir_lean_loop1_dma(lds_addr(prm), rd, 16u * lane, (unsigned)(fl * N + R * q), lds_addr(sm), lds_addr(tab + lane), w);
    } else if constexpr (NUW == 2)
        st = fir_lean_loop2(lds_addr(prm), rd, 16u * lane, (unsigned)(fl * N + R * q), lds_addr(sm), w);
    else
        st = fir_lean_loop1(lds_addr(prm), rd, 16u * lane, (unsigned)(fl * N + R * q), lds_addr(sm), w);
    bool ok = st == 0;
    if (ok) {
        for (int c = nchunks - DR; c < nchunks && ok; c++) {
            ok = wait_ge(&sm->consumed, c + 1, &sm->abort_flag);
            if (ok)
#pragma unroll
                for (int ui = 0; ui < NUW; ui++) {
                    const int g = UF * (u0 + ui) + fl;
                    flush_records<GM, R, DATA>(a, zring, dring, g, f0 + g, q, c, lean_unit_rows(a, f0, u0 + ui) + (size_t)fl * N);
                }
        }
    } else if (lane == 0) {
        __hip_atomic_store(&sm->abort_flag, 1, __ATOMIC_RELAXED, __HIP_MEMORY_SCOPE_WORKGROUP);
    }
#ifdef QPSK_PIPE_PROFILE
    if ((a.dbg & 8388608) && lane == 0) {
        unsigned long long t;
        __builtin_amdgcn_s_waitcnt(0);
        asm volatile("s_memrealtime %0\n\ts_waitcnt lgkmcnt(0)" : "=s"(t)::"memory");
        if (blockIdx.x < 1024 && hwave < 11) g_timeline[48 * blockIdx.x + 5 + hwave] = t;
    }
#endif
    if (!ok && lane == 0) report_status(status, STATUS_PIPE_TIMEOUT);
}

template <bool DATA>
__global__ void __launch_bounds__(pipe2::MAX_THREADS)
rx_lean_kernel(FusedArgs a, unsigned long long layout, int nwin, int *status)
{
    using namespace pipe2;
    using GM = lean::GeomLean;
    extern __shared__ __attribute__((aligned(16))) unsigned char smem_raw[];
    lean::Ctl *sm = reinterpret_cast<lean::Ctl *>(smem_raw);
    const int G = a.G;
    float2 *win = reinterpret_cast<float2 *>(smem_raw + sizeof(lean::Ctl));
    unsigned char *rows = reinterpret_cast<unsigned char *>(win + (size_t)nwin * UF * lean::WS);
    const int tid = threadIdx.x, lane = tid & 63;
    const int wave = __builtin_amdgcn_readfirstlane(tid >> 6);
    const int f0 = blockIdx.x * G;
    const int nchunks = a.nsym / S;

#ifdef QPSK_PIPE_PROFILE
    if ((a.dbg & 8388608) && tid == 0) {
        unsigned long long t;
        asm volatile("s_memrealtime %0\n\ts_waitcnt lgkmcnt(0)" : "=s"(t)::"memory");
        if (blockIdx.x < 1024) g_timeline[48 * blockIdx.x] = t;
    }
#endif
    if (tid < MAX_WAVES) sm->ready[tid] = 0;
    if (tid == 0) { sm->consumed = 0; sm->abort_flag = 0; }
    const int *est = nullptr;
    if (a.est_tw) {
        float *etaps = reinterpret_cast<float *>(rows + (size_t)lean::rows_of(G) * lean::ROW_BYTES);
        int *eidx = reinterpret_cast<int *>(etaps + 128);
        for (int i = tid; i < 128; i += blockDim.x) etaps[i] = i < NTAPS ? a.taps[i] : 0.0f;
        __syncthreads();
        const int nw = (int)blockDim.x / 64;
        const int room = (int)((size_t)nwin * UF * lean::WS / tfft::WSLOTS);
        const int nwe = nw < room ? nw : room;
        if (wave < nwe) {
            float2 *ewin = win + (size_t)wave * tfft::WSLOTS;
            const unsigned erd = lds_addr(ewin + (tfft::R + tfft::PADS) * lane), etap = lds_addr(etaps);
            tfft::Pre5 pre = tfft::load_frame5(a.x + (size_t)min(f0 + wave, a.nframes - 1) * a.frame_pitch, lane);
            for (int fe = wave; fe < G; fe += nwe) {
                tfft::stage_frame5(ewin, lane, pre);
                if (fe + nwe < G) pre = tfft::load_frame5(a.x + (size_t)min(f0 + fe + nwe, a.nframes - 1) * a.frame_pitch, lane);
                tfft::wave_sync();
                v2f e0, e1, e2, e3, e4, e5, e6, e7;
                fir_full8_asm(erd, etap, e0, e1, e2, e3, e4, e5, e6, e7);
                const v2f eacc[tfft::R] = {e0, e1, e2, e3, e4, e5, e6, e7};
                double epv[tfft::R];
                const tfft::cd u = tfft::power_bin(eacc, ewin, lane, a.est_tw, tfft::NFFT / C, nullptr, epv);
                if (lane == 0) {
                    const int best = tfft::pick_index(u, a.est_cs, C, nullptr);
                    eidx[fe] = best;
                    if (a.index_out && f0 + fe < a.nframes) a.index_out[f0 + fe] = best;
                }
                tfft::wave_sync();
            }
        }
        est = eidx;
    }
    __syncthreads();

    if (wave == 0) {
        if (f0 + G > a.nframes) {
            bool ok = true;
            for (int u = (a.nframes - f0 + UF - 1) / UF; u < G / UF && ok; u++) ok = wait_ge(&sm->ready[u], 1, &sm->abort_flag);
            if (!ok) {
                if (lane == 0) report_status(status, STATUS_PIPE_TIMEOUT);
                return;
            }
        }
        costas_wave<GM>(a, sm, reinterpret_cast<const float2 *>(rows), reinterpret_cast<float *>(rows + lean::Z_OFFSET_BYTES), G,
                        f0, lane, nchunks, status);
        return;
    }
    const int mine = wave < 16 ? (int)((layout >> (4 * wave)) & 15) : 0;
    if (mine == 0) return;
#ifdef QPSK_PIPE_PROFILE
    QPSK_TL_STAMP(16 + wave);
#endif
    int u0 = 0, widx = 0;
    for (int v = 1; v < wave; v++) {
        const int cv = (int)((layout >> (4 * v)) & 15);
        u0 += cv;
        widx += a.lean_twowin ? cv : (cv != 0);
    }
    float2 *mywin = win + (size_t)widx * UF * lean::WS;
    if (mine == 2)
        fir_wave_lean<2, DATA>(a, sm, rows, mywin, wave, u0, f0, lane, nchunks, status, est);
    else
        fir_wave_lean<1, DATA>(a, sm, rows, mywin, wave, u0, f0, lane, nchunks, status, est);
}

size_t lean_lds_bytes(int G, int nwin)
{
    size_t b = sizeof(lean::Ctl) + sizeof(float2) * (size_t)nwin * pipe2::UF * lean::WS + (size_t)lean::rows_of(G) * lean::ROW_BYTES;
    return (b + 15) & ~(size_t)15;
}

unsigned long long lean_default_layout(int NU)
{
    if (NU == 8) {
        static const int c8[12] = {0, 2, 2, 2, 0, 1, 1, 0, 0, 0, 0, 0};
        unsigned long long l8 = 0;
        for (int w = 1; w < 12; w++) l8 |= (unsigned long long)c8[w] << (4 * w);
        return l8;
    }
    if (NU != pipe2::MAX_UNITS) return pipe2_default_layout(NU);
    static const int cnt[12] = {0, 2, 2, 2, 1, 2, 2, 2, 0, 1, 1, 1};
    unsigned long long layout = 0;
    for (int w = 1; w < 12; w++) layout |= (unsigned long long)cnt[w] << (4 * w);
    return layout;
}

bool lean_shape_ok(const FusedArgs &a, int G)
{
    return a.nbw == 1 && !a.costas && (!a.state_in || a.seed_setters) && !a.state_out && a.nsym % pipe2::S == 0 && a.nsym >= 2 * pipe2::S &&
           a.frame_size == a.nsym * C && G >= 2 && G % 2 == 0 && G <= pipe2::UF * pipe2::MAX_UNITS && a.nframes >= 1 &&
           !(a.dbg & (8 | 16));
}

struct LeanGeometry {
    bool ok;
    bool est_ok;
    int units, nwin, hw;
    int hw_est, nwe;
    bool twowin, pair;
    size_t lds, lds_est;
};

static LeanGeometry lean_geometry(const FusedArgs &a, int G, unsigned long long layout)
{
    using namespace pipe2;
    LeanGeometry g{};
    g.hw = 1;
    const LayoutCount n = layout_count(layout);
    g.units = n.units;
    g.nwin = n.nwin;
    bool valid = (layout & 15) == 0;
    for (int w = 1; w < 16; w++) {
        const int cw = (int)((layout >> (4 * w)) & 15);
        if (cw > 2 || (cw && w >= MAX_THREADS / 64)) valid = false;
        if (cw) g.hw = w + 1;
    }
    valid = valid && G >= 2 && g.units == G / UF && lean_lds_bytes(G, g.nwin) <= (size_t)MAX_LDS_BYTES;
    g.twowin = valid && a.lean_twowin && a.lean_dma && g.units > g.nwin && lean_lds_bytes(G, g.units) <= (size_t)MAX_LDS_BYTES;
    if (g.twowin) g.nwin = g.units;
    g.pair = (a.lean_pair == 2 && 2 * G <= 64) || (a.lean_pair == 1 && G <= 16) || (a.lean_pair == 3 && G <= 24);
    g.lds = lean_lds_bytes(G, g.nwin);
    {
        const int want = a.est_waves > 0 ? a.est_waves : 12;
        g.hw_est = g.hw < want ? want : g.hw;
        if (g.hw_est > MAX_THREADS / 64) g.hw_est = MAX_THREADS / 64;
    }
    const int room = (int)((size_t)g.nwin * UF * lean::WS / tfft::WSLOTS);
    g.nwe = g.hw_est < room ? g.hw_est : room;
    g.lds_est = g.lds + LEAN_EST_LDS_BYTES;
    g.ok = valid;
    g.est_ok = valid && a.frame_size >= tfft::N0 + tfft::NFFT && g.nwe >= 1 && (G + g.nwe - 1) / g.nwe <= tfft::MAX_FPW && G <= 32 &&
               g.lds_est <= (size_t)MAX_LDS_BYTES;
    return g;
}

bool lean_est_ok(const FusedArgs &a, int G, unsigned long long layout)
{
    return lean_geometry(a, G, layout).est_ok;
}

int launch_rx_lean(const FusedArgs &a0, int G, unsigned long long layout, int *status, hipStream_t s)
{
    FusedArgs a = a0;
    const LeanGeometry g = lean_geometry(a, G, layout);
    if (!g.ok || !lean_shape_ok(a, G) || (a.nframes % G != 0 && !a.sym_pad)) return (int)hipErrorInvalidValue;
    if (a.est_tw && (!g.est_ok || !a.est_cs || a.index)) return (int)hipErrorInvalidValue;
    a.G = G;
    a.mixed = 2;
    a.share_simd0 = ((layout >> 16) & 15) != 0 || ((layout >> 32) & 15) != 0;
    a.lean_twowin = g.twowin;
    a.lean_pair = g.pair;
    hipLaunchKernelGGL(a.data_rule ? rx_lean_kernel<true> : rx_lean_kernel<false>, dim3((a.nframes + G - 1) / G), dim3(64 * (a.est_tw ? g.hw_est : g.hw)), a.est_tw ? g.lds_est : g.lds, s, a,
                       layout, g.nwin, status);
    return (int)hipGetLastError();
}

template <class GM>
static int frames_of(int NF)
{
    return NF * GM::FWV;
}

template <class GM>
static size_t lds_bytes_of(int NF, int nbw)
{
    const size_t G = (size_t)frames_of<GM>(NF);
    size_t b = sizeof(Smem) + sizeof(float2) * (G * GM::WSLOTS + G * GM::DSTRIDE) + sizeof(float) * G * nbw * GM::ZSTRIDE;
    return (b + 15) & ~(size_t)15;
}

size_t pipe_lds_bytes(int NF, int nbw)
{
    return lds_bytes_of<GeomNarrow>(NF, nbw);
}

int pipe_frames(int NF) { return frames_of<GeomNarrow>(NF); }
int pipe_cycles(void) { return C; }
int pipe_max_nf(void) { return GeomNarrow::MAX_NF; }

int launch_rx_fused_pipe(const FusedArgs &a0, int NF, int *status, hipStream_t s)
{
    FusedArgs a = a0;
    a.lean_pair = 0;
    a.mixed = NF == GeomNarrow::MAX_NF && !(a.dbg & (128 | 4));
    if (!a.mixed && a.nbw > 1 && NF <= 3 && !(a.dbg & (128 | 4))) a.mixed = 2;
    const int G = pipe_frames(NF);
    const int blocks = (a.nframes + G - 1) / G;
    const size_t lds = pipe_lds_bytes(NF, a.nbw);
    if (NF < 1 || NF > pipe_max_nf() || lds > (size_t)MAX_LDS_BYTES || G * a.nbw > 64) return (int)hipErrorInvalidValue;
    if (a.est_tw && (a.mixed != 1 || !a.est_cs || a.frame_size < tfft::N0 + tfft::NFFT || a.index ||
                     (size_t)8 * tfft::WSLOTS > (size_t)G * GeomNarrow::WSLOTS))
        return (int)hipErrorInvalidValue;
    const int nfir = a.mixed == 2 ? 2 * NF : NF;
    auto nwaves = [&](int spare) { return (spare && !(a.dbg & 4)) ? nfir + 1 + (nfir - 1) / 3 : nfir + 1; };
    const dim3 threads(a.mixed == 1 ? 512 : 64 * nwaves(GeomNarrow::SPARE));
    hipLaunchKernelGGL(rx_fused_pipe_kernel<GeomNarrow>, dim3(blocks), threads, lds, s, a, status);
    hipError_t e = hipGetLastError();
    return (int)e;
}

int launch_costas_pipe(const FusedArgs &a0, int NF, int *status, hipStream_t s)
{
    using GM = GeomNarrow;
    FusedArgs a = a0;
    a.lean_pair = 0;
    const int G = NF * GM::FWV;
    const int blocks = (a.nframes + G - 1) / G;
    const size_t lds = sizeof(Smem) + sizeof(float2) * (size_t)G * GM::DSTRIDE + sizeof(float) * (size_t)G * GM::ZSTRIDE;
    hipLaunchKernelGGL(costas_pipe_kernel, dim3(blocks), dim3(64 * (NF + 1 + (a.carrier_state ? 1 : 0))), lds, s, a, status);
    return (int)hipGetLastError();
}

namespace histk {
constexpr int G = 16, NSCAN = 4, NFIR = 8, UF = 2, QL = 32, R = 8;
constexpr int TILE = QL * R;
constexpr int DRO = 2, PADS = 2, WPOS = TILE + HIST, WSF = 480, PITCH = TILE + 4;
constexpr int HW_WAVES = 14;
constexpr int THREADS = 64 * HW_WAVES;
__device__ constexpr int role_of(int hw)
{
    return hw == 0 ? 12 : hw <= 3 ? hw - 1 : hw <= 11 ? hw : hw == 13 ? 3 : -1;
}
__device__ __host__ constexpr int slot_of(int p) { return p + PADS * (p / R); }
static_assert(slot_of(WPOS - 1) < WSF && WSF % 2 == 0, "window geometry (timing_scan.hip)");
static_assert(COSTAS_ASM_LO_END_VGPR <= 128, "rx_hist_kernel: four waves on SIMD 0");
struct Ctl {
    int ready[NFIR];
    int consumed[NSCAN];
    int flushed[NSCAN];
    lean::Ctl loop;
};
}

__global__ void __launch_bounds__(histk::THREADS)
rx_hist_kernel(FusedArgs a, int32_t *index_true, const int32_t *hint, int32_t *mis_list, int32_t *mis_count, int *status)
{
    using namespace histk;
    using GM = lean::GeomLean;
    extern __shared__ __attribute__((aligned(16))) unsigned char smem_raw[];
    Ctl *sm = reinterpret_cast<Ctl *>(smem_raw);
    float2 *win = reinterpret_cast<float2 *>(smem_raw + sizeof(Ctl));
    float *ring = reinterpret_cast<float *>(win + (size_t)G * WSF);
    unsigned char *rows = reinterpret_cast<unsigned char *>(ring + (size_t)G * DRO * 2 * PITCH);
    float2 *dring = reinterpret_cast<float2 *>(rows);
    float *zring = reinterpret_cast<float *>(rows + lean::Z_OFFSET_BYTES);
    const int tid = threadIdx.x, lane = tid & 63;
    const int wave = role_of(__builtin_amdgcn_readfirstlane(tid >> 6));
    const int f0 = blockIdx.x * G;
    const int frame_size = a.frame_size, nframes = a.nframes;
    const int ntiles = frame_size / TILE, nchunks = a.nsym / pipe2::S;
    const int gi = __builtin_amdgcn_readfirstlane(hint[0]) & 7;
    int *abortf = &sm->loop.abort_flag;

    if (tid < NFIR) sm->ready[tid] = 0;
    if (tid < NSCAN) { sm->consumed[tid] = 0; sm->flushed[tid] = 0; }
    if (tid < MAX_WAVES) sm->loop.ready[tid] = 0;
    if (tid == 0) { sm->loop.consumed = 0; sm->loop.abort_flag = 0; }
    __syncthreads();

    if (wave < 0) return;
    if (wave == NSCAN + NFIR) {
        costas_wave<GM, StreamLo>(a, &sm->loop, dring, zring, G, f0, lane, nchunks, status);
        return;
    }
    if (wave < NSCAN) {
        __builtin_amdgcn_s_setprio(3);
        const int fl = lane >> 4, comp = (lane >> 3) & 1, q = lane & 7;
        const int g = 4 * wave + fl;
        const float qf = (float)q;
        float av = 0.0f, mx = 0.0f;
        int cum = 0, done = 0;
        bool ok = true;
        auto serve_flush = [&]() {
            const int cons = __builtin_amdgcn_readfirstlane(ld_acquire(&sm->loop.consumed));
            while (done < cons && done < nchunks) {
                if (f0 + g < nframes) flush_records<GM, 4>(a, zring, dring, g, f0 + g, lane & 15, done);
                done++;
                if (lane == 0) st_release(&sm->flushed[wave], done);
            }
        };
        for (int t = 0; t < ntiles && ok; t++) {
            int spins = 0;
            while (!__all(ld_acquire(&sm->ready[g >> 1]) >= t + 1)) {
                serve_flush();
                __builtin_amdgcn_s_sleep(2);
                if (++spins > SPIN_LIMIT || __hip_atomic_load(abortf, __ATOMIC_RELAXED, __HIP_MEMORY_SCOPE_WORKGROUP)) {
                    __hip_atomic_store(abortf, 1, __ATOMIC_RELAXED, __HIP_MEMORY_SCOPE_WORKGROUP);
                    ok = false;
                    break;
                }
            }
            if (!ok) break;
            const float4 *row = reinterpret_cast<const float4 *>(ring + ((size_t)(g * DRO + (t % DRO)) * 2 + comp) * PITCH);
#pragma unroll 4
            for (int sidx = 0; sidx < TILE / 8; sidx++) {
                const float4 va = row[2 * sidx], vb = row[2 * sidx + 1];
                av += fabsf(va.x); av += fabsf(va.y); av += fabsf(va.z); av += fabsf(va.w);
                av += fabsf(vb.x); av += fabsf(vb.y); av += fabsf(vb.z); av += fabsf(vb.w);
                av *= 0.125f;
                if (av > mx) mx = av;
                const float th = (mx * 0.125f) * qf;
                cum += (av <= th) ? 0 : 1;
            }
            if (lane == 0) st_release(&sm->consumed[wave], t + 1);
            serve_flush();
        }
        while (ok && done < nchunks) {
            ok = wait_ge(&sm->loop.consumed, done + 1, abortf);
            if (ok) serve_flush();
        }
        if (!ok) {
            if (lane == 0) report_status(status, STATUS_PIPE_TIMEOUT);
            return;
        }
        if (q == 0) cum = frame_size / 8;
        int h = __shfl_up(cum, 1) - cum;
        if (q == 0) h = 0;
        h += __shfl_xor(h, 8);
        int hmax = 0, best = 0;
#pragma unroll
        for (int k = 0; k < 8; k++) {
            const int hk = __shfl(h, (lane & ~7) + k);
            if (hk > hmax) { hmax = hk; best = k; }
        }
        if (f0 + g < nframes && comp == 0 && q == 0) {
            index_true[f0 + g] = best;
            if (best != gi) mis_list[atomicAdd(mis_count, 1)] = f0 + g;
        }
        return;
    }

    const int w = wave - NSCAN;
    const int fl = lane / QL, q = lane % QL;
    const int g = UF * w + fl;
    const bool fv[UF] = {f0 + UF * w < nframes, f0 + UF * w + 1 < nframes};
    const float4 *src[UF];
#pragma unroll
    for (int ff = 0; ff < UF; ff++)
        src[ff] = reinterpret_cast<const float4 *>(a.x + (size_t)(fv[ff] ? f0 + UF * w + ff : 0) * a.frame_pitch);
    float2 *mywin = win + (size_t)(UF * w) * WSF;
    const unsigned rd_addr = lds_addr(mywin + fl * WSF + (R + PADS) * q);
    const int p0 = 2 * lane + HIST;
    float4 hist[UF], pre[UF][2];
#pragma unroll
    for (int ff = 0; ff < UF; ff++) hist[ff] = make_float4(0.0f, 0.0f, 0.0f, 0.0f);
    auto prefetch = [&](int t) {
#pragma unroll
        for (int ff = 0; ff < UF; ff++)
#pragma unroll
            for (int j = 0; j < 2; j++) {
                float4 v = load_once(&src[ff][(t * TILE + 128 * j + 2 * lane) >> 1]);
                if (!fv[ff]) v = make_float4(0.0f, 0.0f, 0.0f, 0.0f);
                pre[ff][j] = v;
            }
    };
    prefetch(0);
    bool ok = true;
    float2 *drow = dring + (size_t)g * GM::DSTRIDE;
    for (int t = 0; t < ntiles && ok; t++) {
        {
            const int pt = __builtin_amdgcn_readfirstlane(__hip_atomic_load(&sm->ready[w ^ 4], __ATOMIC_RELAXED, __HIP_MEMORY_SCOPE_WORKGROUP));
            if (pt > t) __builtin_amdgcn_s_setprio(2);
            else if (pt < t) __builtin_amdgcn_s_setprio(0);
            else __builtin_amdgcn_s_setprio(1);
        }
#pragma unroll
        for (int ff = 0; ff < UF; ff++) {
            float2 *wf = mywin + ff * WSF;
            if (lane >= 1) *reinterpret_cast<float4 *>(wf + slot_of(p0 - 128)) = hist[ff];
            *reinterpret_cast<float4 *>(wf + slot_of(p0)) = pre[ff][0];
            *reinterpret_cast<float4 *>(wf + slot_of(p0 + 128)) = pre[ff][1];
            hist[ff] = pre[ff][1];
        }
        if (t + 1 < ntiles) prefetch(t + 1);
        v2f a0, a1, a2, a3, a4, a5, a6, a7;
        fir_full8s_asm(rd_addr, a.taps, a0, a1, a2, a3, a4, a5, a6, a7);
        if (t >= DRO) ok = wait_ge(&sm->consumed[g >> 2], t - DRO + 1, abortf);
        const int c = t >> 1;
        if (ok && !(t & 1) && c >= DR) ok = wait_ge(&sm->flushed[g >> 2], c - 1, abortf);
        if (!ok) break;
        const float2 y0 = fir_gain(make_float2(a0.x, a0.y)), y1 = fir_gain(make_float2(a1.x, a1.y)),
                     y2 = fir_gain(make_float2(a2.x, a2.y)), y3 = fir_gain(make_float2(a3.x, a3.y)),
                     y4 = fir_gain(make_float2(a4.x, a4.y)), y5 = fir_gain(make_float2(a5.x, a5.y)),
                     y6 = fir_gain(make_float2(a6.x, a6.y)), y7 = fir_gain(make_float2(a7.x, a7.y));
        float *pi = ring + ((size_t)(g * DRO + (t % DRO)) * 2 + 0) * PITCH + R * q;
        float *pq = pi + PITCH;
        reinterpret_cast<float4 *>(pi)[0] = make_float4(y0.x, y1.x, y2.x, y3.x);
        reinterpret_cast<float4 *>(pi)[1] = make_float4(y4.x, y5.x, y6.x, y7.x);
        reinterpret_cast<float4 *>(pq)[0] = make_float4(y0.y, y1.y, y2.y, y3.y);
        reinterpret_cast<float4 *>(pq)[1] = make_float4(y4.y, y5.y, y6.y, y7.y);
        float2 pick;
        switch (gi) {
        case 0: pick = y0; break;
        case 1: pick = y1; break;
        case 2: pick = y2; break;
        case 3: pick = y3; break;
        case 4: pick = y4; break;
        case 5: pick = y5; break;
        case 6: pick = y6; break;
        default: pick = y7; break;
        }
        drow[(c % DR) * pipe2::S + QL * (t & 1) + q] = pick;
        if (lane == 0) {
            st_release(&sm->ready[w], t + 1);
            if (t & 1) __hip_atomic_store(&sm->loop.ready[w], c + 1, __ATOMIC_RELAXED, __HIP_MEMORY_SCOPE_WORKGROUP);
        }
    }
    if (!ok && lane == 0) {
        __hip_atomic_store(abortf, 1, __ATOMIC_RELAXED, __HIP_MEMORY_SCOPE_WORKGROUP);
        report_status(status, STATUS_PIPE_TIMEOUT);
    }
}

__global__ void __launch_bounds__(1024)
index_majority_kernel(const int32_t *index, int nframes, int32_t *hint, int32_t *mis_count, int32_t *h_stats)
{
    __shared__ int cnt[8];
    if (threadIdx.x < 8) cnt[threadIdx.x] = 0;
    __syncthreads();
    int mine[8] = {0, 0, 0, 0, 0, 0, 0, 0};
    for (int f = threadIdx.x; f < nframes; f += 1024) {
        const int ix = index[f] & 7;
#pragma unroll
        for (int k = 0; k < 8; k++) mine[k] += ix == k;
    }
#pragma unroll
    for (int k = 0; k < 8; k++)
        if (mine[k]) atomicAdd(&cnt[k], mine[k]);
    __syncthreads();
    if (threadIdx.x == 0) {
        int best = 0;
        for (int k = 1; k < 8; k++)
            if (cnt[k] > cnt[best]) best = k;
        const int offm = nframes - cnt[best];
        const int missed = mis_count ? mis_count[0] : 0;
        hint[0] = best;
        if (mis_count) mis_count[0] = 0;
        int4 st = make_int4(best, nframes, offm > missed ? offm : missed, 0);
        *reinterpret_cast<int4 *>(h_stats) = st;
    }
}

static size_t rx_hist_lds_bytes(void)
{
    using namespace histk;
    return sizeof(Ctl) + sizeof(float2) * (size_t)G * WSF + sizeof(float) * (size_t)G * DRO * 2 * PITCH + (size_t)G * lean::ROW_BYTES;
}

bool rx_hist_shape_ok(const FusedArgs &a)
{
    return a.nbw == 1 && !a.costas && !a.state_in && !a.state_out && a.cycles == C && a.frame_size == a.nsym * C &&
           a.nsym % pipe2::S == 0 && a.nsym >= 2 * pipe2::S && (a.frame_pitch & 1) == 0 && ((uintptr_t)a.x & 15) == 0 &&
           a.min_freq < 0.0f && a.max_freq > 0.0f && rx_hist_lds_bytes() <= (size_t)MAX_LDS_BYTES;
}

int launch_rx_hist(const FusedArgs &a0, int32_t *index_true, const int32_t *hint, int32_t *mis_list, int32_t *mis_count, int *status, hipStream_t s)
{
    FusedArgs a = a0;
    if (!rx_hist_shape_ok(a) || !index_true || !hint || !mis_list || !mis_count) return (int)hipErrorInvalidValue;
    a.G = histk::G;
    a.mixed = 2;
    a.share_simd0 = 0;
    a.lean_pair = a.lean_pair != 0;
    a.index = nullptr;
    a.est_tw = nullptr;
    hipLaunchKernelGGL(rx_hist_kernel, dim3((a.nframes + histk::G - 1) / histk::G), dim3(histk::THREADS), rx_hist_lds_bytes(), s, a, index_true,
                       hint, mis_list, mis_count, status);
    return (int)hipGetLastError();
}

int launch_index_majority(const int32_t *index, int nframes, int32_t *hint, int32_t *mis_count, int32_t *h_stats, hipStream_t s)
{
    hipLaunchKernelGGL(index_majority_kernel, dim3(1), dim3(1024), 0, s, index, nframes, hint, mis_count, h_stats);
    return (int)hipGetLastError();
}

int prepare_pipe_kernel(void)
{
    hipError_t e0 = hipFuncSetAttribute(reinterpret_cast<const void *>(rx_hist_kernel), hipFuncAttributeMaxDynamicSharedMemorySize, MAX_LDS_BYTES);
    if (e0 != hipSuccess) return (int)e0;
    hipError_t e = hipFuncSetAttribute(reinterpret_cast<const void *>(costas_pipe_kernel),
                                       hipFuncAttributeMaxDynamicSharedMemorySize, MAX_LDS_BYTES);
    if (e != hipSuccess) return (int)e;
    e = hipFuncSetAttribute(reinterpret_cast<const void *>(rx_pipe2_kernel), hipFuncAttributeMaxDynamicSharedMemorySize,
                            MAX_LDS_BYTES);
    if (e != hipSuccess) return (int)e;
    e = hipFuncSetAttribute(reinterpret_cast<const void *>(rx_lean_kernel<false>), hipFuncAttributeMaxDynamicSharedMemorySize,
                            MAX_LDS_BYTES);
    if (e != hipSuccess) return (int)e;
    e = hipFuncSetAttribute(reinterpret_cast<const void *>(rx_lean_kernel<true>), hipFuncAttributeMaxDynamicSharedMemorySize,
                            MAX_LDS_BYTES);
    if (e != hipSuccess) return (int)e;
    return (int)hipFuncSetAttribute(reinterpret_cast<const void *>(rx_fused_pipe_kernel<GeomNarrow>),
                                    hipFuncAttributeMaxDynamicSharedMemorySize, MAX_LDS_BYTES);
}

}

#ifdef QPSK_PIPE_PROFILE
extern "C" __attribute__((visibility("default"))) int qpsk_prof_timeline(unsigned long long *dst, int n)
{
    if (n > 1024 * 48) n = 1024 * 48;
    return (int)hipMemcpyFromSymbol(dst, HIP_SYMBOL(qpsk::g_timeline), sizeof(unsigned long long) * (size_t)n);
}
#endif
```

Before: 443,800.

## Run Costas chain on guessed timing index while FFT estimate runs beside it

```diff
diff --git a/qpsk_amd/csrc/api.cpp b/qpsk_amd/csrc/api.cpp
--- a/qpsk_amd/csrc/api.cpp
+++ b/qpsk_amd/csrc/api.cpp
@@ -67,6 +67,7 @@
     int lean_pair = -1;
     int viterbi_lds = -1;
     int fft_fused = -1;
+    int fft_guess = -1;
     int viterbi_chunk_rows = -1;
 };
 
@@ -81,6 +82,7 @@
     {"QPSK_STREAM_SCAN", &Tuning::stream_scan}, {"QPSK_STREAM_CARRIER", &Tuning::stream_carrier},
     {"QPSK_LEAN_DMA", &Tuning::lean_dma},     {"QPSK_LEAN_PAIR", &Tuning::lean_pair},
     {"QPSK_EST_WAVES", &Tuning::est_waves},   {"QPSK_HIST_ONEPASS", &Tuning::hist_onepass},
+    {"QPSK_FFT_GUESS", &Tuning::fft_guess},
     {"QPSK_VITERBI_LDS", &Tuning::viterbi_lds},   {"QPSK_VITERBI_CHUNK_ROWS", &Tuning::viterbi_chunk_rows},
 };
 
@@ -111,12 +113,14 @@
     int *d_status = nullptr;
     std::vector<float> h_gains;
     DevBuf index, filtered, mixed, keystream, sympad, mislist;
+    DevBuf specstatus;
     DevBuf datacostas;
     DevBuf vitdec;
     DevBuf softgain;
     int32_t *d_hint = nullptr;
     int32_t *h_hist_stats = nullptr, *d_hist_stats = nullptr;
     bool hint_valid = false;
+    int guess_parity = 0;
     int keystream_len = 0;
     std::map<int, double *> twiddles;
     float *d_fast = nullptr;
@@ -174,6 +178,7 @@
 static int check_status(qpsk_ctx *c)
 {
     const int st = __atomic_exchange_n(c->h_status, 0, __ATOMIC_ACQ_REL);
+    if (st != 0) c->hint_valid = false;
     if (st != STATUS_PIPE_TIMEOUT) c->stream_work_unchecked = false;
     if (st == STATUS_PIPE_TIMEOUT) {
         if (c->nstreams > 0 && c->stream_work_unchecked) {
@@ -415,6 +420,7 @@
     hipFree(c->keystream.p);
     hipFree(c->sympad.p);
     hipFree(c->mislist.p);
+    hipFree(c->specstatus.p);
     hipFree(c->softgain.p);
     hipFree(c->vitdec.p);
     hipFree(c->dfstage.p);
@@ -661,6 +667,8 @@
     bool need_pad = false;
     bool data_rule = false;
     bool need_dump = false;
+    bool fft_books = false;
+    bool fft_guess = false;
 };
 
 static bool tuned_layout(const qpsk_ctx *c, unsigned long long *layout)
@@ -670,7 +678,14 @@
     return true;
 }
 
-static int rx_route(const qpsk_ctx *c, const FusedArgs &a, bool want_data, RxRoute *rt)
+static bool last_batch_on_one_index(const qpsk_ctx *c)
+{
+    if (!c->h_hist_stats) return false;
+    const int seen = __atomic_load_n(&c->h_hist_stats[1], __ATOMIC_ACQUIRE), off_majority = __atomic_load_n(&c->h_hist_stats[2], __ATOMIC_ACQUIRE);
+    return seen > 0 && off_majority == 0;
+}
+
+static int rx_route(const qpsk_ctx *c, const FusedArgs &a, bool want_data, bool ext, RxRoute *rt)
 {
     const int nframes = a.nframes, nbw = a.nbw;
     *rt = RxRoute{};
@@ -740,6 +755,30 @@
                     a.frame_size >= timing_fft_first() + timing_fft_nfft() &&
                     ((rt->kind == K_FUSED_PIPE && rt->nf == pipe_max_nf() && !(a.dbg & (128 | 4))) ||
                      (rt->kind == K_LEAN && lean_est_ok(a, rt->G, rt->layout)));
+    const int fg = tuned(c->tune.fft_guess, -1);
+    rt->fft_books = rt->fused_fft && rt->kind == K_LEAN && !ext && !want_data && !a.state_in && fg != 0 && lean_guess_ok(a, rt->G, rt->layout);
+    rt->fft_guess = rt->fft_books && c->d_hint && c->hint_valid && (fg == 1 || last_batch_on_one_index(c));
+    return QPSK_OK;
+}
+
+static int ensure_hint(qpsk_ctx *c)
+{
+    if (c->d_hint) return QPSK_OK;
+    int32_t *d_hint = nullptr, *h_stats = nullptr, *d_stats = nullptr;
+    hipError_t e = hipMalloc((void **)&d_hint, 4 * sizeof(int32_t));
+    if (e == hipSuccess) e = hipMemset(d_hint, 0, 4 * sizeof(int32_t));
+    if (e == hipSuccess) e = hipHostMalloc((void **)&h_stats, 4 * sizeof(int32_t), hipHostMallocMapped);
+    if (e == hipSuccess) e = hipHostGetDevicePointer((void **)&d_stats, h_stats, 0);
+    if (e != hipSuccess) {
+        if (h_stats) hipHostFree(h_stats);
+        if (d_hint) hipFree(d_hint);
+        return fail(QPSK_ERR_HIP, "the timing guess's books: %s", hipGetErrorString(e));
+    }
+    h_stats[0] = h_stats[1] = h_stats[2] = -1;
+    c->d_hint = d_hint;
+    c->h_hist_stats = h_stats;
+    c->d_hist_stats = d_stats;
+    c->hint_valid = false;
     return QPSK_OK;
 }
 
@@ -747,17 +786,9 @@
 {
     *taken = false;
     if (!rt.pipe_ok || !c->taps_symmetric || !scan_fused_ok(c, (const float *)a.x) || c->tune.pipe_v >= 0) return QPSK_OK;
-    if (!c->d_hint) {
-        HIP_TRY(hipMalloc((void **)&c->d_hint, 2 * sizeof(int32_t)));
-        HIP_TRY(hipMemset(c->d_hint, 0, 2 * sizeof(int32_t)));
-        HIP_TRY(hipHostMalloc((void **)&c->h_hist_stats, 4 * sizeof(int32_t), hipHostMallocMapped));
-        HIP_TRY(hipHostGetDevicePointer((void **)&c->d_hist_stats, c->h_hist_stats, 0));
-        c->h_hist_stats[0] = c->h_hist_stats[1] = c->h_hist_stats[2] = -1;
-        c->hint_valid = false;
-    }
+    if (int rc = ensure_hint(c)) return rc;
     const int op = tuned(c->tune.hist_onepass, -1);
-    const int seen = __atomic_load_n(&c->h_hist_stats[1], __ATOMIC_ACQUIRE), off_majority = __atomic_load_n(&c->h_hist_stats[2], __ATOMIC_ACQUIRE);
-    const bool guess_is_good = seen > 0 && off_majority == 0;
+    const bool guess_is_good = last_batch_on_one_index(c);
     if (op == 0 || !c->hint_valid || !(op == 1 || guess_is_good) || !rx_hist_shape_ok(a)) return QPSK_OK;
     if (int rc = ensure(c, c->index, sizeof(int32_t) * (size_t)a.nframes)) return rc;
     if (int rc = ensure(c, c->mislist, sizeof(int32_t) * (size_t)a.nframes)) return rc;
@@ -787,7 +818,9 @@
     switch (rt.kind) {
     case K_LEAN:
         KERNEL_TRY(launch_rx_lean(a, rt.G, rt.layout, c->d_status, c->stream));
-        c->last_kernel = a.est_tw ? "rx_lean_kernel (FFT timing estimate inside the launch)" : "rx_lean_kernel";
+        c->last_kernel = a.guess    ? "rx_lean_kernel (FFT timing estimate inside the launch, beside the chain on the guessed index) + rx_fused_kernel (fall-back list)"
+                         : a.est_tw ? "rx_lean_kernel (FFT timing estimate inside the launch)"
+                                    : "rx_lean_kernel";
         break;
     case K_PIPE2:
         KERNEL_TRY(launch_rx_pipe2(a, rt.G, rt.layout, c->d_status, c->stream));
@@ -801,6 +834,23 @@
         KERNEL_TRY(launch_rx_fused(a, c->stream));
         c->last_kernel = "rx_fused_kernel";
     }
+    return QPSK_OK;
+}
+
+static int rx_fft_guess_tail(qpsk_ctx *c, const FusedArgs &a)
+{
+    FusedArgs af = a;
+    af.est_tw = af.est_cs = nullptr;
+    af.index_out = nullptr;
+    af.guess = nullptr;
+    af.index = (const int32_t *)c->index.p;
+    af.frame_list = a.mis_list;
+    af.frame_list_count = a.mis_count;
+    af.G = 4;
+    af.S = 64;
+    const GuessTail t = {(const int32_t *)c->index.p, c->d_hint, c->d_hint + 1 + (c->guess_parity ^ 1), c->d_hist_stats, a.spec_status};
+    KERNEL_TRY(launch_rx_fallback_majority(af, t, c->ncu, c->stream));
+    c->guess_parity ^= 1;
     return QPSK_OK;
 }
 
@@ -848,7 +898,7 @@
     }
 
     RxRoute rt;
-    if (int rc = rx_route(c, a, d_data != nullptr, &rt)) return rc;
+    if (int rc = rx_route(c, a, d_data != nullptr, ext != nullptr, &rt)) return rc;
 
     a.data_rule = rt.data_rule;
     if (rt.need_pad) {
@@ -864,6 +914,7 @@
     if (hist_guess) {
         bool taken = false;
         const int rc = rx_hist_onepass(c, a, rt, d_index, &taken);
+        if (rc) c->hint_valid = false;
         if (rc || taken) return rc;
     }
 
@@ -877,10 +928,21 @@
         if (int rc = fft_timing_tables(c, &est_tw, &est_cs)) return rc;
         a.est_tw = reinterpret_cast<const double2 *>(est_tw);
         a.est_cs = reinterpret_cast<const double2 *>(est_cs);
-        a.index_out = d_index ? (int32_t *)c->index.p : nullptr;
-        if (d_index) idx = (const int32_t *)c->index.p;
-    }
-
+        a.index_out = d_index || rt.fft_books ? (int32_t *)c->index.p : nullptr;
+        if (a.index_out) idx = a.index_out;
+    }
+    if (rt.fft_books)
+        if (int rc = ensure_hint(c)) return rc;
+    if (rt.fft_guess) {
+        if (int rc = ensure(c, c->mislist, sizeof(int32_t) * (size_t)nframes)) return rc;
+        if (int rc = ensure(c, c->specstatus, sizeof(int32_t) * (size_t)nframes)) return rc;
+        a.guess = c->d_hint;
+        a.mis_list = (int32_t *)c->mislist.p;
+        a.mis_count = c->d_hint + 1 + c->guess_parity;
+        a.spec_status = (int32_t *)c->specstatus.p;
+    }
+
+    if (rt.fft_guess) c->hint_valid = false;
     if (int rc = rx_launch(c, a, rt)) return rc;
 
     if (hist_guess && c->d_hint && idx && tuned(c->tune.hist_onepass, -1) != 0) {
@@ -891,6 +953,14 @@
         const size_t last0 = (size_t)((nframes - 1) / rt.G) * (size_t)rt.G;
         HIP_TRY(hipMemcpyAsync(a.sym + (size_t)(nframes - 1) * (size_t)c->nsym, a.sym_pad + ((size_t)(nframes - 1) - last0) * (size_t)c->nsym,
                                (size_t)c->nsym, hipMemcpyDeviceToDevice, c->stream));
+    }
+    if (rt.fft_guess) {
+        if (int rc = rx_fft_guess_tail(c, a)) return rc;
+        c->hint_valid = true;
+    } else if (rt.fft_books && idx) {
+        KERNEL_TRY(launch_index_majority(idx, nframes, c->d_hint, c->d_hint + 1, c->d_hist_stats, c->stream));
+        c->guess_parity = 0;
+        c->hint_valid = true;
     }
     if (d_data && !a.data_rule)
         KERNEL_TRY(launch_data_from_costas(a.costas, d_data, (size_t)nframes * (size_t)c->nsym, c->stream));
diff --git a/qpsk_amd/csrc/index_majority.h b/qpsk_amd/csrc/index_majority.h
--- /dev/null
+++ b/qpsk_amd/csrc/index_majority.h
@@ -0,0 +1,54 @@
+#ifndef QPSK_INDEX_MAJORITY_H
+#define QPSK_INDEX_MAJORITY_H
+
+#include <hip/hip_runtime.h>
+#include <stdint.h>
+
+namespace qpsk {
+
+__device__ __forceinline__ void index_majority_block(int *cnt, const int32_t *index, int nframes, int32_t *hint, const int32_t *mis_count,
+                                                     int32_t *mis_zero, int32_t *h_stats, const int32_t *spec = nullptr, int *status = nullptr)
+{
+    constexpr int B = 8;
+    const int nt = (int)blockDim.x, tid = (int)threadIdx.x;
+    const int gi = hint[0];
+    const int missed = mis_count ? mis_count[0] : 0;
+    if (tid < 8) cnt[tid] = 0;
+    __syncthreads();
+    int mine[8] = {0, 0, 0, 0, 0, 0, 0, 0};
+    int bad = 0;
+    for (int base = tid; base < nframes; base += B * nt) {
+        int ix[B], sv[B];
+#pragma unroll
+        for (int j = 0; j < B; j++) {
+            const int f = min(base + j * nt, nframes - 1);
+            ix[j] = index[f];
+            sv[j] = spec ? spec[f] : 0;
+        }
+#pragma unroll
+        for (int j = 0; j < B; j++)
+            if (base + j * nt < nframes) {
+#pragma unroll
+                for (int k = 0; k < 8; k++) mine[k] += (ix[j] & 7) == k;
+                if (sv[j] != 0 && ix[j] == gi) bad = sv[j];
+            }
+    }
+    if (bad && status) __hip_atomic_store(status, bad, __ATOMIC_RELAXED, __HIP_MEMORY_SCOPE_SYSTEM);
+#pragma unroll
+    for (int k = 0; k < 8; k++)
+        if (mine[k]) atomicAdd(&cnt[k], mine[k]);
+    __syncthreads();
+    if (tid == 0) {
+        int best = 0;
+        for (int k = 1; k < 8; k++)
+            if (cnt[k] > cnt[best]) best = k;
+        const int offm = nframes - cnt[best];
+        hint[0] = best;
+        if (mis_zero) mis_zero[0] = 0;
+        int4 st = make_int4(best, nframes, offm > missed ? offm : missed, 0);
+        *reinterpret_cast<int4 *>(h_stats) = st;
+    }
+}
+
+}
+#endif
diff --git a/qpsk_amd/csrc/kernels.h b/qpsk_amd/csrc/kernels.h
--- a/qpsk_amd/csrc/kernels.h
+++ b/qpsk_amd/csrc/kernels.h
@@ -30,6 +30,9 @@
     int fixed_index;
     const double2 *est_tw, *est_cs;
     int32_t *index_out;
+    const int32_t *guess;
+    int32_t *mis_list, *mis_count;
+    int32_t *spec_status;
     int lean_twowin;
     int lean_dma;
     int est_waves;
@@ -97,6 +100,15 @@
 bool rx_hist_shape_ok(const FusedArgs &a);
 int launch_rx_hist(const FusedArgs &a, int32_t *index_true, const int32_t *hint, int32_t *mis_list, int32_t *mis_count, int *status, hipStream_t s);
 int launch_index_majority(const int32_t *index, int nframes, int32_t *hint, int32_t *mis_count, int32_t *h_stats, hipStream_t s);
+bool lean_guess_ok(const FusedArgs &a, int G, unsigned long long layout);
+struct GuessTail {
+    const int32_t *index;
+    int32_t *hint;
+    int32_t *mis_next;
+    int32_t *h_stats;
+    const int32_t *spec_status;
+};
+int launch_rx_fallback_majority(const FusedArgs &a, const GuessTail &t, int ncu, hipStream_t s);
 int launch_rrc_fir(const float *x, const float *memory, float *y, const float *taps, int nframes, int length,
                    hipStream_t s, size_t in_pitch = 0);
 int launch_rrc_fir_stream(const float *x, const float *memory, float *y, const float *taps, int nframes, int length,
diff --git a/qpsk_amd/csrc/kernels.hip b/qpsk_amd/csrc/kernels.hip
--- a/qpsk_amd/csrc/kernels.hip
+++ b/qpsk_amd/csrc/kernels.hip
@@ -3,13 +3,13 @@
 #include "qpsk_device.h"
 #include "fft_lds.h"
 #include "kernels.h"
+#include "index_majority.h"
 
 namespace qpsk {
 
 constexpr int FUSED_THREADS = 256;
 
-__global__ void __launch_bounds__(FUSED_THREADS)
-rx_fused_kernel(FusedArgs a)
+__device__ __forceinline__ void rx_fused_body(const FusedArgs &a, int blk)
 {
     extern __shared__ __attribute__((aligned(16))) unsigned char smem[];
     const int G = a.G, S = a.S, C = a.cycles, L = a.frame_size, N = a.nsym, nbw = a.nbw;
@@ -23,7 +23,7 @@
     int *fid = idx + G;
 
     const int tid = threadIdx.x;
-    const int f0 = blockIdx.x * G;
+    const int f0 = blk * G;
     const int total = a.frame_list_count ? min(*a.frame_list_count, a.nframes) : a.nframes;
     if (f0 >= total) return;
     const int gcount = min(G, total - f0);
@@ -120,6 +120,25 @@
         if (over && a.status) __hip_atomic_store(a.status, STATUS_PHASE_RANGE, __ATOMIC_RELAXED, __HIP_MEMORY_SCOPE_SYSTEM);
         else if (a.status && !loop_state_finite(st.phase, st.freq))
             __hip_atomic_store(a.status, STATUS_NONFINITE, __ATOMIC_RELAXED, __HIP_MEMORY_SCOPE_SYSTEM);
+    }
+}
+
+__global__ void __launch_bounds__(FUSED_THREADS)
+rx_fused_kernel(FusedArgs a)
+{
+    rx_fused_body(a, blockIdx.x);
+}
+
+__global__ void __launch_bounds__(FUSED_THREADS)
+rx_fallback_majority_kernel(FusedArgs a, GuessTail t)
+{
+    __shared__ int cnt[8];
+    if (blockIdx.x == 0)
+        index_majority_block(cnt, t.index, a.nframes, t.hint, a.frame_list_count, t.mis_next, t.h_stats, t.spec_status, a.status);
+    const int total = min(*a.frame_list_count, a.nframes);
+    for (int blk = blockIdx.x; blk * a.G < total; blk += gridDim.x) {
+        __syncthreads();
+        rx_fused_body(a, blk);
     }
 }
 
@@ -579,6 +598,19 @@
     return 0;
 }
 
+int launch_rx_fallback_majority(const FusedArgs &a, const GuessTail &t, int ncu, hipStream_t s)
+{
+    if (a.est_tw || !a.frame_list || !a.frame_list_count || !a.index || !t.index || !t.hint || !t.mis_next || t.mis_next == a.frame_list_count ||
+        !t.h_stats || !t.spec_status)
+        return (int)hipErrorInvalidValue;
+    const int blocks = (a.nframes + a.G - 1) / a.G;
+    const size_t lds = fused_lds_bytes(a.G, a.S, a.cycles, a.nbw);
+    if (lds > 48 * 1024) return (int)hipErrorInvalidValue;
+    hipLaunchKernelGGL(rx_fallback_majority_kernel, dim3(blocks < ncu || ncu < 1 ? blocks : ncu), dim3(FUSED_THREADS), lds, s, a, t);
+    LAUNCH_CHECK();
+    return 0;
+}
+
 __global__ void fft_big_first_kernel(const double2 *__restrict__ in, double2 *__restrict__ out, const double2 *__restrict__ twb,
                                      int n, int log2n, int inverse);
 __global__ void fft_big_late_kernel(double2 *__restrict__ data, const double2 *__restrict__ twn, int n, int log2n, int inverse);
diff --git a/qpsk_amd/csrc/rx_fused.hip b/qpsk_amd/csrc/rx_fused.hip
--- a/qpsk_amd/csrc/rx_fused.hip
+++ b/qpsk_amd/csrc/rx_fused.hip
@@ -15,6 +15,7 @@
 #include "fir_lean_prof_asm.h"
 #endif
 #include "kernels.h"
+#include "index_majority.h"
 
 #ifndef QPSK_PIPE1_ASM
 #define QPSK_PIPE1_ASM 1
@@ -129,7 +130,7 @@
     template <class... A> static __device__ __forceinline__ unsigned run(A &&...a) { return costas_asm_run_lo(a...); }
 };
 
-template <class GM, class ST = StreamHi, class SM>
+template <class GM, class ST = StreamHi, bool SPEC = false, class SM>
 __device__ __forceinline__ void costas_wave(const FusedArgs &a, SM *sm, const float2 *dring, float *zring, int G,
                                             int f0, int lane, int nchunks, int *status)
 {
@@ -376,8 +377,12 @@
         if (a.state_out) { a.state_out[2 * o] = st.phase; a.state_out[2 * o + 1] = st.freq; }
     }
     if (!ok && lane == 0) report_status(status, STATUS_PIPE_TIMEOUT);
-    if (over) report_status(status, STATUS_PHASE_RANGE);
-    else if (active && ok && !loop_state_finite(ph, fr)) report_status(status, STATUS_NONFINITE);
+    if constexpr (SPEC) {
+        if (active && !odd) a.spec_status[f0 + g] = over ? STATUS_PHASE_RANGE : ok && !loop_state_finite(ph, fr) ? STATUS_NONFINITE : 0;
+    } else {
+        if (over) report_status(status, STATUS_PHASE_RANGE);
+        else if (active && ok && !loop_state_finite(ph, fr)) report_status(status, STATUS_NONFINITE);
+    }
 }
 
 template <class GM, int RW = GM::R, bool DATA = false>
@@ -1450,7 +1455,41 @@
     if (!ok && lane == 0) report_status(status, STATUS_PIPE_TIMEOUT);
 }
 
-template <bool DATA>
+template <bool GUESS>
+__device__ __forceinline__ void lean_estimate_frames(const FusedArgs &a, float2 *ewin, const float *etaps, int *eidx, int r, int nwe, int G,
+                                                     int f0, int lane, int gi)
+{
+    const int nf = GUESS ? min(G, a.nframes - f0) : G;
+    if (r >= nf) return;
+    const unsigned erd = lds_addr(ewin + (tfft::R + tfft::PADS) * lane), etap = lds_addr(etaps);
+    tfft::Pre5 pre = tfft::load_frame5(a.x + (size_t)min(f0 + r, a.nframes - 1) * a.frame_pitch, lane);
+    for (int fe = r; fe < nf; fe += nwe) {
+        tfft::stage_frame5(ewin, lane, pre);
+        if (fe + nwe < nf) pre = tfft::load_frame5(a.x + (size_t)min(f0 + fe + nwe, a.nframes - 1) * a.frame_pitch, lane);
+        tfft::wave_sync();
+        v2f e0, e1, e2, e3, e4, e5, e6, e7;
+        fir_full8_asm(erd, etap, e0, e1, e2, e3, e4, e5, e6, e7);
+        const v2f eacc[tfft::R] = {e0, e1, e2, e3, e4, e5, e6, e7};
+        double epv[tfft::R];
+        const tfft::cd u = tfft::power_bin(eacc, ewin, lane, a.est_tw, tfft::NFFT / C, nullptr, epv);
+        if (lane == 0) {
+            const int best = tfft::pick_index(u, a.est_cs, C, nullptr);
+            if constexpr (GUESS) {
+                a.index_out[f0 + fe] = best;
+                if (best != gi) {
+                    const int k = atomicAdd(a.mis_count, 1);
+                    if (k < a.nframes) a.mis_list[k] = f0 + fe;
+                }
+            } else {
+                eidx[fe] = best;
+                if (a.index_out && f0 + fe < a.nframes) a.index_out[f0 + fe] = best;
+            }
+        }
+        tfft::wave_sync();
+    }
+}
+
+template <bool DATA, bool GUESS = false>
 __global__ void __launch_bounds__(pipe2::MAX_THREADS)
 rx_lean_kernel(FusedArgs a, unsigned long long layout, int nwin, int *status)
 {
@@ -1476,35 +1515,19 @@
     if (tid < MAX_WAVES) sm->ready[tid] = 0;
     if (tid == 0) { sm->consumed = 0; sm->abort_flag = 0; }
     const int *est = nullptr;
-    if (a.est_tw) {
-        float *etaps = reinterpret_cast<float *>(rows + (size_t)lean::rows_of(G) * lean::ROW_BYTES);
-        int *eidx = reinterpret_cast<int *>(etaps + 128);
+    float *etaps = reinterpret_cast<float *>(rows + (size_t)lean::rows_of(G) * lean::ROW_BYTES);
+    int *eidx = reinterpret_cast<int *>(etaps + 128);
+    if constexpr (GUESS) {
+        for (int i = tid; i < 128; i += blockDim.x) etaps[i] = i < NTAPS ? a.taps[i] : 0.0f;
+        if (tid < 32) eidx[tid] = a.guess[0];
+        est = eidx;
+    } else if (a.est_tw) {
         for (int i = tid; i < 128; i += blockDim.x) etaps[i] = i < NTAPS ? a.taps[i] : 0.0f;
         __syncthreads();
         const int nw = (int)blockDim.x / 64;
         const int room = (int)((size_t)nwin * UF * lean::WS / tfft::WSLOTS);
         const int nwe = nw < room ? nw : room;
-        if (wave < nwe) {
-            float2 *ewin = win + (size_t)wave * tfft::WSLOTS;
-            const unsigned erd = lds_addr(ewin + (tfft::R + tfft::PADS) * lane), etap = lds_addr(etaps);
-            tfft::Pre5 pre = tfft::load_frame5(a.x + (size_t)min(f0 + wave, a.nframes - 1) * a.frame_pitch, lane);
-            for (int fe = wave; fe < G; fe += nwe) {
-                tfft::stage_frame5(ewin, lane, pre);
-                if (fe + nwe < G) pre = tfft::load_frame5(a.x + (size_t)min(f0 + fe + nwe, a.nframes - 1) * a.frame_pitch, lane);
-                tfft::wave_sync();
-                v2f e0, e1, e2, e3, e4, e5, e6, e7;
-                fir_full8_asm(erd, etap, e0, e1, e2, e3, e4, e5, e6, e7);
-                const v2f eacc[tfft::R] = {e0, e1, e2, e3, e4, e5, e6, e7};
-                double epv[tfft::R];
-                const tfft::cd u = tfft::power_bin(eacc, ewin, lane, a.est_tw, tfft::NFFT / C, nullptr, epv);
-                if (lane == 0) {
-                    const int best = tfft::pick_index(u, a.est_cs, C, nullptr);
-                    eidx[fe] = best;
-                    if (a.index_out && f0 + fe < a.nframes) a.index_out[f0 + fe] = best;
-                }
-                tfft::wave_sync();
-            }
-        }
+        if (wave < nwe) lean_estimate_frames<false>(a, win + (size_t)wave * tfft::WSLOTS, etaps, eidx, wave, nwe, G, f0, lane, 0);
         est = eidx;
     }
     __syncthreads();
@@ -1518,12 +1541,26 @@
                 return;
             }
         }
-        costas_wave<GM>(a, sm, reinterpret_cast<const float2 *>(rows), reinterpret_cast<float *>(rows + lean::Z_OFFSET_BYTES), G,
-                        f0, lane, nchunks, status);
+        costas_wave<GM, StreamHi, GUESS>(a, sm, reinterpret_cast<const float2 *>(rows), reinterpret_cast<float *>(rows + lean::Z_OFFSET_BYTES), G,
+                                         f0, lane, nchunks, status);
         return;
     }
     const int mine = wave < 16 ? (int)((layout >> (4 * wave)) & 15) : 0;
-    if (mine == 0) return;
+    if (mine == 0) {
+        if constexpr (GUESS) {
+            if ((wave & 3) == 0) return;
+            int r = 0, nwe = 0;
+            for (int v = 1; v < (int)blockDim.x / 64; v++)
+                if ((v & 3) != 0 && ((layout >> (4 * v)) & 15) == 0) {
+                    r += v < wave;
+                    nwe++;
+                }
+            __builtin_amdgcn_s_setprio(0);
+            float2 *ewin = reinterpret_cast<float2 *>(reinterpret_cast<unsigned char *>(etaps) + LEAN_EST_LDS_BYTES) + (size_t)r * tfft::WSLOTS;
+            lean_estimate_frames<true>(a, ewin, etaps, nullptr, r, nwe, G, f0, lane, __builtin_amdgcn_readfirstlane(a.guess[0]));
+        }
+        return;
+    }
 #ifdef QPSK_PIPE_PROFILE
     QPSK_TL_STAMP(16 + wave);
 #endif
@@ -1573,8 +1610,10 @@
     bool est_ok;
     int units, nwin, hw;
     int hw_est, nwe;
+    bool guess_ok;
+    int nwg;
     bool twowin, pair;
-    size_t lds, lds_est;
+    size_t lds, lds_est, lds_guess;
 };
 
 static LeanGeometry lean_geometry(const FusedArgs &a, int G, unsigned long long layout)
@@ -1607,12 +1646,21 @@
     g.ok = valid;
     g.est_ok = valid && a.frame_size >= tfft::N0 + tfft::NFFT && g.nwe >= 1 && (G + g.nwe - 1) / g.nwe <= tfft::MAX_FPW && G <= 32 &&
                g.lds_est <= (size_t)MAX_LDS_BYTES;
+    for (int w = 1; w < g.hw_est; w++)
+        if ((w & 3) != 0 && ((layout >> (4 * w)) & 15) == 0) g.nwg++;
+    g.lds_guess = g.lds_est + (size_t)g.nwg * tfft::WSLOTS * sizeof(float2);
+    g.guess_ok = g.est_ok && g.nwg >= 1 && (G + g.nwg - 1) / g.nwg <= tfft::MAX_FPW && g.lds_guess <= (size_t)MAX_LDS_BYTES;
     return g;
 }
 
 bool lean_est_ok(const FusedArgs &a, int G, unsigned long long layout)
 {
     return lean_geometry(a, G, layout).est_ok;
+}
+
+bool lean_guess_ok(const FusedArgs &a, int G, unsigned long long layout)
+{
+    return lean_geometry(a, G, layout).guess_ok;
 }
 
 int launch_rx_lean(const FusedArgs &a0, int G, unsigned long long layout, int *status, hipStream_t s)
@@ -1621,13 +1669,19 @@
     const LeanGeometry g = lean_geometry(a, G, layout);
     if (!g.ok || !lean_shape_ok(a, G) || (a.nframes % G != 0 && !a.sym_pad)) return (int)hipErrorInvalidValue;
     if (a.est_tw && (!g.est_ok || !a.est_cs || a.index)) return (int)hipErrorInvalidValue;
+    if (a.guess && (!g.guess_ok || !a.est_tw || a.data_rule || !a.index_out || !a.mis_list || !a.mis_count || !a.spec_status))
+        return (int)hipErrorInvalidValue;
     a.G = G;
     a.mixed = 2;
     a.share_simd0 = ((layout >> 16) & 15) != 0 || ((layout >> 32) & 15) != 0;
     a.lean_twowin = g.twowin;
     a.lean_pair = g.pair;
-    hipLaunchKernelGGL(a.data_rule ? rx_lean_kernel<true> : rx_lean_kernel<false>, dim3((a.nframes + G - 1) / G), dim3(64 * (a.est_tw ? g.hw_est : g.hw)), a.est_tw ? g.lds_est : g.lds, s, a,
-                       layout, g.nwin, status);
+    const dim3 grid((a.nframes + G - 1) / G);
+    if (a.guess)
+        hipLaunchKernelGGL((rx_lean_kernel<false, true>), grid, dim3(64 * g.hw_est), g.lds_guess, s, a, layout, g.nwin, status);
+    else
+        hipLaunchKernelGGL(a.data_rule ? rx_lean_kernel<true> : rx_lean_kernel<false>, grid, dim3(64 * (a.est_tw ? g.hw_est : g.hw)),
+                           a.est_tw ? g.lds_est : g.lds, s, a, layout, g.nwin, status);
     return (int)hipGetLastError();
 }
 
@@ -1801,7 +1855,10 @@
         }
         if (f0 + g < nframes && comp == 0 && q == 0) {
             index_true[f0 + g] = best;
-            if (best != gi) mis_list[atomicAdd(mis_count, 1)] = f0 + g;
+            if (best != gi) {
+                const int k = atomicAdd(mis_count, 1);
+                if (k < nframes) mis_list[k] = f0 + g;
+            }
         }
         return;
     }
@@ -1892,29 +1949,7 @@
 index_majority_kernel(const int32_t *index, int nframes, int32_t *hint, int32_t *mis_count, int32_t *h_stats)
 {
     __shared__ int cnt[8];
-    if (threadIdx.x < 8) cnt[threadIdx.x] = 0;
-    __syncthreads();
-    int mine[8] = {0, 0, 0, 0, 0, 0, 0, 0};
-    for (int f = threadIdx.x; f < nframes; f += 1024) {
-        const int ix = index[f] & 7;
-#pragma unroll
-        for (int k = 0; k < 8; k++) mine[k] += ix == k;
-    }
-#pragma unroll
-    for (int k = 0; k < 8; k++)
-        if (mine[k]) atomicAdd(&cnt[k], mine[k]);
-    __syncthreads();
-    if (threadIdx.x == 0) {
-        int best = 0;
-        for (int k = 1; k < 8; k++)
-            if (cnt[k] > cnt[best]) best = k;
-        const int offm = nframes - cnt[best];
-        const int missed = mis_count ? mis_count[0] : 0;
-        hint[0] = best;
-        if (mis_count) mis_count[0] = 0;
-        int4 st = make_int4(best, nframes, offm > missed ? offm : missed, 0);
-        *reinterpret_cast<int4 *>(h_stats) = st;
-    }
+    index_majority_block(cnt, index, nframes, hint, mis_count, mis_count, h_stats);
 }
 
 static size_t rx_hist_lds_bytes(void)
@@ -1967,6 +2002,9 @@
     e = hipFuncSetAttribute(reinterpret_cast<const void *>(rx_lean_kernel<true>), hipFuncAttributeMaxDynamicSharedMemorySize,
                             MAX_LDS_BYTES);
     if (e != hipSuccess) return (int)e;
+    e = hipFuncSetAttribute(reinterpret_cast<const void *>(rx_lean_kernel<false, true>), hipFuncAttributeMaxDynamicSharedMemorySize,
+                            MAX_LDS_BYTES);
+    if (e != hipSuccess) return (int)e;
     return (int)hipFuncSetAttribute(reinterpret_cast<const void *>(rx_fused_pipe_kernel<GeomNarrow>),
                                     hipFuncAttributeMaxDynamicSharedMemorySize, MAX_LDS_BYTES);
 }
```

Result: no change. 442,500 (-0.3%).
